# maropu/spark-data-repair-plugin

Hardware: AMD Instinct MI355X
Metric: repaired cells/sec (higher is better)
Workload: dtype f32 gradients (LightGBM's score_t), exact int64 fixed-point histogram sums, f64 scores

## Files before the change

### include/rgbm.h

```cpp
#ifndef RGBM_H_
#define RGBM_H_

#include <stddef.h>
#include <stdint.h>

#ifdef __cplusplus
extern "C" {
#endif

#define RGBM_OK 0
#define RGBM_ERR_ARG (-1)
#define RGBM_ERR_PARAM (-2)
#define RGBM_ERR_LABEL (-3)
#define RGBM_ERR_NO_DEVICE (-10)
#define RGBM_ERR_HIP (-11)
#define RGBM_ERR_NOMEM (-12)
#define RGBM_ERR_FORMAT (-20)

#define RGBM_OBJ_BINARY 0
#define RGBM_OBJ_MULTICLASS 1
#define RGBM_OBJ_REGRESSION 2

typedef struct rgbm_model rgbm_model;
typedef struct rgbm_table rgbm_table;
// ... 35 lines not shown
    int64_t level_atomics_per_row;
} rgbm_train_stats;

int rgbm_device_count(void);
int rgbm_release_cache(void);
const char* rgbm_last_error(void);
int rgbm_version(void);

int rgbm_train(const int32_t* X_colmajor, int64_t n, int32_t f, const int32_t* n_codes,
               const int32_t* y_code, int32_t n_y_codes, const double* y_value,
               const double* class_weight, const double* sample_weight,
               const rgbm_params* p, rgbm_model** out, rgbm_train_stats* stats );

int rgbm_predict(const rgbm_model* m, const int32_t* X_colmajor, int64_t n, int32_t f,
                 int32_t device_id, double* out);

int rgbm_repair_chain(const rgbm_model* const* models, int32_t T, const int32_t* target_col,
                      const int32_t* feat_cols, const int32_t* feat_off,
                      const int32_t* class_code, const int32_t* class_off,
                      int32_t* table_colmajor, int64_t n, int32_t c, int32_t device_id,
                      int32_t* out_label, double* out_prob);

int rgbm_table_create(const int32_t* codes_colmajor, int64_t n, int32_t c, const int32_t* n_codes,
                      int32_t device_id, rgbm_table** out);
int rgbm_table_set_column_kind(rgbm_table* t, int32_t col, int32_t kind);
int rgbm_table_set_column_values(rgbm_table* t, int32_t col, const double* values, int32_t n);
int rgbm_host_alloc(size_t bytes, void** out);
void rgbm_host_free(void* p);
void rgbm_table_free(rgbm_table* t);
int rgbm_table_train(const rgbm_table* t, int32_t target_col, const int32_t* feat_cols, int32_t f,
                     const double* y_value ,
                     const double* class_weight ,
                     const rgbm_params* p, rgbm_model** out, rgbm_train_stats* stats);
int rgbm_table_set_row_multiplicity(rgbm_table* t, const uint8_t* mult );
int rgbm_table_read_row_multiplicity(const rgbm_table* t, uint8_t* mult_out );
int rgbm_table_distinct_rows(const rgbm_table* t, rgbm_table** out, int64_t* n_out, int64_t* inverse_out );
int rgbm_table_distinct_view_info(const rgbm_table* t, int32_t* state, int64_t* rows, int64_t* builds);
int rgbm_distinct_view_eligible(int64_t rows, int32_t f, const rgbm_params* p, int32_t table_has_mult, int64_t min_rows);
typedef struct {
    const rgbm_table* table;
    int32_t target_col, n_features;
    const int32_t* feat_cols;
    const double* y_value;
    const double* class_weight;
    const rgbm_params* params;
    const rgbm_table* valid_table;
    int32_t* valid_label_out;
    double* valid_value_out;
} rgbm_fit_spec;
int rgbm_table_train_batch(const rgbm_fit_spec* fits, int32_t n_fits, rgbm_model** out_models , int32_t* out_status );
int rgbm_table_repair_chain(rgbm_table* t, const rgbm_model* const* models, int32_t T,
                            const int32_t* target_col, const int32_t* feat_cols, const int32_t* feat_off,
                            int64_t row_begin, int64_t n_rows, int32_t* out_label, double* out_prob);
int rgbm_table_read_column(const rgbm_table* t, int32_t col, int32_t* out );

int rgbm_table_detect_nulls(rgbm_table* t, const int32_t* cols, int32_t n_cols, int64_t* n_cells_out);
int rgbm_table_detect_cells(rgbm_table* t, const int32_t* cols, int32_t n_cols, const uint8_t* null_is_error ,
                            const int32_t* keep_lo, const int32_t* keep_hi ,
                            const uint64_t* const* flag_bits , int64_t* n_cells_out);
int rgbm_table_detect_constraint(rgbm_table* t, const int32_t* eq_cols, int32_t n_eq, int32_t iq_col,
                                 const int32_t* cell_cols, int32_t n_cell_cols,
                                 int64_t* n_rows_out , int64_t* n_cells_out);
#define RGBM_DC_EQ 0
#define RGBM_DC_IQ 1
#define RGBM_DC_LT 2
#define RGBM_DC_GT 3
typedef struct rgbm_dc_pred {
    int32_t op;
    int32_t left_col;
    int32_t right_col;
    int32_t reserved;
    const int32_t* left_rank;
    const int32_t* right_rank;
} rgbm_dc_pred;
int rgbm_table_detect_dc(rgbm_table* t, const rgbm_dc_pred* preds, int32_t n_preds, const int32_t* cell_cols, int32_t n_cell_cols,
                         int64_t max_pairs, int64_t* n_rows_out , int64_t* n_cells_out);
int rgbm_table_detect_row_bits(rgbm_table* t, const int32_t* cols, int32_t n_cols, const uint64_t* const* bits ,
                               const int32_t* cell_cols, int32_t n_cell_cols, int64_t* n_rows_out , int64_t* n_cells_out);
int rgbm_table_rows_of_cells(rgbm_table* t, const int64_t* rows, int64_t n_cells, int64_t* n_rows_out);
int rgbm_table_cells_fetch(const rgbm_table* t, int64_t* rows_out , int32_t* cols_out );
int rgbm_table_null_cells(rgbm_table* t, const int64_t* rows, const int32_t* cols, int64_t n_cells,
                          const int32_t* target_cols, int32_t n_targets);
int rgbm_table_read_cells(const rgbm_table* t, const int64_t* rows, const int32_t* cols, int64_t n_cells, int32_t* codes_out);
int rgbm_table_write_cells(rgbm_table* t, const int64_t* rows, const int32_t* cols, const int32_t* codes, int64_t n_cells);
int rgbm_table_gather_rows(const rgbm_table* t, const int64_t* rows, int64_t n_rows, rgbm_table** out);
int rgbm_table_count_codes(const rgbm_table* t, int32_t col, int64_t* counts_out ,
                           int64_t* n_null_out );
int rgbm_table_column_stats(const rgbm_table* t, const int32_t* cols, int32_t n_cols, const int32_t* const* len_lut,
                            int32_t n_bins, int64_t* stats_out, int32_t* edges_out);
int rgbm_table_create_dict(const int32_t* idx_colmajor, int64_t n, int32_t c, const int32_t* const* remap,
                           const int32_t* dict_size , int32_t device_id, rgbm_table** out);
int rgbm_table_repair_pmf(rgbm_table* t, const rgbm_model* m, int32_t target_col, const int32_t* feat_cols, int32_t f,
                          int32_t top_k, double threshold, const int32_t* cur_code, int64_t cap, int64_t* n_cells_out,
                          int64_t* rows_out , int32_t* class_out ,
                          double* prob_out , double* cur_prob_out );
int rgbm_table_repair_pmf_weighted(rgbm_table* t, const rgbm_model* m, int32_t target_col, const int32_t* feat_cols, int32_t f,
                                   int32_t top_k, double threshold, const int32_t* cur_code ,
                                   const int32_t* cost_row , const double* cost ,
                                   int64_t n_cost_rows, double weight, int32_t renormalise, int64_t cap, int64_t* n_cells_out,
                                   int64_t* rows_out , int32_t* class_out , double* prob_out ,
                                   double* cur_prob_out , double* top1_cost_out );
int rgbm_edit_distance(int32_t device_id, const int32_t* a_cp, const int64_t* a_off, int64_t n_a, const int32_t* b_cp,
                       const int64_t* b_off, int64_t n_b, int32_t* dist_out);
int rgbm_table_pair_counts(rgbm_table* t, const int32_t* pair_cols, int32_t n_pairs, const int32_t* const* luts ,
                           const int32_t* n_bins , int64_t* counts_out);
int rgbm_table_cell_domains(rgbm_table* t, int32_t target_col, const int64_t* rows, int64_t n_cells, const int32_t* pair_idx, int32_t k,
                            const int64_t* min_cnt , const uint8_t* single_ok , double beta, int64_t row_count,
                            uint8_t* weak_out, int32_t* top_out, double* top_prob_out, double* probs_out );
int rgbm_table_fd_map(const rgbm_table* t, int32_t x_col, int32_t y_col, int32_t* map_out );
int rgbm_table_rule_fill(rgbm_table* t, int32_t y_col, int32_t x_col , const int32_t* lut, int32_t n_lut, int64_t row_begin,
                         int64_t n_rows, int32_t* out_label );
int rgbm_nearest_values(int32_t device_id, const int32_t* a_cp, const int64_t* a_off, int64_t n_a, const int32_t* b_cp, const int64_t* b_off,
                        int64_t n_b, const double* cost , double threshold, int32_t* nearest_out );
int rgbm_lof_1d(int32_t device_id, const double* values , const int64_t* counts ,
                int32_t d, int32_t k , double threshold ,
                double* score_out , uint64_t* flag_bits_out , int64_t* info_out );
int rgbm_table_kmeans_assign(rgbm_table* t, const int32_t* cols, int32_t n_cols, const int64_t* code_off ,
                             int32_t k, const double* p , int64_t d_tot, const double* h ,
                             int32_t first ,
                             int64_t* counts_out , int64_t* sizes_out , int64_t* n_changed_out);
int rgbm_table_kmeans_read(const rgbm_table* t, int32_t* assign_out );
int rgbm_table_shape(const rgbm_table* t, int64_t* n_out, int32_t* c_out, int32_t* n_codes_out );

#define RGBM_COMM_ID_BYTES 128
#define RGBM_FLAG_ROW_SHARDED 1
#define RGBM_FLAG_WHOLE_TABLE 4
#define RGBM_FLAG_NO_MODEL 2
int rgbm_comm_unique_id(void* id_out );
int rgbm_comm_init(const void* id, int32_t rank, int32_t nranks, int32_t device_id);
int rgbm_comm_finalize(void);
int rgbm_comm_info(int32_t* info );
int rgbm_comm_count(int32_t* n_out );
int rgbm_comm_all_gather_sizes(const int64_t* mine, int32_t n, int64_t* all );
int rgbm_comm_all_gather_bytes(const void* send, int64_t my_bytes, int64_t block_bytes , void* recv );
int rgbm_table_repair_chain_gather(rgbm_table* t, const rgbm_model* const* models, int32_t T, const int32_t* target_col,
                                   const int32_t* feat_cols, const int32_t* feat_off, int64_t row_begin, int64_t n_rows, int64_t max_rows,
                                   int32_t* out_label, double* out_prob);
int rgbm_comm_gather_stats(int64_t* out );
int rgbm_local_group_create(int32_t nranks, int32_t device_id, void** group_out);
void rgbm_local_group_free(void* group);
int rgbm_comm_init_local(void* group, int32_t rank);

int rgbm_fusion_create(int32_t n_members, void** fusion_out);
int rgbm_fusion_join(void* fusion, int32_t member );
int rgbm_fusion_leave(int32_t failed );
int rgbm_fusion_info(void* fusion, int64_t* info );
int rgbm_fusion_free(void* fusion);

int rgbm_model_save(const rgbm_model* m, void* buf, size_t* len);
int rgbm_model_load(const void* buf, size_t len, rgbm_model** out);
void rgbm_model_free(rgbm_model* m);
int rgbm_model_info(const rgbm_model* m, int32_t* info);
int rgbm_model_predict_form(const rgbm_model* m, int32_t* out);
int rgbm_level_pass_plan(const int32_t* nbins, int32_t f, int64_t n_rows, int32_t k, int32_t max_depth, int32_t with_mult, double* out, int32_t out_len, int32_t* n_out);
int rgbm_model_importance(const rgbm_model* m, int32_t type, double* out );

#ifdef __cplusplus
}
#endif
#endif
```

### spark-data-repair-plugin_amd/csrc/rgbm.hip

```cpp
#include <hip/hip_runtime.h>
#include <algorithm>
#include <atomic>
#include <condition_variable>
#include <chrono>
#include <cmath>
#include <cstdio>
#include <cstdlib>
#include <cstring>
#include <deque>
#include <map>
#include <memory>
#include <stdexcept>
#include <mutex>
#include <string>
#include <thread>
#include <vector>

#include "rgbm_host.h"
#include "rgbm_kernels.h"
#include "rgbm_level.h"
#include "rgbm_small.h"


namespace {
using rgh::fail; using rgh::DevBuf; using rgh::use_device; using rgh::StreamGuard; using rgh::guarded;
using rgh::AR_I64; using rgh::AR_U32; using rgh::AR_I32; using rgh::all_reduce; using rgh::all_gather_on; using rgh::stream_sync_watchdog; using rgh::comm_abort;
using rgh::comm_kind; using rgh::comm_rank; using rgh::comm_nranks; using rgh::upload_pinned;

struct Feat {
    int32_t n_codes = 0, V = 0, has_nan = 0; std::vector<int32_t> ub;
    std::vector<uint32_t> unseen;
    bool is_unseen(int32_t c) const { return !unseen.empty() && ((unseen[(size_t)c >> 5] >> (c & 31)) & 1u); }
};
struct Tree {
    int32_t L = 1;
    double *gain = nullptr, *leaf_value = nullptr;
    int32_t *feat = nullptr, *theta = nullptr, *dleft = nullptr, *left = nullptr, *right = nullptr, *leaf_count = nullptr;
    std::unique_ptr<double[]> own;
    static size_t doubles(int L) { const size_t n = (size_t)L - 1; return n + (size_t)L + (5 * n + (size_t)L + 1) / 2; }
    void place(double* p, int L_) {
        L = L_; const size_t n = (size_t)L - 1;
        gain = p; leaf_value = p + n;
        int32_t* q = reinterpret_cast<int32_t*>(p + n + L);
        feat = q; theta = q + n; dleft = q + 2 * n; left = q + 3 * n; right = q + 4 * n; leaf_count = q + 5 * n;
    }
    void alloc(int L_) { own.reset(new double[doubles(L_)]); place(own.get(), L_); }
};

struct DeviceModel {
    DevBuf<rg::PNode> nodes; DevBuf<double> leaf_value;
    DevBuf<uint32_t> qs_masks, qs_used; DevBuf<double> qs_leaves; DevBuf<int32_t> qs_foff; int qs_S = 0, qs_MW = 0;
    DevBuf<uint8_t> lut; DevBuf<long long> lut_off; DevBuf<int32_t> n_codes; DevBuf<uint8_t> miss; DevBuf<int32_t> ident;
    int node_stride = 1, leaf_stride = 1;
};

}

struct rgbm_model {
    int32_t objective = 0, num_class = 0, K = 1, n_iter = 0, F = 0;
    std::vector<Feat> feats;
    std::vector<Tree> trees;
    std::unique_ptr<double[]> tree_arena;
    std::mutex mu;
    std::map<int, DeviceModel*> dev;
    ~rgbm_model() { for (auto& kv : dev) { (void)hipSetDevice(kv.first); delete kv.second; } }
};


namespace {

int32_t mid_code(int32_t a, int32_t b, const double* vals) {
    if (!vals) return (int32_t)(((int64_t)a + (int64_t)b) / 2);
    const double m = (vals[a] + vals[b]) / 2.0;
    int32_t lo = a, hi = b - 1;
    while (lo < hi) { const int32_t c = lo + (hi - lo + 1) / 2; if (vals[c] <= m) lo = c; else hi = c - 1; }
    return lo;
}

int greedy_find_bin(const std::vector<int32_t>& dv, const std::vector<int64_t>& cnt, int max_bin, int64_t total_cnt,
                    int min_data_in_bin, std::vector<int32_t>& ub, const double* vals) {
    const int nd = (int)dv.size();
    ub.clear();
    if (nd <= 0) return 0;
    if (nd <= max_bin) {
        int64_t cur = 0;
        for (int i = 0; i + 1 < nd; ++i) {
            cur += cnt[i];
            if (cur >= min_data_in_bin) { ub.push_back(mid_code(dv[i], dv[i + 1], vals)); cur = 0; }
        }
        ub.push_back(INT32_MAX);
        return (int)ub.size();
    }
    if (min_data_in_bin > 0) {
        max_bin = (int)std::min<int64_t>(max_bin, total_cnt / min_data_in_bin);
        max_bin = std::max(max_bin, 1);
    }
    double mean_bin_size = (double)total_cnt / max_bin;
    int rest_bin_cnt = max_bin;
    int64_t rest_sample_cnt = total_cnt;
    std::vector<char> big(nd, 0);
    for (int i = 0; i < nd; ++i)
        if ((double)cnt[i] >= mean_bin_size) { big[i] = 1; --rest_bin_cnt; rest_sample_cnt -= cnt[i]; }
    mean_bin_size = (double)rest_sample_cnt / rest_bin_cnt;
    std::vector<int32_t> upper(max_bin, INT32_MAX), lower(max_bin, INT32_MAX);
    int bin_cnt = 0;
    lower[0] = dv[0];
    int64_t cur = 0;
    for (int i = 0; i + 1 < nd; ++i) {
        if (!big[i]) rest_sample_cnt -= cnt[i];
        cur += cnt[i];
        double half = mean_bin_size * 0.5f;
        if (half < 1.0) half = 1.0;
        if (big[i] || (double)cur >= mean_bin_size || (big[i + 1] && (double)cur >= half)) {
            upper[bin_cnt] = dv[i];
            ++bin_cnt;
            lower[bin_cnt] = dv[i + 1];
            if (bin_cnt >= max_bin - 1) break;
            cur = 0;
            if (!big[i]) { --rest_bin_cnt; mean_bin_size = (double)rest_sample_cnt / (double)rest_bin_cnt; }
        }
    }
    ++bin_cnt;
    for (int i = 0; i + 1 < bin_cnt; ++i) {
        int32_t v = mid_code(upper[i], lower[i + 1], vals);
        if (ub.empty() || ub.back() != v) ub.push_back(v);
    }
    ub.push_back(INT32_MAX);
    return (int)ub.size();
}

void find_bin(const unsigned int* cnt, int32_t n_codes, int64_t n_train, const rgbm_params& p, Feat& f, const double* vals) {
    std::vector<int32_t> dv; std::vector<int64_t> dc;
    int64_t seen = 0;
    for (int32_t c = 0; c < n_codes; ++c) if (cnt[c]) { dv.push_back(c); dc.push_back(cnt[c]); seen += cnt[c]; }
    const int64_t na = n_train - seen;
    int mb = p.max_bin - (na > 0 ? 1 : 0) - 1;
    if (mb < 1) mb = 1;
    f.n_codes = n_codes; f.has_nan = na > 0 ? 1 : 0;
    f.V = greedy_find_bin(dv, dc, mb, seen, p.min_data_in_bin, f.ub, vals);
}


constexpr double DISTINCT_MAX_RATIO = 0.5;
constexpr long long DISTINCT_MIN_ROWS = 1ll << 20;
struct RunSwitches {
    int grower = 0;
    bool timing = false;
    int lv_lds = 0;
    long long lv_blocks = 0;
    long long mt_blocks = 0;
    int mt_T = 0;
    int mt_rep = 8;
    bool joint_root = true;
    bool mt_acc2 = true;
    bool mt_sparse = true;
    int mt_rot = -1;
    int mt_rot_copies2 = 16;
    int mt_rot_tmin = 2;
    bool step_readback = false;
    int step_threads = 0;
    int step_max_gx = 0;
    bool fx_separate = false;
    bool distinct = true;
    double distinct_max_ratio = DISTINCT_MAX_RATIO;
    long long distinct_min_rows = DISTINCT_MIN_ROWS;
};
RunSwitches read_switches() {
    RunSwitches w;
    if (const char* e = getenv("RGBM_GROWER")) w.grower = strcmp(e, "leafwise") == 0 ? 2 : (strcmp(e, "level") == 0 ? 1 : 0);
    if (const char* e = getenv("RGBM_LV_LDS")) w.lv_lds = atoi(e);
    if (const char* e = getenv("RGBM_LV_BLOCKS")) w.lv_blocks = atoll(e);
    if (const char* e = getenv("RGBM_MT_BLOCKS")) w.mt_blocks = atoll(e);
    if (const char* e = getenv("RGBM_MT_TREES")) w.mt_T = atoi(e);
    if (const char* e = getenv("RGBM_MT_REP")) w.mt_rep = atoi(e);
    if (const char* e = getenv("RGBM_JOINT_ROOT")) w.joint_root = atoi(e) != 0;
    if (const char* e = getenv("RGBM_MT_ACC2")) w.mt_acc2 = atoi(e) != 0;
    if (const char* e = getenv("RGBM_MT_SPARSE")) w.mt_sparse = atoi(e) != 0;
    if (const char* e = getenv("RGBM_STEP_READBACK")) w.step_readback = atoi(e) != 0;
    if (const char* e = getenv("RGBM_STEP_THREADS")) w.step_threads = atoi(e);
    if (const char* e = getenv("RGBM_STEP_MAX_GX")) w.step_max_gx = atoi(e);
    if (const char* e = getenv("RGBM_FX_MEASURE")) w.fx_separate = strcmp(e, "separate") == 0;
    if (const char* e = getenv("RGBM_MT_ROT")) w.mt_rot = atoi(e);
    if (const char* e = getenv("RGBM_MT_ROT_COPIES2")) w.mt_rot_copies2 = atoi(e);
    if (const char* e = getenv("RGBM_MT_ROT_TMIN")) w.mt_rot_tmin = atoi(e);
    if (const char* e = getenv("RGBM_DISTINCT")) w.distinct = atoi(e) != 0;
    if (const char* e = getenv("RGBM_DISTINCT_MAX_RATIO")) { const double r = atof(e); if (r >= 0.0 && r <= 1.0) w.distinct_max_ratio = r; }
    if (const char* e = getenv("RGBM_DISTINCT_MIN_ROWS")) w.distinct_min_rows = std::max(1ll, atoll(e));
    w.timing = getenv("RGBM_TIMING") != nullptr;
    return w;
}

struct LgbRand {
    uint32_t x;
    explicit LgbRand(uint32_t seed) : x(seed) {}
    int rnd16() { x = 214013u * x + 2531011u; return (int)((x >> 16) & 0x7FFF); }
    int rnd32() { x = 214013u * x + 2531011u; return (int)(x & 0x7FFFFFFF); }
    float next_float() { return (float)rnd16() / 32768.0f; }
    int next_int(int lo, int hi) { return rnd32() % (hi - lo) + lo; }
    std::vector<int> sample(int N, int K) {
        std::vector<int> ret;
        if (K > N || K <= 0) return ret;
        if (K == N) { for (int i = 0; i < N; ++i) ret.push_back(i); return ret; }
        if (K > 1 && (double)K > ((double)N / std::log2((double)K))) {
            for (int i = 0; i < N; ++i) {
                double prob = (double)(K - (int)ret.size()) / (double)(N - i);
                if (next_float() < prob) ret.push_back(i);
            }
            return ret;
        }
        std::vector<char> in(N, 0);
        for (int r = N - K; r < N; ++r) { int v = next_int(0, r); if (in[v]) in[r] = 1; else in[v] = 1; }
        for (int i = 0; i < N; ++i) if (in[i]) ret.push_back(i);
        return ret;
    }
};


void check_params(const rgbm_params& p) {
    if (p.objective < 0 || p.objective > 2) throw std::invalid_argument("objective must be 0 (binary), 1 (multiclass) or 2 (regression)");
    if (p.max_bin < 2 || p.max_bin > 255) throw std::invalid_argument("max_bin must be in [2, 255]");
    if (p.num_leaves < 2 || p.num_leaves > 32767) throw std::invalid_argument("num_leaves must be in [2, 32767]");
    if (p.n_estimators < 1) throw std::invalid_argument("n_estimators must be positive");
    if (!(p.learning_rate > 0.0)) throw std::invalid_argument("learning_rate must be positive");
    if (p.objective == 2 && p.learning_rate > 1.0) throw std::invalid_argument("regression with learning_rate > 1 is not supported");
    if (p.objective == 1 && p.num_class < 2) throw std::invalid_argument("multiclass needs num_class >= 2");
    if (p.min_data_in_leaf < 0 || p.lambda_l1 < 0 || p.lambda_l2 < 0) throw std::invalid_argument("negative regularisation / min_data_in_leaf");
    if (p.bagging_fraction <= 0.0 || p.bagging_fraction > 1.0) throw std::invalid_argument("bagging_fraction must be in (0, 1]");
    if (p.feature_fraction <= 0.0 || p.feature_fraction > 1.0) throw std::invalid_argument("feature_fraction must be in (0, 1]");
}

struct HostLabelStats {
    bool valid = false;
    std::vector<double> tot; double suml = 0.0, w_max = 0.0;
};

struct FitHost {
    int64_t n_train = 0; int nchunk = 1; size_t lds_hist = 0;
    std::vector<int32_t> cols, ncod; std::vector<long long> cnt_off, lut_off; std::vector<unsigned int> cnt;
    std::vector<rg::FeatMeta> fmeta; std::vector<rg::ChunkMeta> cmeta; std::vector<uint8_t> lut, miss, trivial;
    std::vector<double> init, yv32; rg::TrainConst tc;
    std::unique_ptr<rgbm_model> model;
};

void fit_setup(const rgbm_table& tab, const double* y_value_in, const double* class_weight, const HostLabelStats* hls, const rgbm_params& p, int32_t F, FitHost& h) {
    using namespace rg;
    const int64_t N = tab.n;
    const int obj = p.objective;
    const std::vector<int32_t>& cols = h.cols; const std::vector<int32_t>& ncod = h.ncod; const std::vector<long long>& cnt_off = h.cnt_off;
    const std::vector<unsigned int>& cnt = h.cnt;
    const int n_y = ncod[F];
    const int K = obj == 1 ? p.num_class : 1;
    const double* y_value = nullptr;
    if (obj == 2) { h.yv32.resize(std::max(n_y, 1)); for (int c = 0; c < n_y; ++c) h.yv32[c] = (double)(float)y_value_in[c]; y_value = h.yv32.data(); }
    const unsigned int* ycnt = cnt.data() + cnt_off[F];
    int64_t& n_train = h.n_train; n_train = 0;
    for (int c = 0; c < n_y; ++c) n_train += ycnt[c];
    if (n_train <= 0) throw std::out_of_range("no training rows (every target cell is NULL)");
    if (N >= (1ll << 31) - 4096) throw std::invalid_argument("more than 2^31 rows per table are not supported");

    h.model.reset(new rgbm_model());
    rgbm_model* model = h.model.get();
    model->objective = obj; model->num_class = obj == 1 ? K : (obj == 0 ? 2 : 1); model->K = K; model->F = F;
    model->feats.resize(F);
    std::vector<FeatMeta>& fmeta = h.fmeta; fmeta.assign(F, FeatMeta());
    std::vector<long long>& lut_off = h.lut_off; lut_off.assign(F + 1, 0);
    std::vector<uint8_t>& miss = h.miss; std::vector<uint8_t>& trivial = h.trivial; miss.assign(F, 0); trivial.assign(F, 0);
    int totbins = 0;
    for (int f = 0; f < F; ++f) {
        Feat& ft = model->feats[f];
        const std::vector<double>* cv = (size_t)cols[f] < tab.col_values.size() ? &tab.col_values[cols[f]] : nullptr;
        find_bin(cnt.data() + cnt_off[f], ncod[f], n_train, p, ft, (cv && (int32_t)cv->size() == ncod[f] && ncod[f] > 0) ? cv->data() : nullptr);
        if ((size_t)cols[f] < tab.col_kind.size() && tab.col_kind[cols[f]] == 1) {
            const unsigned int* cf = cnt.data() + cnt_off[f];
            bool any = false;
            for (int32_t c = 0; c < ncod[f]; ++c) any |= cf[c] == 0;
            if (any) {
                ft.unseen.assign((size_t)(ncod[f] + 31) / 32, 0u);
                for (int32_t c = 0; c < ncod[f]; ++c) if (cf[c] == 0) ft.unseen[(size_t)c >> 5] |= 1u << (c & 31);
            }
        }
        fmeta[f].V = ft.V; fmeta[f].has_nan = ft.has_nan; fmeta[f].nbins = std::max(ft.V + ft.has_nan, 1); fmeta[f].hoff = totbins;
        totbins += fmeta[f].nbins;
        trivial[f] = (ft.V + ft.has_nan <= 1) || ft.V == 0;
        miss[f] = (uint8_t)(ft.has_nan ? ft.V : 0);
        lut_off[f + 1] = lut_off[f] + std::max(ncod[f], 1);
    }
    std::vector<uint8_t>& lut = h.lut; lut.assign(lut_off[F], 0);
    for (int f = 0; f < F; ++f) {
        const Feat& ft = model->feats[f];
        int b = 0;
        for (int c = 0; c < ncod[f]; ++c) { while (b < ft.V - 1 && c > ft.ub[b]) ++b; lut[lut_off[f] + c] = (uint8_t)(ft.V > 0 ? b : 0); }
    }
    const int nchunk = (F + 15) / 16; h.nchunk = nchunk;
    std::vector<ChunkMeta>& cmeta = h.cmeta; cmeta.assign(nchunk, ChunkMeta());
    size_t& lds_hist = h.lds_hist; lds_hist = 0;
    for (int ch = 0; ch < nchunk; ++ch) {
        ChunkMeta& cm = cmeta[ch]; cm.first_feat = ch * 16; cm.nfeat = std::min(16, F - ch * 16); cm.fast_slots = 0; cm.wide_bins = 0;
        for (int j = 0; j < cm.nfeat; ++j) {
            FeatMeta& m = fmeta[ch * 16 + j];
            int sh = 0; while (sh < 5 && (m.nbins << (sh + 1)) <= 256) ++sh;
            m.rep_shift = sh; m.fast_base = cm.fast_slots; m.wide_off = cm.wide_bins;
            cm.fast_slots += m.nbins << sh; cm.wide_bins += m.nbins;
        }
        lds_hist = std::max(lds_hist, (size_t)cm.fast_slots * 16);
    }

    const int nl = std::max({n_y, obj == 0 ? 2 : 1, obj == 1 ? K : 1});
    std::vector<double> tot(nl, 0.0);
    double w_max = 0.0;
    if (hls && hls->valid) { tot = hls->tot; tot.resize(nl, 0.0); w_max = hls->w_max; }
    else {
        for (int c = 0; c < n_y; ++c) {
            const double cw32 = class_weight ? (double)(float)class_weight[c] : 1.0;
            tot[c] = (double)ycnt[c] * cw32;
            if (ycnt[c]) w_max = std::max(w_max, cw32);
        }
    }
    if (!(w_max > 0.0)) w_max = 1.0;
    double sumw = 0.0;
    for (int c = 0; c < nl; ++c) sumw += tot[c];
    std::vector<double>& init = h.init; init.assign(K, 0.0);
    double ymin = 0.0, ymax = 0.0;
    const double keps = k_eps();
    if (obj == 2) {
        bool first = true; double suml = 0.0;
        for (int c = 0; c < n_y; ++c) {
            if (!ycnt[c]) continue;
            if (first) { ymin = ymax = y_value[c]; first = false; }
            ymin = std::min(ymin, y_value[c]); ymax = std::max(ymax, y_value[c]);
        }
        if (hls && hls->valid) suml = hls->suml; else for (int c = 0; c < nl; ++c) suml += tot[c] * (c < n_y ? y_value[c] : 0.0);
        init[0] = suml / sumw;
    } else if (obj == 0) {
        double pavg = tot[1] / sumw;
        if (pavg > 1.0 - keps) pavg = 1.0 - keps;
        if (pavg < keps) pavg = keps;
        init[0] = std::log(pavg / (1.0 - pavg));
    } else {
        for (int k = 0; k < K; ++k) { double pr = tot[k] / sumw; init[k] = std::log(pr > keps ? pr : keps); }
    }
    const double factor = obj == 1 ? (double)K / (double)(K - 1) : 1.0;
    double bound_g, bound_h;
    if (obj == 2) { bound_g = (ymax - ymin) * w_max; if (!(bound_g > 0.0)) bound_g = 1.0; bound_h = w_max; }
    else if (obj == 0) { bound_g = w_max; bound_h = 0.25 * w_max; }
    else { bound_g = w_max; bound_h = factor * 0.25 * w_max; }
    double wr = sumw / w_max;
    long long q_mult = 1;
    if (const char* th = std::getenv("RGBM_TEST_HOOKS")) if (std::atoi(th) != 0) if (const char* ev = std::getenv("RGBM_FX_ROWS")) {
        const double R = std::atof(ev);
        if (R > (double)n_train && R <= 4294967296.0 && n_train > 0) {
            wr *= R / (double)n_train; q_mult = ((long long)R + n_train - 1) / n_train;
            static std::atomic<bool> said{false};
            if (!said.exchange(true)) fprintf(stderr, "[rgbm] TEST HOOK active: RGBM_FX_ROWS=%s coarsens the fixed-point grid of every model trained by this process\n", ev);
        }
    }
    const int e_g = rg::fx_exponent(bound_g, wr), e_h = rg::fx_exponent(bound_h, wr);

    TrainConst& tc = h.tc; memset(&tc, 0, sizeof(tc));
    tc.sg = std::ldexp(1.0, e_g); tc.sh = std::ldexp(1.0, e_h); tc.inv_sg = std::ldexp(1.0, -e_g); tc.inv_sh = std::ldexp(1.0, -e_h);
    tc.l1 = p.lambda_l1; tc.l2 = p.lambda_l2; tc.min_gain_to_split = p.min_gain_to_split; tc.min_sum_hessian = p.min_sum_hessian_in_leaf;
    tc.learning_rate = p.learning_rate; tc.factor = factor; tc.min_data_in_leaf = p.min_data_in_leaf; tc.max_depth = p.max_depth;
    tc.num_leaves = p.num_leaves; tc.F = F; tc.K = K; tc.totbins = std::max(totbins, 1); tc.nchunk = nchunk; tc.objective = obj;
    tc.N = N; tc.n_train = n_train; tc.NG = N;
    tc.fx.c_g = 24 - rg::fx_ceil_log2(bound_g); tc.fx.c_h = 24 - rg::fx_ceil_log2(bound_h);
    tc.fx.e_g_min = e_g; tc.fx.e_h_min = e_h;
    tc.fx.e_g_max = 50 - rg::fx_ceil_log2(bound_g); tc.fx.e_h_max = 50 - rg::fx_ceil_log2(bound_h);
    tc.fx.q_mult = q_mult;
}

struct HostTrees { const int32_t *L, *feat, *theta, *dleft, *left, *right, *cnt; const double *gain, *val; const int32_t* any; };
size_t model_trees_begin(rgbm_model* model, const HostTrees& h, int NE, int K) {
    int n_iter = NE;
    for (int it = 0; it < NE; ++it) if (!h.any[it]) { n_iter = it > 0 ? it : 1; break; }
    model->n_iter = n_iter;
    const size_t nt = (size_t)n_iter * K;
    model->trees.clear(); model->trees.resize(nt);
    size_t total = 0;
    for (size_t t = 0; t < nt; ++t) total += Tree::doubles(std::max(h.L[t], 1));
    model->tree_arena.reset(new double[std::max<size_t>(total, 1)]);
    size_t off = 0;
    for (size_t t = 0; t < nt; ++t) { const int L = std::max(h.L[t], 1); model->trees[t].place(model->tree_arena.get() + off, L); off += Tree::doubles(L); }
    return nt;
}
void model_trees_fill(rgbm_model* model, const HostTrees& h, int NL, size_t t0, size_t t1) {
    for (size_t t = t0; t < t1; ++t) {
        Tree& tr = model->trees[t];
        const size_t n = (size_t)tr.L - 1, nb = t * (NL - 1), lb = t * NL;
        memcpy(tr.feat, h.feat + nb, 4 * n); memcpy(tr.theta, h.theta + nb, 4 * n); memcpy(tr.dleft, h.dleft + nb, 4 * n);
        memcpy(tr.left, h.left + nb, 4 * n); memcpy(tr.right, h.right + nb, 4 * n); memcpy(tr.gain, h.gain + nb, 8 * n);
        memcpy(tr.leaf_value, h.val + lb, 8 * (size_t)tr.L); memcpy(tr.leaf_count, h.cnt + lb, 4 * (size_t)tr.L);
    }
}
void model_from_trees(rgbm_model* model, const HostTrees& h, int NE, int K, int NL) {
    const size_t n = model_trees_begin(model, h, NE, K);
    model_trees_fill(model, h, NL, 0, n);
}

std::vector<uint8_t> make_used_masks(const rgbm_params& p, size_t NT, int F, const std::vector<uint8_t>& trivial) {
    std::vector<uint8_t> used(NT * F, 0);
    LgbRand sr((uint32_t)p.seed);
    sr.rnd16(); sr.rnd16(); sr.rnd16();
    LgbRand ff((uint32_t)sr.rnd16());
    std::vector<int> valid; for (int f = 0; f < F; ++f) if (!trivial[f]) valid.push_back(f);
    for (size_t t = 0; t < NT; ++t) {
        uint8_t* u = used.data() + t * F;
        if (p.feature_fraction < 1.0) {
            int cntf = (int)std::floor((double)valid.size() * p.feature_fraction + 0.5);
            if (cntf < 1) cntf = 1;
            for (int i : ff.sample((int)valid.size(), cntf)) u[valid[i]] = 1;
        } else for (int f : valid) u[f] = 1;
    }
    return used;
}

struct MtLaunch { int ch, slot0, nslots, route, T, G, gx, acc2, rot; };
struct LevelPassPlan {
    int root_gx = 8;
    std::vector<std::vector<MtLaunch>> mt;
    std::vector<int> mt_gx;
    size_t part_items = 0;
};

struct PassCost { double t_fix_us, t_row_ns, t_pair_ns; };
constexpr PassCost MT_COST_REP{14.0, 0.2, 0.75};
constexpr PassCost MT_COST_ROT{14.0, 1.0, 0.5};
constexpr PassCost ROOT_PASS_COST{8.0, 1.2, 0.0};
inline const PassCost& mt_pass_cost(bool , bool rot) { return rot ? MT_COST_ROT : MT_COST_REP; }
inline double pass_model_us(long long workgroups, double rows_per_block, int T, const PassCost& c) {
    const long long rounds = (workgroups + 255) / 256;
    return (double)rounds * (c.t_fix_us + rows_per_block * (c.t_row_ns + (double)T * c.t_pair_ns) * 1e-3);
}

inline int level_lds_bytes(const RunSwitches& sw) { return (sw.lv_lds >= 65536 && sw.lv_lds <= rg::LV_LDS_BYTES) ? sw.lv_lds : rg::LV_LDS_BYTES; }

LevelPassPlan plan_level_passes(const RunSwitches& sw, const std::vector<rg::FeatMeta>& fmeta, const std::vector<rg::ChunkMeta>& cmeta,
                                long long N, int K, int max_depth, bool wm , int lds_bytes) {
    using namespace rg;
    const int nchunk = (int)cmeta.size();
    LevelPassPlan P;
    P.mt.resize(LV_MAX_DEPTH + 1); P.mt_gx.assign(LV_MAX_DEPTH + 1, 8);
    const long long ntiles = (N + LV_TILE - 1) / LV_TILE;
    {
        const long long cu_slots = 256, per = (long long)K * nchunk;
        const long long gmin = std::max<long long>(1, (N + (1ll << 22) - 1) >> 22);
        auto time_of = [&](long long g) { return pass_model_us(g * per, (double)N / (double)g, 1, ROOT_PASS_COST); };
        const long long gfloor = std::max<long long>(8, (gmin + 7) / 8 * 8), gcap = std::max<long long>(gfloor, std::min<long long>(512, (ntiles + 7) / 8 * 8));
        long long g2 = gfloor; double best2 = -1.0;
        for (int pass = 0; pass < 2 && best2 < 0.0; ++pass)
            for (long long g = gfloor; g <= gcap; g += 8) {
                if (pass == 0 && per >= 16 && (g * per < 3 * cu_slots || g * per > 5 * cu_slots)) continue;
                const double t = time_of(g);
                if (best2 < 0.0 || t < best2 * (1.0 - 1e-9)) { best2 = t; g2 = g; }
            }
        if (sw.lv_blocks >= 1) g2 = (sw.lv_blocks + 7) / 8 * 8;
        P.root_gx = (int)g2;
    }
    for (int ch = 0; ch < nchunk; ++ch)
        if ((long long)lv_slots(fmeta.data() + cmeta[ch].first_feat, cmeta[ch].nfeat, 0) * 16 + LV_ROOT_FIXED > lds_bytes)
            throw std::invalid_argument("histogram of one node exceeds LDS");
    P.part_items = (size_t)K * P.root_gx;
    for (int level = 1; level < max_depth; ++level) {
        const int worst = 1 << (level - 1);
        bool acc2 = nchunk == 2 && sw.mt_acc2;
        if (acc2) {
            const long long nb2 = ((long long)lv_slots(fmeta.data() + cmeta[0].first_feat, cmeta[0].nfeat, 0) + lv_slots(fmeta.data() + cmeta[1].first_feat, cmeta[1].nfeat, 0)) * 16;
            if (nb2 > mt_hist_bytes(lds_bytes, MT_THREADS_ACC2, true, true, cmeta[1].nfeat > 15 || wm)) acc2 = false;
        }
        if (wm && nchunk == 2 && !acc2) throw std::invalid_argument("a two-chunk table with row multiplicities needs the one-pass level form (the multiplicity rides in the second record)");
        for (int ch = 0; ch < (acc2 ? 1 : nchunk); ++ch) {
            const FeatMeta* fm = fmeta.data() + cmeta[ch].first_feat;
            long long node_bytes = (long long)lv_slots(fm, cmeta[ch].nfeat, 0) * 16;
            if (acc2) node_bytes += (long long)lv_slots(fmeta.data() + cmeta[1].first_feat, cmeta[1].nfeat, 0) * 16;
            const int mt_thr = acc2 ? MT_THREADS_ACC2 : LV_THREADS;
            const bool li_arr = cmeta[acc2 ? 1 : ch].nfeat > 15 || wm;
            const long long hist_room = mt_hist_bytes(lds_bytes, mt_thr, acc2, acc2 , li_arr);
            long long cap = hist_room / std::max<long long>(node_bytes, 1);
            cap = std::min<long long>(cap, MT_MAX_NODES);
            if (cap < 1) throw std::invalid_argument("histogram of one node exceeds LDS");
            const int win = (int)std::min<long long>(worst, cap);
            const long long rep_target = std::max(1, sw.mt_rep);
            const long long t_nodes = std::max<long long>(win, cap / rep_target);
            int T = (int)std::max<long long>(1, std::min<long long>(std::min<long long>(t_nodes / win, MT_MAX_T), std::min<long long>(K, MT_RT_BUDGET / (2 * worst))));
            if (sw.mt_T >= 1) T = std::max(1, std::min(T, sw.mt_T));
            const bool plain1 = nchunk == 1 || acc2;
            const bool rot_full = cmeta[ch].nfeat >= 12 && (!acc2 || cmeta[1].nfeat >= 12);
            const long long rot_node_bytes = node_bytes + mt_rot_dummy(true) * 16;
            const long long cap_rot = std::min<long long>(hist_room / rot_node_bytes, MT_MAX_NODES);
            const long long T_rot = std::min<long long>(std::min<long long>(cap_rot / win, MT_MAX_T), std::min<long long>(K, MT_RT_BUDGET / (2 * worst)));
            const bool few_trees = T < sw.mt_rot_tmin && T_rot >= 2 * (long long)T;
            const bool rot = plain1 && (sw.mt_rot == 1 || (sw.mt_rot < 0 && rot_full && (cap * 2 < (long long)sw.mt_rot_copies2 * T * win || few_trees))) &&
                             (long long)T * win * rot_node_bytes <= hist_room;
            if (rot && sw.mt_T < 1) T = (int)std::max<long long>(T, T_rot);
            const int G = (K + T - 1) / T;
            for (int s0 = 0; s0 < worst; s0 += win)
                P.mt[level].push_back(MtLaunch{ch, s0, win, (ch == 0 && s0 == 0) ? 1 : 0, T, G, 0, acc2 ? 1 : 0, rot ? 1 : 0});
        }
        const long long gmin = std::max<long long>(1, (N + (1ll << 22) - 1) >> 22);
        const long long nwt = (N + MT_WT_ROWS - 1) / MT_WT_ROWS;
        const long long gx_lo = std::max<long long>(8, (gmin + 7) / 8 * 8), gx_hi = std::max<long long>(gx_lo, std::min<long long>(512, (nwt / (4 * (LV_THREADS / 64)) + 7) / 8 * 8));
        long long gx = gx_lo; double best = 0.0;
        for (long long g = gx_lo; g <= gx_hi; g += 8) {
            double t = 0.0;
            for (const auto& L : P.mt[level]) t += pass_model_us((long long)L.G * g, (double)N / (double)g, std::min(L.T, K), mt_pass_cost(L.acc2 != 0, L.rot != 0));
            if (g == gx_lo || t < best * (1.0 - 1e-9)) { best = t; gx = g; }
        }
        if (sw.mt_blocks >= 1) gx = (sw.mt_blocks + 7) / 8 * 8;
        P.mt_gx[level] = (int)gx;
        for (auto& L : P.mt[level]) L.gx = (int)gx;
        P.part_items = std::max(P.part_items, (size_t)K * (size_t)gx * (size_t)worst);
    }
    return P;
}

struct JointRootPlan {
    bool on = false;
    std::vector<std::vector<int>> groups;
    std::vector<rg::FeatMeta> vfm; rg::ChunkMeta vcm;
    std::vector<rg::JointFeat> jf;
    std::vector<int16_t> binfeat;
};
JointRootPlan plan_joint_root(const std::vector<rg::FeatMeta>& fmeta, int totbins, bool wm, int lds_bytes) {
    using namespace rg;
    const int F = (int)fmeta.size();
    JointRootPlan J;
    std::vector<int> order(F); for (int f = 0; f < F; ++f) order[f] = f;
    std::stable_sort(order.begin(), order.end(), [&](int a, int b) { return fmeta[a].nbins > fmeta[b].nbins; });
    std::vector<int> prod;
    for (int f : order) {
        int best = -1;
        for (size_t g = 0; g < J.groups.size(); ++g)
            if ((long long)prod[g] * fmeta[f].nbins <= 256 && (best < 0 || prod[g] > prod[best])) best = (int)g;
        if (best < 0) { J.groups.emplace_back(); prod.push_back(1); best = (int)J.groups.size() - 1; }
        J.groups[best].push_back(f); prod[best] *= fmeta[f].nbins;
    }
    const int VF = (int)J.groups.size();
    if (VF > (wm ? 15 : 16) || VF > F - 2) return J;
    J.vfm.resize(VF); J.jf.resize(F); J.binfeat.assign(totbins, 0);
    ChunkMeta& vcm = J.vcm; vcm.first_feat = 0; vcm.nfeat = VF; vcm.fast_slots = 0; vcm.wide_bins = 0;
    for (int v = 0; v < VF; ++v) {
        FeatMeta& m = J.vfm[v]; memset(&m, 0, sizeof(m));
        m.V = prod[v]; m.has_nan = 0; m.nbins = prod[v]; m.hoff = vcm.wide_bins; m.wide_off = vcm.wide_bins;
        int sh = 0; while (sh < 5 && (m.nbins << (sh + 1)) <= 256) ++sh;
        m.rep_shift = sh; m.fast_base = vcm.fast_slots; vcm.fast_slots += m.nbins << sh; vcm.wide_bins += m.nbins;
        int stride = 1;
        for (int f : J.groups[v]) {
            JointFeat& j = J.jf[f]; memset(&j, 0, sizeof(j));
            j.voff = m.hoff; j.stride = stride; j.nbins = fmeta[f].nbins; j.nbv = prod[v]; j.hoff = fmeta[f].hoff; j.vbyte = v;
            stride *= fmeta[f].nbins;
            for (int b = 0; b < fmeta[f].nbins; ++b) J.binfeat[fmeta[f].hoff + b] = (int16_t)f;
        }
    }
    J.on = (long long)lv_slots(J.vfm.data(), VF, 0) * 16 + LV_ROOT_FIXED <= lds_bytes;
    return J;
}

#define RGBM_MT_FORMS(X) \
    X(0, rg::LV_THREADS, false, false, false)  \
    X(1, rg::LV_THREADS, false, false, false)  \
    X(1, rg::LV_THREADS, false, false, true)   \
    X(2, rg::LV_THREADS, false, false, false)  \
    X(2, rg::MT_THREADS_ACC2, true, true, false)  \
    X(2, rg::MT_THREADS_ACC2, true, true, true)
struct MtForm { int nchr, threads; bool acc2, spec, rot; };
constexpr MtForm MT_FORMS[] = {
#define RGBM_MT_FORM_ENTRY(NCHR, THR, ACC, SPEC, ROT) {NCHR, THR, ACC, SPEC, ROT},
    RGBM_MT_FORMS(RGBM_MT_FORM_ENTRY)
#undef RGBM_MT_FORM_ENTRY
};
using MtKernel = decltype(&rg::k_level_mt<1, false, true, rg::LV_THREADS, false, false, false>);
MtKernel mt_kernel(const MtForm& f, bool bag, bool route) {
#define RGBM_MT_FORM_KERNEL(NCHR, THR, ACC, SPEC, ROT) \
    if (f.nchr == NCHR && f.threads == THR && f.acc2 == ACC && f.spec == SPEC && f.rot == ROT) \
        return bag ? (route ? rg::k_level_mt<NCHR, true, true, THR, ACC, SPEC, ROT> : rg::k_level_mt<NCHR, true, false, THR, ACC, SPEC, ROT>) \
                   : (route ? rg::k_level_mt<NCHR, false, true, THR, ACC, SPEC, ROT> : rg::k_level_mt<NCHR, false, false, THR, ACC, SPEC, ROT>);
    RGBM_MT_FORMS(RGBM_MT_FORM_KERNEL)
#undef RGBM_MT_FORM_KERNEL
    throw std::logic_error("level pass: no such launch form");
}
void launch_level_mt(const MtForm& f, bool bag, bool route, dim3 grid, hipStream_t s, const uint4* rec, const float2* gh, uint8_t* node, const uint8_t* inbag,
                     const rg::LvPlan* plan, rg::HistBin* part, int32_t* count, const rg::FeatMeta* fmeta, const rg::ChunkMeta* cmeta, int32_t* err_flag,
                     const rg::FxScale* fxs, const rg::LevelConst& c) {
    hipLaunchKernelGGL(mt_kernel(f, bag, route), grid, dim3(f.threads), rg::LV_LDS_BYTES, s, rec, gh, node, inbag, plan, part, count, fmeta, cmeta, err_flag, fxs, c);
}
struct HistTimers {
    bool on; hipStream_t s;
    std::deque<rgh::Event> ev; std::vector<char> root;
    template <typename Fn> void timed(bool is_root, Fn&& fn) {
        if (!on) { fn(); return; }
        HIPCHK(hipEventRecord(ev.emplace_back().e, s));
        fn();
        HIPCHK(hipEventRecord(ev.emplace_back().e, s));
        root.push_back(is_root ? 1 : 0);
    }
};

struct LevelTrace {
    struct Rec { std::string name; int it, level; size_t off, bytes; };
    const char* dir; bool on; hipStream_t s;
    int lo = 44, hi = 44, cur_it = 0;
    std::vector<Rec> idx; size_t used = 0;
    DevBuf<unsigned char> buf;
    LevelTrace(bool level_mode, int K, hipStream_t stream) : dir(getenv("RGBM_TRACE")), s(stream) {
        on = dir && level_mode && (!getenv("RGBM_TRACE_K") || atoi(getenv("RGBM_TRACE_K")) == K);
        if (on && getenv("RGBM_TRACE_ITERS")) sscanf(getenv("RGBM_TRACE_ITERS"), "%d:%d", &lo, &hi);
    }
    void copy(const char* name, int level, const void* src, size_t bytes) {
        if (!on || cur_it < lo || cur_it > hi) return;
        if (used + bytes > buf.n) return;
        HIPCHK(hipMemcpyAsync(buf.p + used, src, bytes, hipMemcpyDeviceToDevice, s));
        idx.push_back({name, cur_it, level, used, bytes}); used += (bytes + 15) & ~(size_t)15;
    }
    void sum(const char* name, const void* src, size_t bytes) {
        if (!on || used + 16 > buf.n) return;
        HIPCHK(hipMemsetAsync(buf.p + used, 0, 8, s));
        rgh::trace_sum(src, bytes, (unsigned long long*)(buf.p + used), s);
        idx.push_back({name, cur_it, -1, used, 8}); used += 16;
    }
    void write(int target_col) {
        if (!on || !used) return;
        std::vector<unsigned char> h(used);
        HIPCHK(hipMemcpy(h.data(), buf.p, used, hipMemcpyDeviceToHost));
        char path[512];
        snprintf(path, sizeof(path), "%s/target%d.bin", dir, target_col);
        if (FILE* f = fopen(path, "wb")) { fwrite(h.data(), 1, h.size(), f); fclose(f); }
        snprintf(path, sizeof(path), "%s/target%d.idx", dir, target_col);
        if (FILE* f = fopen(path, "w")) { for (const auto& r : idx) fprintf(f, "%s %d %d %zu %zu\n", r.name.c_str(), r.it, r.level, r.off, r.bytes); fclose(f); }
    }
};

void fill_train_stats(rgbm_train_stats* stats, float total_ms, const HistTimers& timers, const HostTrees& h, const rgbm_params& p, bool level_mode, bool use_bagging,
                      int nranks , int64_t N, int64_t n_train, int F, int root_feats ,
                      int K, unsigned long long statrows) {
    const int NE = p.n_estimators, NL = p.num_leaves;
    memset(stats, 0, sizeof(*stats));
    stats->total_ms = total_ms;
    stats->hist_launches = (int64_t)timers.root.size();
    for (size_t i = 0; i < timers.root.size(); ++i) {
        float m2 = 0.f; HIPCHK(hipEventElapsedTime(&m2, timers.ev[2 * i].e, timers.ev[2 * i + 1].e));
        stats->hist_ms += m2; if (timers.root[i]) stats->root_ms += m2;
    }
    stats->trees = (int64_t)NE * K;
    const bool root_done = n_train >= (int64_t)p.min_data_in_leaf * 2;
    if (level_mode) {
        const int64_t root_rows = (root_done && !use_bagging) ? (int64_t)NE * K * n_train : 0;
        const int64_t rows_acc = (int64_t)(statrows / (unsigned long long)nranks);
        stats->hist_rows = rows_acc; stats->root_rows = root_rows / nranks;
        stats->root_atomics_per_row = 2 * (int64_t)root_feats; stats->level_atomics_per_row = 2 * (int64_t)F;
        stats->hist_bytes = rows_acc * ((int64_t)F + 8);
        return;
    }
    int64_t rows = 0, root_rows = 0;
    for (size_t t = 0; t < (size_t)NE * K; ++t) {
        const int L = h.L[t];
        const int32_t* left = h.left + t * (NL - 1); const int32_t* right = h.right + t * (NL - 1);
        if (root_done) { rows += N; root_rows += N; }
        std::vector<int64_t> fin(h.cnt + t * NL, h.cnt + t * NL + NL);
        std::vector<int64_t> nodecnt(std::max(L - 1, 1), 0);
        auto sub = [&](int ch) -> int64_t { return ch < 0 ? fin[~ch] : nodecnt[ch]; };
        for (int j = L - 2; j >= 0; --j) nodecnt[j] = sub(left[j]) + sub(right[j]);
        std::vector<int> node_depth(std::max(L - 1, 1), 0);
        for (int j = 0; j < L - 1; ++j) {
            const int lc = left[j], rc = right[j];
            if (lc >= 0) node_depth[lc] = node_depth[j] + 1;
            if (rc >= 0) node_depth[rc] = node_depth[j] + 1;
            const int64_t a = sub(lc), b = sub(rc);
            bool go = j + 2 < NL;
            if (p.max_depth > 0 && node_depth[j] + 1 >= p.max_depth) go = false;
            if (a < (int64_t)p.min_data_in_leaf * 2 && b < (int64_t)p.min_data_in_leaf * 2) go = false;
            if (go) rows += std::min(a, b);
        }
    }
    stats->hist_rows = rows; stats->root_rows = root_rows;
    stats->hist_bytes = rows * ((int64_t)F + 8) + (rows - root_rows) * 4;
}

void check_fit_args(const rgbm_table& tab, int32_t target_col, const int32_t* feat_cols, int32_t F, const double* y_value, const rgbm_params& p) {
    check_params(p);
    if (F <= 0) throw std::invalid_argument("no feature columns");
    if (target_col < 0 || target_col >= tab.c) throw std::invalid_argument("target column out of range");
    for (int f = 0; f < F; ++f) if (feat_cols[f] < 0 || feat_cols[f] >= tab.c) throw std::invalid_argument("feature column out of range");
    const int obj = p.objective, n_y = tab.n_codes[target_col];
    if (obj == 1 && n_y > p.num_class) throw std::out_of_range("target has more label codes than num_class");
    if (obj == 0 && n_y > 2) throw std::out_of_range("binary objective with more than 2 label codes");
    if (obj == 2 && !y_value) throw std::out_of_range("regression needs the y_value dictionary");
}

struct BinRecords {
    DevBuf<int32_t> cols, ncod; DevBuf<long long> cnt_off; DevBuf<unsigned int> cnt;
    DevBuf<rg::FeatMeta> fmeta; DevBuf<rg::ChunkMeta> cmeta; DevBuf<long long> lut_off; DevBuf<uint8_t> lut, miss; DevBuf<uint4> rec;
    void count_codes(const rgbm_table& tab, int32_t target_col, const int32_t* feat_cols, int32_t F, FitHost& h, hipStream_t s) {
        h.cols.assign(feat_cols, feat_cols + F); h.cols.push_back(target_col);
        h.ncod.resize(F + 1); h.cnt_off.assign(F + 2, 0);
        for (int f = 0; f <= F; ++f) { h.ncod[f] = tab.n_codes[h.cols[f]]; h.cnt_off[f + 1] = h.cnt_off[f] + std::max(h.ncod[f], 1); }
        cols.alloc(F + 1); ncod.alloc(F + 1); cnt_off.alloc(F + 2); cnt.alloc(h.cnt_off[F + 1]);
        cols.upload(h.cols.data(), F + 1, s); ncod.upload(h.ncod.data(), F + 1, s); cnt_off.upload(h.cnt_off.data(), F + 2, s); cnt.zero(s);
        const int gx = (int)std::min<int64_t>((tab.n + 255) / 256, 1024);
        hipLaunchKernelGGL(rg::k_count_codes, dim3(gx, F + 1), dim3(256), 0, s, tab.codes.p, (long long)tab.n, tab.codes.p + (long long)target_col * tab.n, cols.p, ncod.p,
                           cnt_off.p, cnt.p, tab.has_mult ? tab.mult.p : (const uint8_t*)nullptr);
    }
    void download_counts(FitHost& h, hipStream_t s) const { h.cnt.resize(cnt.n); cnt.download(h.cnt.data(), cnt.n, s); }
    void fill(const FitHost& h, long long N, hipStream_t s) {
        const int F = h.tc.F;
        fmeta.alloc(F); cmeta.alloc(h.nchunk); lut_off.alloc(F + 1); lut.alloc(h.lut.size()); miss.alloc(F);
        fmeta.upload(h.fmeta.data(), F, s); cmeta.upload(h.cmeta.data(), h.nchunk, s); lut_off.upload(h.lut_off.data(), F + 1, s);
        lut.upload(h.lut.data(), h.lut.size(), s); miss.upload(h.miss.data(), F, s);
        rec.alloc((size_t)h.nchunk * N);
    }
    void pack(const rgbm_table& t, const uint8_t* lut_, const uint8_t* miss_, uint4* out, const uint8_t* mult, hipStream_t s) const {
        hipLaunchKernelGGL(rg::k_pack_bins, dim3((unsigned)((t.n + 255) / 256)), dim3(256), 0, s, t.codes.p, (long long)t.n, 0ll, (long long)t.n, cols.p, ncod.p,
                           lut_off.p, lut_, miss_, (int)fmeta.n, (int)cmeta.n, out, mult);
    }
    void pack(const rgbm_table& tab, hipStream_t s) { pack(tab, lut.p, miss.p, rec.p, tab.has_mult ? tab.mult.p : (const uint8_t*)nullptr, s); }
};

struct BagState {
    DevBuf<unsigned int> blk, rand, bagcnt; DevBuf<int32_t> sorted_rows, oob; DevBuf<uint8_t> inbag;
    std::vector<unsigned int> seeds;
    long long off = 0, local = 0, nrb = 1;
    void order_rows(const int32_t* d_ycol, long long N, long long n_train, hipStream_t s) {
        const long long nblk = (N + 1023) / 1024;
        blk.alloc(nblk); sorted_rows.alloc(n_train); oob.alloc(n_train); inbag.alloc(N); bagcnt.alloc(2);
        hipLaunchKernelGGL(rg::k_block_count, dim3((unsigned)nblk), dim3(256), 0, s, d_ycol, N, blk.p);
        hipLaunchKernelGGL(rg::k_block_scan, dim3(1), dim3(1024), 0, s, blk.p, nblk);
        hipLaunchKernelGGL(rg::k_stable_compact, dim3((unsigned)nblk), dim3(256), 0, s, d_ycol, N, blk.p, sorted_rows.p);
    }
    void seed(const rgbm_params& p, long long bag_off, long long bag_local, hipStream_t s) {
        off = bag_off; local = bag_local;
        nrb = std::max<long long>(1, (off + local + 1023) / 1024 - off / 1024);
        LgbRand sr2((uint32_t)p.seed); sr2.rnd16();
        const int bagging_seed = sr2.rnd16();
        seeds.resize(nrb);
        for (long long b = 0; b < nrb; ++b) seeds[b] = (unsigned int)(bagging_seed + off / 1024 + b);
        rand.alloc(nrb); rand.upload(seeds.data(), nrb, s);
    }
};

struct TreeBlock {
    DevBuf<int32_t> L, feat, theta, dleft, left, right, cnt, any; DevBuf<double> gain, val;
    void alloc(size_t NT, int NL, int NE, hipStream_t s) {
        const size_t nn = NT * (size_t)(NL - 1), nl = NT * (size_t)NL;
        any.alloc(NE); any.zero(s);
        L.alloc(NT); feat.alloc(nn); theta.alloc(nn); dleft.alloc(nn); left.alloc(nn); right.alloc(nn); cnt.alloc(nl); gain.alloc(nn); val.alloc(nl);
        cnt.zero(s); val.zero(s);
    }
    rg::TreeOut out() const { return rg::TreeOut{L.p, feat.p, theta.p, dleft.p, left.p, right.p, gain.p, val.p, cnt.p}; }
    void host_layout(size_t (&off)[11]) const {
        const size_t bytes[10] = {L.n * 4, feat.n * 4, theta.n * 4, dleft.n * 4, left.n * 4, right.n * 4, cnt.n * 4, gain.n * 8, val.n * 8, any.n * 4};
        off[0] = 0;
        for (int i = 0; i < 10; ++i) off[i + 1] = off[i] + ((bytes[i] + 63) & ~(size_t)63);
    }
    size_t host_bytes() const { size_t off[11]; host_layout(off); return off[10]; }
    HostTrees download(char* base, hipStream_t s) const {
        size_t off[11]; host_layout(off);
        auto get = [&](const auto& buf, int i) { auto* h = reinterpret_cast<decltype(buf.p)>(base + off[i]); buf.download(h, buf.n, s); return h; };
        return HostTrees{get(L, 0), get(feat, 1), get(theta, 2), get(dleft, 3), get(left, 4), get(right, 5), get(cnt, 6), get(gain, 7), get(val, 8), get(any, 9)};
    }
};

struct FitState {
    const rgbm_table& tab; const rgbm_params& p; hipStream_t s; const int32_t F;
    const RunSwitches sw = read_switches();
    const int K = p.objective == 1 ? p.num_class : 1, NL = p.num_leaves, NE = p.n_estimators; const int64_t N = tab.n;
    const bool use_bagging = p.bagging_freq > 0 && p.bagging_fraction < 1.0;
    const bool level_mode = p.max_depth >= 1 && p.max_depth <= rg::LV_MAX_DEPTH && F <= 255 && sw.grower != 2;
    const bool dp = (p.reserved & RGBM_FLAG_ROW_SHARDED) != 0;
    const int32_t* d_ycol; const uint8_t* d_mult = tab.has_mult ? tab.mult.p : (const uint8_t*)nullptr;
    FitHost h; BinRecords bins;
    DevBuf<int32_t> base;
    DevBuf<unsigned int> counter;
    DevBuf<float2> gh;
    DevBuf<double> score, init;
    DevBuf<unsigned long long> fxq;
    DevBuf<rg::FxScale> fxs;
    DevBuf<unsigned long long> qpart; long long fx_parts = 0; bool fx_fused = false;
    TreeBlock trees;
    DevBuf<double> cw, yv, sw_rows; DevBuf<uint8_t> used;
    BagState bag; DevBuf<unsigned int> bagcnt_g;
    const unsigned int* n_in_ptr = nullptr;
    DevBuf<int32_t> it;
    HistTimers timers;

    FitState(const rgbm_table& tab_, int32_t target_col, int32_t F_, const rgbm_params& p_, bool timed, hipStream_t s_)
        : tab(tab_), p(p_), s(s_), F(F_), d_ycol(tab_.codes.p + (long long)target_col * tab_.n), timers{timed, s_} {}

    int grad_gx() const { return (int)std::min<long long>((N + 255) / 256, 4096); }
    bool mc_tile() const { return p.objective == 1 && K >= 16 && K <= 112; }
    bool mc_rows() const { return p.objective == 1 && K < 16; }
    void alloc_fx_parts() {
        if (sw.fx_separate || (p.objective == 1 && !mc_tile() && !mc_rows())) return;
        fx_fused = true; fx_parts = mc_tile() ? (N + 63) / 64 : (mc_rows() ? ((N + 255) / 256) * 4 : (long long)grad_gx());
        qpart.alloc((size_t)fx_parts * K * 2);
    }
    void enqueue_grad(uint8_t* node0, long long NS);
    void enqueue_bagging();
};

struct LevelGrower {
    FitState& st; hipStream_t s;
    int root_feats;
    unsigned long long statrows = 0;
    rg::LevelConst lc, lcj; LevelPassPlan passes;
    const int n_hnodes = (1 << st.p.max_depth) - 1;
    bool use_reduce = false;
    bool joint_root = false; int vtotbins = 0;
    DevBuf<rg::FeatMeta> vfmeta; DevBuf<rg::ChunkMeta> vcmeta; DevBuf<uint4> rec_j; DevBuf<rg::HistBin> part_j, red_j; DevBuf<rg::JointFeat> jf; DevBuf<int16_t> binfeat;
    DevBuf<uint8_t> node; DevBuf<rg::LvPlan> plan; DevBuf<rg::SNode> snodes;
    DevBuf<rg::ScanLane> scan_map; std::vector<rg::ScanLane> h_scan; int scan_waves = 0; bool step_hist_lds = true;
    int step_threads = 512, step_max_gx = 256;
    DevBuf<rg::HistBin> part, lpool, part_red; DevBuf<int32_t> count, count_g, err, leafnode; DevBuf<double> ndelta; DevBuf<unsigned long long> d_statrows;
    const int score_gx = (int)std::max<long long>(1, std::min<long long>((st.N + 1023) / 1024, (2048 + st.K - 1) / st.K));
    LevelTrace trace;
    int32_t h_err = 0;
    std::vector<rg::RootLayout> h_root_lay; std::vector<rg::MtLayout> h_mt_lay; std::vector<int> mt_lay_keys;
    DevBuf<rg::RootLayout> root_lay; DevBuf<rg::MtLayout> mt_lay;
    static int mt_lay_key(const MtLaunch& L) { return L.ch * 4 + (L.acc2 ? 2 : 0) + (L.rot ? 1 : 0); }
    int mt_lay_index(const MtLaunch& L) const {
        for (size_t i = 0; i < mt_lay_keys.size(); ++i) if (mt_lay_keys[i] == mt_lay_key(L)) return (int)i;
        return -1;
    }

    explicit LevelGrower(FitState& st_) : st(st_), s(st_.s), root_feats(st_.F), trace(true, st_.K, st_.s) {
        using namespace rg;
        memset(&lc, 0, sizeof(lc)); memset(&lcj, 0, sizeof(lcj));
        lc.lds_bytes = level_lds_bytes(st.sw);
        lc.nchunk = st.h.nchunk; lc.K = st.K; lc.F = st.F; lc.totbins = st.h.tc.totbins;
        lc.num_leaves = st.NL; lc.max_depth = st.p.max_depth; lc.min_data_in_leaf = st.p.min_data_in_leaf; lc.N = st.N; lc.NS = (st.N + 255) & ~255ll; lc.NG = lc.NS;
        lc.sib_local = (st.dp && comm_rank() == 0) ? 1 : 0;
        lc.has_mult = st.tab.has_mult ? 1u : 0u;
        passes = plan_level_passes(st.sw, st.h.fmeta, st.h.cmeta, st.N, st.K, st.p.max_depth, st.tab.has_mult, lc.lds_bytes);
        lc.gx = passes.root_gx; lc.xcd_blocks = 1; lc.max_built = 1;
        node.alloc((size_t)st.K * lc.NS);
        HIPCHK(hipMemsetAsync(node.p, 0xFF, (size_t)st.K * lc.NS, s));
        plan.alloc(st.K); snodes.alloc((size_t)st.K * 256);
        part.alloc(passes.part_items * st.h.tc.totbins); lpool.alloc((size_t)st.K * n_hnodes * st.h.tc.totbins);
        scan_waves = scan_lane_map(st.h.fmeta.data(), st.F, h_scan);
        scan_map.alloc(h_scan.size()); scan_map.upload(h_scan.data(), h_scan.size(), s);
        step_hist_lds = ls_hist_in_lds(st.h.tc.totbins, st.F) && !st.sw.step_readback;
        if (st.sw.step_threads >= 128 && st.sw.step_threads <= LS_MAX_THREADS && st.sw.step_threads % 64 == 0) step_threads = st.sw.step_threads;
        if (st.sw.step_max_gx >= 1) step_max_gx = st.sw.step_max_gx;
        count.alloc((size_t)st.K * 256); use_reduce = st.dp || lc.gx > step_max_gx;
        if (st.dp) count_g.alloc((size_t)st.K * 256);
        const int max_built_all = 1 << std::max(0, st.p.max_depth - 2);
        part_red.alloc((size_t)st.K * max_built_all * st.h.tc.totbins + (size_t)st.K * 128 );
        leafnode.alloc((size_t)st.K * LV_MAX_LEAVES); err.alloc(1); err.zero(s); ndelta.alloc((size_t)st.K * 256); d_statrows.alloc(1); d_statrows.zero(s);
        if (st.sw.joint_root && ((long long)st.K * st.N >= (1ll << 21) || (st.tab.has_mult && st.h.nchunk == 2))) {
            const JointRootPlan jp = plan_joint_root(st.h.fmeta, st.h.tc.totbins, st.tab.has_mult, lc.lds_bytes);
            if (jp.on) {
                const int VF = (int)jp.vfm.size();
                joint_root = true; vtotbins = jp.vcm.wide_bins;
                vfmeta.alloc(VF); vfmeta.upload(jp.vfm.data(), VF, s); vcmeta.alloc(1); vcmeta.upload(&jp.vcm, 1, s);
                jf.alloc(st.F); jf.upload(jp.jf.data(), st.F, s); binfeat.alloc(jp.binfeat.size()); binfeat.upload(jp.binfeat.data(), jp.binfeat.size(), s);
                rec_j.alloc((size_t)st.N);
                hipLaunchKernelGGL(k_pack_joint, dim3((unsigned)((st.N + 255) / 256)), dim3(256), 0, s, st.bins.rec.p, (long long)st.N, st.F, jf.p, rec_j.p, st.tab.has_mult ? st.h.nchunk - 1 : -1);
                part_j.alloc((size_t)st.K * lc.gx * vtotbins); red_j.alloc((size_t)st.K * vtotbins + (size_t)st.K * 128 );
                lcj = lc; lcj.nchunk = 1; lcj.F = VF; lcj.totbins = vtotbins; lcj.max_built = 1;
                h_root_lay.resize(1); root_layout_fill(h_root_lay[0], jp.vfm.data(), VF, lc.lds_bytes);
                use_reduce = true; root_feats = VF;
                HIPCHK(hipStreamSynchronize(s));
            }
        }
        if (st.tab.has_mult && st.h.nchunk == 2 && !joint_root)
            throw std::invalid_argument("a two-chunk table with row multiplicities needs the joint-bin root pass (its record carries the multiplicity); this feature set does not pack into 15 groups");
        if (!joint_root) {
            h_root_lay.resize(st.h.nchunk);
            for (int ch = 0; ch < st.h.nchunk; ++ch) root_layout_fill(h_root_lay[ch], st.h.fmeta.data() + st.h.cmeta[ch].first_feat, st.h.cmeta[ch].nfeat, lc.lds_bytes);
        }
        root_lay.alloc(h_root_lay.size()); root_lay.upload(h_root_lay.data(), h_root_lay.size(), s);
        lc.root_lay = root_lay.p; lcj.root_lay = root_lay.p;
        for (int level = 1; level < st.p.max_depth; ++level) for (const auto& L : passes.mt[level]) if (mt_lay_index(L) < 0) {
            const bool acc2 = L.acc2 != 0;
            const ChunkMeta& cm = st.h.cmeta[L.ch];
            const int nf_last = acc2 ? st.h.cmeta[1].nfeat : cm.nfeat;
            const bool li_in_rec = nf_last <= 15 && !st.tab.has_mult;
            mt_lay_keys.push_back(mt_lay_key(L)); h_mt_lay.emplace_back();
            mt_layout_fill(h_mt_lay.back(), st.h.fmeta.data() + cm.first_feat, cm.nfeat, acc2 ? st.h.fmeta.data() + st.h.cmeta[1].first_feat : nullptr, acc2 ? st.h.cmeta[1].nfeat : 0,
                           cm.wide_bins, L.rot != 0, mt_hist_bytes(lc.lds_bytes, acc2 ? MT_THREADS_ACC2 : LV_THREADS, acc2, acc2, !li_in_rec));
        }
        if (!h_mt_lay.empty()) { mt_lay.alloc(h_mt_lay.size()); mt_lay.upload(h_mt_lay.data(), h_mt_lay.size(), s); }
        if (st.sw.timing) {
            fprintf(stderr, "[rgbm] root: gx %d joint %d groups %d\n", lc.gx, joint_root ? 1 : 0, joint_root ? lcj.F : 0);
            for (int level = 1; level < st.p.max_depth; ++level) for (const auto& L : passes.mt[level])
                fprintf(stderr, "[rgbm] level %d launch: chunk %d slots %d..%d route %d T %d G %d gx %d acc2 %d rot %d\n", level, L.ch, L.slot0, L.slot0 + L.nslots - 1, L.route, L.T, L.G, L.gx, L.acc2, L.rot);
        }
        rgh::once_per_device(st.tab.device, rgh::ONCE_LEVEL_LDS, [] {
            HIPCHK(hipFuncSetAttribute((const void*)rg::k_level_root, hipFuncAttributeMaxDynamicSharedMemorySize, rg::LV_LDS_BYTES));
            for (const MtForm& f : MT_FORMS) for (int bag = 0; bag < 2; ++bag) for (int route = 0; route < 2; ++route)
                HIPCHK(hipFuncSetAttribute((const void*)mt_kernel(f, bag != 0, route != 0), hipFuncAttributeMaxDynamicSharedMemorySize, rg::LV_LDS_BYTES));
        });
        if (trace.on) trace.buf.alloc(((size_t)st.K * n_hnodes * st.h.tc.totbins * 16 + (size_t)st.K * 256 * (sizeof(SNode) + 4) + (size_t)st.K * sizeof(LvPlan) + 4096) * (size_t)(st.p.max_depth + 1) * (size_t)(trace.hi - trace.lo + 1) + (size_t)st.NE * 64 + 4096);
    }

    void trace_level(int level) {
        trace.copy("count", level, count.p, (size_t)st.K * 256 * 4);
        trace.copy("plan", level, plan.p, (size_t)st.K * sizeof(rg::LvPlan));
        trace.copy("snodes", level, snodes.p, (size_t)st.K * 256 * sizeof(rg::SNode));
        trace.copy("lpool", level, lpool.p, (size_t)st.K * n_hnodes * st.h.tc.totbins * 16);
    }
    std::pair<const rg::HistBin*, rg::LevelConst> exchange(bool root, int nb, const rg::LevelConst& lp) {
        using namespace rg;
        if (root ? !use_reduce : (!st.dp && lp.gx <= step_max_gx)) return {part.p, lp};
        if (root && joint_root) {
            hipLaunchKernelGGL(k_level_reduce, dim3((vtotbins + 63) / 64, 1, st.K), dim3(256), 0, s, part_j.p, red_j.p, plan.p, count.p, 1, 1, lcj);
            hipLaunchKernelGGL(k_level_marginal, dim3((st.h.tc.totbins + 255) / 256, st.K), dim3(256), 0, s, red_j.p, part_red.p, plan.p, count.p, jf.p, binfeat.p, vtotbins, lc);
        } else
            hipLaunchKernelGGL(k_level_reduce, dim3((st.h.tc.totbins + 63) / 64, nb, st.K), dim3(256), 0, s, part.p, part_red.p, plan.p, count.p, root ? 1 : 0, nb, lp);
        if (st.dp) {
            const size_t nh = (size_t)st.K * nb * st.h.tc.totbins * 2;
            all_reduce(part_red.p, nh + (size_t)st.K * 256, AR_I64, s);
            hipLaunchKernelGGL(k_counts_unpack, dim3(st.K), dim3(256), 0, s, reinterpret_cast<const long long*>(part_red.p) + nh, count_g.p);
        }
        LevelConst r = lp; r.gx = 1; r.max_built = nb;
        return {part_red.p, r};
    }
    void enqueue_iteration(int it) {
        using namespace rg;
        const TreeOut to = st.trees.out();
        trace.cur_it = it;
        trace.sum("gh", st.gh.p, (size_t)st.K * st.h.tc.NG * 8);
        hipLaunchKernelGGL(k_level_init, dim3(st.K), dim3(64), 0, s, plan.p, snodes.p, count.p, st.n_in_ptr, (long long)st.h.n_train, st.fxq.p, st.h.tc.fx, st.fxs.p, st.it.p, lc);
        const size_t step_lds = ls_lds_bytes(st.h.tc.totbins, st.F, step_hist_lds);
        int32_t* cntg = st.dp ? count_g.p : count.p;
        st.timers.timed(true, [&]() {
            if (joint_root)
                hipLaunchKernelGGL(k_level_root, dim3((unsigned)lc.gx * (unsigned)st.K, 1, 1), dim3(LV_THREADS), lc.lds_bytes, s, rec_j.p, st.gh.p, node.p, plan.p, part_j.p,
                                   vfmeta.p, vcmeta.p, st.fxs.p, lcj);
            else
                hipLaunchKernelGGL(k_level_root, dim3((unsigned)lc.gx * (unsigned)st.K, 1, st.h.nchunk), dim3(LV_THREADS), lc.lds_bytes, s, st.bins.rec.p, st.gh.p, node.p, plan.p, part.p,
                                   st.bins.fmeta.p, st.bins.cmeta.p, st.fxs.p, lc);
        });
        {
            auto ex = exchange(true, 1, lc);
            hipLaunchKernelGGL(k_level_step<true>, dim3(1, st.K), dim3(step_threads), step_lds, s, ex.first, lpool.p, plan.p, snodes.p, cntg, count.p, st.bins.fmeta.p,
                               st.used.p, scan_map.p, scan_waves, step_hist_lds ? 1 : 0, d_statrows.p, st.it.p, n_hnodes, st.fxs.p, st.h.tc, ex.second);
            trace_level(0);
        }
        for (int level = 1; level < st.p.max_depth; ++level) {
            hipLaunchKernelGGL(k_level_plan, dim3(st.K), dim3(64), 0, s, plan.p, snodes.p, st.bins.fmeta.p, level, st.h.tc, lc);
            LevelConst lp = lc;
            lp.xcd_blocks = 0; lp.gx = passes.mt_gx[level]; lp.max_built = 1 << (level - 1);
            for (const MtLaunch& L : passes.mt[level]) {
                LevelConst l1 = lp;
                l1.mt_T = L.T; l1.mt_G = L.G; l1.mt_ch = L.ch; l1.mt_slot0 = L.slot0; l1.mt_nslots = L.nslots; l1.mt_route = L.route; l1.mt_sparse = st.sw.mt_sparse ? 1 : 0;
                l1.mt_lay = mt_lay.p + mt_lay_index(L);
                const bool acc2 = L.acc2 != 0;
                const MtForm form{acc2 ? 2 : (st.h.nchunk <= 2 ? st.h.nchunk : 0), acc2 ? MT_THREADS_ACC2 : LV_THREADS, acc2, acc2, L.rot != 0};
                st.timers.timed(false, [&]() {
                    launch_level_mt(form, st.use_bagging, L.route != 0, dim3((unsigned)L.G * (unsigned)L.gx), s, st.bins.rec.p, st.gh.p, node.p, st.bag.inbag.p,
                                    plan.p, part.p, count.p, st.bins.fmeta.p, st.bins.cmeta.p, err.p, st.fxs.p, l1);
                });
            }
            auto ex = exchange(false, 1 << (level - 1), lp);
            hipLaunchKernelGGL(k_level_step<false>, dim3(1 << (level - 1), st.K), dim3(step_threads), step_lds, s, ex.first, lpool.p, plan.p, snodes.p,
                               cntg, count.p, st.bins.fmeta.p, st.used.p, scan_map.p, scan_waves, step_hist_lds ? 1 : 0, d_statrows.p, st.it.p, n_hnodes, st.fxs.p, st.h.tc, ex.second);
            trace_level(level);
        }
        hipLaunchKernelGGL(k_level_plan, dim3(st.K), dim3(64), 0, s, plan.p, snodes.p, st.bins.fmeta.p, st.p.max_depth, st.h.tc, lc);
        hipLaunchKernelGGL(k_level_replay, dim3(st.K), dim3(64), 0, s, plan.p, snodes.p, cntg, to, st.init.p, ndelta.p, leafnode.p, st.trees.any.p, err.p, st.it.p, st.h.tc);
        hipLaunchKernelGGL(k_level_final, dim3(score_gx, st.K), dim3(256), 0, s, st.bins.rec.p, node.p, st.bag.inbag.p, plan.p, to, ndelta.p, st.score.p, count.p, st.it.p, lc);
        if (st.dp) { hipLaunchKernelGGL(k_copy_i32, dim3(st.K), dim3(256), 0, s, count.p, count_g.p, (long long)st.K * 256); all_reduce(count_g.p, (size_t)st.K * 256, AR_I32, s); }
        hipLaunchKernelGGL(k_level_leafcount, dim3(st.K), dim3(LV_MAX_LEAVES), 0, s, plan.p, cntg, leafnode.p, to, st.it.p, st.h.tc);
        trace_level(st.p.max_depth);
        trace.sum("score", st.score.p, (size_t)st.K * st.N * 8); trace.sum("node", node.p, (size_t)st.K * lc.NS);
    }
    void enqueue_report() { err.download(&h_err, 1, s); d_statrows.download(&statrows, 1, s); }
    void report(int32_t target_col) {
        trace.write(target_col);
        if (h_err & 2) throw std::runtime_error("level grower: a level pass was launched with more built nodes / route entries than its workgroup tables hold (sizing violated)");
        if (h_err) throw std::runtime_error("level grower: a node outside the speculative expansion was selected (expansion bound violated)");
    }
};

struct LeafwiseGrower {
    FitState& st; hipStream_t s;
    DevBuf<int32_t> idx0, idx1, sorted; DevBuf<rg::HistBin> pool; DevBuf<rg::TreeState> state; DevBuf<rg::Leaf> leaves; DevBuf<rg::Cand> cand; DevBuf<double> upd;
    const long long root_tiles = (st.N + rg::TILE_ROWS - 1) / rg::TILE_ROWS;
    const int hist_gx = (int)std::max<long long>(1, std::min<long long>(root_tiles, (1536 + (long long)st.K * st.h.nchunk - 1) / ((long long)st.K * st.h.nchunk)));
    const int part_gx = (int)std::max<long long>(1, std::min<long long>((st.h.n_train + 1023) / 1024, (1024 + st.K - 1) / st.K));
    const int upd_gx = (int)std::max<long long>(1, std::min<long long>((st.h.n_train + 255) / 256, (2048 + st.K - 1) / st.K));
    const size_t upd_lds = (size_t)(3 * st.NL + (st.NL & 1)) * 4 + (size_t)st.NL * 8;

    explicit LeafwiseGrower(FitState& st_) : st(st_), s(st_.s) {
        idx0.alloc((size_t)st.K * st.h.n_train); idx1.alloc((size_t)st.K * st.h.n_train);
        pool.alloc((size_t)st.K * st.NL * st.h.tc.totbins);
        state.alloc(st.K); leaves.alloc((size_t)st.K * st.NL); cand.alloc((size_t)st.K * 2 * st.F);
        upd.alloc((size_t)st.K * st.NL); sorted.alloc((size_t)st.K * st.NL * 3);
        if (st.h.lds_hist > 64 * 1024)
            rgh::once_per_device(st.tab.device, rgh::ONCE_HIST_LDS, [] { HIPCHK(hipFuncSetAttribute((const void*)rg::k_hist, hipFuncAttributeMaxDynamicSharedMemorySize, 160 * 1024)); });
        if (st.h.lds_hist > 160 * 1024) throw std::invalid_argument("histogram working set exceeds LDS");
    }
    void enqueue_iteration(int it) {
        using namespace rg;
        const TreeOut to = st.trees.out();
        const uint8_t* usedp = st.used.p + (size_t)it * st.K * st.F;
        hipLaunchKernelGGL(k_init_iter, dim3(st.K), dim3(64), 0, s, state.p, leaves.p, pool.p, to, st.n_in_ptr, it, st.h.tc);
        for (int step = 0; step < st.NL - 1; ++step) {
            st.timers.timed(step == 0, [&]() {
                hipLaunchKernelGGL(k_hist, dim3(hist_gx, st.K, st.h.nchunk), dim3(256), st.h.lds_hist, s, st.bins.rec.p, st.gh.p, idx0.p, idx1.p, st.base.p,
                                   state.p, pool.p, st.bins.fmeta.p, st.bins.cmeta.p, st.fxs.p, st.h.tc);
            });
            hipLaunchKernelGGL(k_split_find, dim3((st.F + 3) / 4, st.K), dim3(256), 0, s, pool.p, state.p, leaves.p, st.bins.fmeta.p, usedp, cand.p, st.fxs.p, st.h.tc);
            hipLaunchKernelGGL(k_tree_step, dim3(st.K), dim3(64), 0, s, state.p, leaves.p, cand.p, pool.p, st.bins.fmeta.p, to, it, st.h.tc);
            hipLaunchKernelGGL(k_partition, dim3(part_gx, st.K), dim3(256), 0, s, reinterpret_cast<const uint8_t*>(st.bins.rec.p), idx0.p, idx1.p, st.base.p, state.p, st.h.tc);
            hipLaunchKernelGGL(k_finish_split, dim3(st.K), dim3(64), 0, s, state.p, leaves.p, to, it, st.h.tc);
        }
        hipLaunchKernelGGL(k_finalize_tree, dim3(st.K), dim3(64), 0, s, state.p, leaves.p, to, st.init.p, upd.p, sorted.p, st.trees.any.p, it, st.h.tc);
        hipLaunchKernelGGL(k_score_update, dim3(upd_gx, st.K), dim3(256), upd_lds, s, state.p, leaves.p, sorted.p, upd.p, idx0.p, idx1.p, st.base.p, st.score.p, st.n_in_ptr, st.h.tc);
        if (st.use_bagging)
            hipLaunchKernelGGL(k_score_update_oob, dim3(upd_gx, st.K), dim3(256), 0, s, reinterpret_cast<const uint8_t*>(st.bins.rec.p), st.bag.oob.p, st.bag.bagcnt.p,
                               state.p, to, st.bins.fmeta.p, upd.p, st.score.p, it, st.h.tc);
    }
};

void FitState::enqueue_grad(uint8_t* node0, long long NS) {
    using namespace rg;
    if (p.objective == 0) hipLaunchKernelGGL(k_grad<0>, dim3(grad_gx()), dim3(256), 0, s, score.p, d_ycol, yv.p, cw.p, sw_rows.p, bag.inbag.p, gh.p, node0, NS, qpart.p, d_mult, h.tc);
    else if (mc_rows())
        hipLaunchKernelGGL(k_grad_mc_rows<256>, dim3((unsigned)((N + 255) / 256)), dim3(256), (size_t)K * 256 * 8, s, score.p, d_ycol, cw.p, sw_rows.p, bag.inbag.p, gh.p, node0, NS, qpart.p, d_mult, h.tc);
    else if (mc_tile())
        hipLaunchKernelGGL(k_grad_mc, dim3((unsigned)((N + 63) / 64)), dim3(256), (size_t)(K * 64 + 320) * 8, s, score.p, d_ycol, cw.p, sw_rows.p, bag.inbag.p, gh.p, node0, NS, qpart.p, d_mult, h.tc);
    else if (p.objective == 1) hipLaunchKernelGGL(k_grad<1>, dim3(grad_gx()), dim3(256), 0, s, score.p, d_ycol, yv.p, cw.p, sw_rows.p, bag.inbag.p, gh.p, node0, NS, (unsigned long long*)nullptr, d_mult, h.tc);
    else hipLaunchKernelGGL(k_grad<2>, dim3(grad_gx()), dim3(256), 0, s, score.p, d_ycol, yv.p, cw.p, sw_rows.p, bag.inbag.p, gh.p, node0, NS, qpart.p, d_mult, h.tc);
    if (fx_fused) {
        const long long total = fx_parts * K * 2;
        const unsigned gx = (unsigned)std::max<long long>(1, std::min<long long>(256, (total + 8191) / 8192));
        hipLaunchKernelGGL(k_fx_reduce, dim3(gx), dim3(256), (size_t)K * 2 * 8, s, qpart.p, fx_parts, 2 * K, fxq.p);
    } else {
        const unsigned gx = (unsigned)std::max<long long>(1, std::min<long long>(128, (N + 4095) / 4096));
        hipLaunchKernelGGL(k_fx_measure, dim3(gx, K), dim3(256), 0, s, gh.p, (long long)N, (long long)h.tc.NG, h.tc.fx, fxq.p, d_mult);
    }
    if (dp) all_reduce(fxq.p, (size_t)K * 2, AR_I64, s);
    if (!level_mode) hipLaunchKernelGGL(k_fx_scale, dim3(1), dim3(256), 0, s, fxq.p, K, h.tc.fx, fxs.p);
}
void FitState::enqueue_bagging() {
    using namespace rg;
    hipLaunchKernelGGL(k_bagging, dim3((unsigned)((bag.nrb + 63) / 64)), dim3(64), 0, s, bag.rand.p, bag.local, p.bagging_fraction, bag.sorted_rows.p, bag.inbag.p, bag.bagcnt.p,
                       bag.off, (long long)h.n_train);
    hipLaunchKernelGGL(k_bag_lists, dim3((unsigned)((std::max<long long>(bag.local, 1) + 255) / 256)), dim3(256), 0, s, bag.sorted_rows.p, bag.local, bag.inbag.p, base.p, bag.oob.p, bag.bagcnt.p);
    if (dp) {
        hipLaunchKernelGGL(k_copy_i32, dim3(1), dim3(256), 0, s, reinterpret_cast<const int32_t*>(bag.bagcnt.p), reinterpret_cast<int32_t*>(bagcnt_g.p), 2ll);
        all_reduce(bagcnt_g.p, 2, AR_U32, s);
    }
}

rgbm_model* train_core(const rgbm_table& tab, int32_t target_col, const int32_t* feat_cols, int32_t F,
                       const double* y_value, const double* class_weight, const double* sample_weight_host,
                       const HostLabelStats* hls, const rgbm_params& p, rgbm_train_stats* stats, bool view_stats = false) {
    using namespace rg;
    check_fit_args(tab, target_col, feat_cols, F, y_value, p);
    if (F > 65535) throw std::invalid_argument("more than 65535 feature columns");
    StreamGuard sg_; hipStream_t s = sg_.s;
    rgh::Event ev_begin, ev_end;
    HIPCHK(hipEventRecord(ev_begin.e, s));

    FitState st(tab, target_col, F, p, stats != nullptr, s);
    auto now = []() { return std::chrono::duration<double, std::milli>(std::chrono::steady_clock::now().time_since_epoch()).count(); };
    const double t_start = now();
    st.bins.count_codes(tab, target_col, feat_cols, F, st.h, s);
    if (st.dp) {
        if (comm_kind() == 0) throw std::invalid_argument("row-sharded training requested but this thread has no communicator (rgbm_comm_init)");
        all_reduce(st.bins.cnt.p, st.bins.cnt.n, AR_U32, s);
    }
    st.bins.download_counts(st.h, s);
    if (st.dp) stream_sync_watchdog(s); else HIPCHK(hipStreamSynchronize(s));
    fit_setup(tab, y_value, class_weight, hls, p, F, st.h);
    if (p.objective == 2) y_value = st.h.yv32.data();
    const int n_y = st.h.ncod[F];

    const double t_bins = now();
    st.bins.fill(st.h, st.N, s);
    if (tab.has_mult && (!st.level_mode || st.h.nchunk > 2 || (F % 16) == 0 || sample_weight_host || st.use_bagging))
        throw std::invalid_argument("a table with row multiplicities trains with the level grower (1 <= max_depth <= 7), at most 32 features of which the last 16-feature "
                                    "chunk holds at most 15, without bagging and without per-row weights");
    st.bins.pack(tab, s);
    if (st.dp && (!st.level_mode || sample_weight_host))
        throw std::invalid_argument("row-sharded training supports the level grower (1 <= max_depth <= 7) without per-row weights");
    st.counter.alloc(1); st.counter.zero(s);
    if (!st.level_mode || st.use_bagging) {
        st.base.alloc(st.h.n_train);
        hipLaunchKernelGGL(k_iota_train, dim3((unsigned)((st.N + 255) / 256)), dim3(256), 0, s, st.d_ycol, (long long)st.N, st.base.p, st.counter.p);
    }
    if (st.level_mode) st.h.tc.NG = (st.N + 255) & ~255ll;
    st.gh.alloc((size_t)st.K * st.h.tc.NG); st.gh.zero(s);
    st.score.alloc((size_t)st.K * st.N); st.init.alloc(st.K);
    st.init.upload(st.h.init.data(), st.K, s);
    st.fxq.alloc((size_t)st.K * 2); st.fxq.zero(s);
    st.fxs.alloc(st.K);
    hipLaunchKernelGGL(k_init_score, dim3((unsigned)((st.N + 255) / 256)), dim3(256), 0, s, st.score.p, (long long)st.N, st.K, st.init.p);
    const size_t NT = (size_t)st.NE * st.K;
    st.trees.alloc(NT, st.NL, st.NE, s);
    std::unique_ptr<LevelGrower> lg; std::unique_ptr<LeafwiseGrower> lw;
    if (st.level_mode) lg.reset(new LevelGrower(st)); else lw.reset(new LeafwiseGrower(st));
    if (class_weight) { st.cw.alloc(n_y); st.cw.upload(class_weight, n_y, s); }
    if (y_value) { st.yv.alloc(n_y); st.yv.upload(y_value, n_y, s); }
    if (sample_weight_host) { st.sw_rows.alloc(st.N); st.sw_rows.upload(sample_weight_host, st.N, s); }

    const std::vector<uint8_t> used = make_used_masks(p, NT, F, st.h.trivial);
    st.used.alloc(used.size()); st.used.upload(used.data(), used.size(), s);

// ... 874 lines not shown
        HIPCHK(hipMemcpy(table, codes.p, (size_t)n * c * sizeof(int32_t), hipMemcpyDeviceToHost));
        return RGBM_OK;
    });
}

RGBM_EXPORT int rgbm_table_set_row_multiplicity(rgbm_table* t, const uint8_t* mult) {
    if (!t) return fail(RGBM_ERR_ARG, "rgbm_table_set_row_multiplicity: bad argument");
    return guarded([&]() {
        use_device(t->device);
        rgh::ViewWrite view_wr(t);
        if (!mult) { t->has_mult = false; t->mult_total = 0; return RGBM_OK; }
        int64_t tot = 0;
        for (int64_t i = 0; i < t->n; ++i) { if (mult[i] == 0) throw std::invalid_argument("rgbm_table_set_row_multiplicity: a multiplicity of 0"); tot += mult[i]; }
        if (tot >= (1ll << 31) - 4096) throw std::invalid_argument("rgbm_table_set_row_multiplicity: the expanded table has more than 2^31 rows");
        StreamGuard sg;
        t->mult.alloc((size_t)t->n);
        t->mult.upload(mult, (size_t)t->n, sg.s);
        HIPCHK(hipStreamSynchronize(sg.s));
        t->has_mult = true; t->mult_total = tot;
        return RGBM_OK;
    });
}

RGBM_EXPORT int rgbm_table_repair_chain(rgbm_table* t, const rgbm_model* const* models, int32_t T, const int32_t* target_col,
                                        const int32_t* feat_cols, const int32_t* feat_off, int64_t row_begin, int64_t n_rows,
                                        int32_t* out_label, double* out_prob) {
    if (!t || !models || T < 0 || !target_col || !feat_cols || !feat_off || row_begin < 0 || n_rows < 0 || row_begin + n_rows > t->n)
        return fail(RGBM_ERR_ARG, "rgbm_table_repair_chain: bad argument");
    if (n_rows == 0 || T == 0) return RGBM_OK;
    return guarded([&]() {
        use_device(t->device);
        rgh::ViewWrite view_wr(t);
        StreamGuard sg;
        return chain_device(const_cast<rgbm_model* const*>(models), T, target_col, feat_cols, feat_off, nullptr, nullptr, t->codes.p, t->n, row_begin, n_rows,
                            t->device, sg.s, out_label, out_prob);
    });
}

RGBM_EXPORT int rgbm_model_save(const rgbm_model* m, void* buf, size_t* len) {
    if (!m || !len) return fail(RGBM_ERR_ARG, "rgbm_model_save: bad argument");
    return guarded([&]() {
        const size_t need = serialised_size(*m);
        if (!buf) { *len = need; return RGBM_OK; }
        if (*len < need) { *len = need; return fail(RGBM_ERR_ARG, "rgbm_model_save: buffer too small"); }
        serialise_into(*m, (uint8_t*)buf); *len = need;
        return RGBM_OK;
    });
}

RGBM_EXPORT int rgbm_model_load(const void* buf, size_t len, rgbm_model** out) {
    if (!buf || !out) return fail(RGBM_ERR_ARG, "rgbm_model_load: bad argument");
    return guarded([&]() {
        const uint8_t* p = (const uint8_t*)buf; const uint8_t* end = p + len;
        auto need = [&](size_t n) { if ((size_t)(end - p) < n) throw std::length_error("truncated model"); };
        try {
            need(28); int32_t hdr[7]; memcpy(hdr, p, 28); p += 28;
            if (hdr[0] != 0x4D424752 || (hdr[1] != 1 && hdr[1] != 2)) return fail(RGBM_ERR_FORMAT, "rgbm_model_load: bad magic/version");
            std::unique_ptr<rgbm_model> m(new rgbm_model());
            m->objective = hdr[2]; m->num_class = hdr[3]; m->K = hdr[4]; m->n_iter = hdr[5]; m->F = hdr[6];
            if (m->F < 0 || m->K < 1 || m->n_iter < 0 || m->F > 65535) return fail(RGBM_ERR_FORMAT, "rgbm_model_load: bad header");
            if (m->objective < 0 || m->objective > 2 || m->num_class < 1) return fail(RGBM_ERR_FORMAT, "rgbm_model_load: bad objective / num_class");
            if (m->objective == 1 ? m->K != m->num_class : m->K != 1) return fail(RGBM_ERR_FORMAT, "rgbm_model_load: class-tree count does not match the objective");
            if (m->objective == 0 && m->num_class != 2) return fail(RGBM_ERR_FORMAT, "rgbm_model_load: binary model with num_class != 2");
            if ((unsigned long long)m->n_iter * (unsigned long long)m->K > (unsigned long long)(end - p) / 16ull) return fail(RGBM_ERR_FORMAT, "rgbm_model_load: tree count exceeds the buffer");
            m->feats.resize(m->F);
            for (Feat& f : m->feats) {
                need(12); int32_t h3[3]; memcpy(h3, p, 12); p += 12;
                f.n_codes = h3[0]; f.V = h3[1]; f.has_nan = h3[2];
                if (f.V < 0 || f.V > 255) return fail(RGBM_ERR_FORMAT, "rgbm_model_load: bad bin count");
                need(4 * (size_t)f.V); f.ub.resize(f.V); memcpy(f.ub.data(), p, 4 * (size_t)f.V); p += 4 * (size_t)f.V;
                if (hdr[1] == 2) {
                    need(4); int32_t nw; memcpy(&nw, p, 4); p += 4;
                    if (nw < 0 || (nw != 0 && (f.n_codes < 0 || nw != (f.n_codes + 31) / 32))) return fail(RGBM_ERR_FORMAT, "rgbm_model_load: bad unseen-category bitmap");
                    need(4 * (size_t)nw); f.unseen.resize(nw); memcpy(f.unseen.data(), p, 4 * (size_t)nw); p += 4 * (size_t)nw;
                }
            }
            m->trees.resize((size_t)m->n_iter * m->K);
            std::vector<uint8_t> refs;
            for (Tree& t : m->trees) {
                int32_t L_; need(4); memcpy(&L_, p, 4); p += 4;
                if (L_ < 1 || L_ > 32767) return fail(RGBM_ERR_FORMAT, "rgbm_model_load: bad leaf count");
                const size_t n = (size_t)L_ - 1;
                need(n * 28 + (size_t)L_ * 12);
                t.alloc(L_);
                auto rd32 = [&](int32_t* v, size_t k) { memcpy(v, p, 4 * k); p += 4 * k; };
                auto rd64 = [&](double* v, size_t k) { memcpy(v, p, 8 * k); p += 8 * k; };
                rd32(t.feat, n); rd32(t.theta, n); rd32(t.dleft, n); rd32(t.left, n); rd32(t.right, n); rd64(t.gain, n);
                rd64(t.leaf_value, t.L); rd32(t.leaf_count, t.L);
                for (size_t j = 0; j < n; ++j) {
                    if (t.feat[j] < 0 || t.feat[j] >= m->F) return fail(RGBM_ERR_FORMAT, "rgbm_model_load: node feature out of range");
                    if (t.theta[j] < -1 || t.theta[j] > 254) return fail(RGBM_ERR_FORMAT, "rgbm_model_load: node threshold out of range");
                    auto okc = [&](int ch) { return ch < 0 ? (~ch) < t.L : ch < (int)n && ch > (int)j; };
                    if (!okc(t.left[j]) || !okc(t.right[j])) return fail(RGBM_ERR_FORMAT, "rgbm_model_load: bad child link");
                }
                refs.assign(n + (size_t)t.L, 0);
                bool tree_ok = true;
                for (size_t j = 0; j < n; ++j)
                    for (int ch : {t.left[j], t.right[j]}) if (++refs[ch < 0 ? n + (size_t)(~ch) : (size_t)ch] > 1) tree_ok = false;
                for (size_t j = 1; j < refs.size(); ++j) if (refs[j] != 1) tree_ok = false;
                if (!tree_ok) return fail(RGBM_ERR_FORMAT, "rgbm_model_load: child links do not form a tree");
            }
            *out = m.release();
            return RGBM_OK;
        } catch (const std::length_error&) { return fail(RGBM_ERR_FORMAT, "rgbm_model_load: truncated buffer"); }
    });
}

RGBM_EXPORT int rgbm_table_repair_chain_gather(rgbm_table* t, const rgbm_model* const* models, int32_t T, const int32_t* target_col,
                                               const int32_t* feat_cols, const int32_t* feat_off, int64_t row_begin, int64_t n_rows, int64_t max_rows,
                                               int32_t* out_label, double* out_prob) {
    if (!t || !models || T < 1 || !target_col || !feat_cols || !feat_off || row_begin < 0 || n_rows < 0 || row_begin + n_rows > t->n || max_rows < n_rows || max_rows < 1 || !out_label || !out_prob)
        return fail(RGBM_ERR_ARG, "rgbm_table_repair_chain_gather: bad argument");
    return guarded([&]() {
        use_device(t->device);
        rgh::ViewWrite view_wr(t);
        const int nr = std::max(1, comm_nranks());
        StreamGuard sg; hipStream_t s = sg.s;
        const size_t blk = (size_t)T * (size_t)max_rows;
        DevBuf<int32_t> d_lab(blk), d_lab_all(blk * (size_t)nr); DevBuf<double> d_prob(blk), d_prob_all(blk * (size_t)nr);
        d_lab.zero(s); d_prob.zero(s);
        if (n_rows > 0)
            chain_device(const_cast<rgbm_model* const*>(models), T, target_col, feat_cols, feat_off, nullptr, nullptr, t->codes.p, t->n, row_begin, n_rows,
                         t->device, s, nullptr, nullptr, d_lab.p, d_prob.p, (long long)max_rows);
        const auto t0 = std::chrono::steady_clock::now();
        all_gather_on(d_lab.p, d_lab_all.p, blk * sizeof(int32_t), s);
        all_gather_on(d_prob.p, d_prob_all.p, blk * sizeof(double), s);
        HIPCHK(hipMemcpyAsync(out_label, d_lab_all.p, blk * (size_t)nr * sizeof(int32_t), hipMemcpyDeviceToHost, s));
        HIPCHK(hipMemcpyAsync(out_prob, d_prob_all.p, blk * (size_t)nr * sizeof(double), hipMemcpyDeviceToHost, s));
        stream_sync_watchdog(s);
        rgh::GatherStats& G = rgh::gather_stats();
        G.bytes += (long long)(blk * (size_t)nr * 12); G.calls += 2;
        G.ns += std::chrono::duration_cast<std::chrono::nanoseconds>(std::chrono::steady_clock::now() - t0).count();
        return RGBM_OK;
    });
}

RGBM_EXPORT void rgbm_model_free(rgbm_model* m) { delete m; }

RGBM_EXPORT int rgbm_model_info(const rgbm_model* m, int32_t* info) {
    if (!m || !info) return fail(RGBM_ERR_ARG, "rgbm_model_info: bad argument");
    info[0] = m->objective; info[1] = m->num_class; info[2] = m->K; info[3] = m->n_iter; info[4] = m->F;
    return RGBM_OK;
}

RGBM_EXPORT int rgbm_model_predict_form(const rgbm_model* m, int32_t* out) {
    if (!m || !out) return fail(RGBM_ERR_ARG, "rgbm_model_predict_form: bad argument");
    return guarded([&]() {
        const PredictForm pf = predict_form(m);
        out[0] = pf.form; out[1] = pf.mw; out[2] = pf.tw; out[3] = pf.tb; out[4] = (int32_t)pf.lds;
        return RGBM_OK;
    });
}

RGBM_EXPORT int rgbm_level_pass_plan(const int32_t* nbins, int32_t f, int64_t n_rows, int32_t k, int32_t max_depth, int32_t with_mult, double* out, int32_t out_len, int32_t* n_out) {
    if (!nbins || !out || !n_out || f < 1 || f > 255 || n_rows < 1 || k < 1 || max_depth < 1 || max_depth > rg::LV_MAX_DEPTH) return fail(RGBM_ERR_ARG, "rgbm_level_pass_plan: bad argument");
    return guarded([&]() {
        using namespace rg;
        const RunSwitches sw = read_switches();
        std::vector<FeatMeta> fmeta(f); std::vector<ChunkMeta> cmeta((f + 15) / 16);
        int totbins = 0;
        for (int j = 0; j < f; ++j) {
            if (nbins[j] < 1 || nbins[j] > 256) return fail(RGBM_ERR_ARG, "rgbm_level_pass_plan: a feature has 1..256 bins");
            FeatMeta& m = fmeta[j]; memset(&m, 0, sizeof(m)); m.nbins = nbins[j]; m.V = nbins[j]; m.hoff = totbins; totbins += nbins[j];
        }
        for (size_t ch = 0; ch < cmeta.size(); ++ch) {
            ChunkMeta& cm = cmeta[ch]; cm.first_feat = (int)ch * 16; cm.nfeat = std::min(16, f - (int)ch * 16); cm.fast_slots = 0; cm.wide_bins = 0;
            for (int j = 0; j < cm.nfeat; ++j) { fmeta[ch * 16 + j].wide_off = cm.wide_bins; cm.wide_bins += fmeta[ch * 16 + j].nbins; }
        }
        const LevelPassPlan P = plan_level_passes(sw, fmeta, cmeta, n_rows, k, max_depth, with_mult != 0, level_lds_bytes(sw));
        std::vector<double> v;
        const long long root_wg = (long long)P.root_gx * k * (long long)cmeta.size();
        v.insert(v.end(), {(double)P.root_gx, (double)P.part_items, 0.0, (double)root_wg, ROOT_PASS_COST.t_fix_us, (double)n_rows / P.root_gx * ROOT_PASS_COST.t_row_ns * 1e-3});
        int nl = 0;
        for (int level = 1; level < max_depth; ++level) for (const MtLaunch& L : P.mt[level]) {
            const PassCost& c = mt_pass_cost(L.acc2 != 0, L.rot != 0);
            v.insert(v.end(), {(double)level, (double)L.ch, (double)L.slot0, (double)L.nslots, (double)L.route, (double)L.T, (double)L.G, (double)L.gx, (double)L.acc2, (double)L.rot,
                               c.t_fix_us, (double)n_rows / L.gx * (c.t_row_ns + std::min(L.T, (int)k) * c.t_pair_ns) * 1e-3});
            ++nl;
        }
        v[2] = (double)nl;
        *n_out = (int32_t)v.size();
        if ((size_t)out_len < v.size()) return fail(RGBM_ERR_ARG, "rgbm_level_pass_plan: output too small");
        std::copy(v.begin(), v.end(), out);
        return RGBM_OK;
    });
}

RGBM_EXPORT int rgbm_model_importance(const rgbm_model* m, int32_t type, double* out) {
    if (!m || !out) return fail(RGBM_ERR_ARG, "rgbm_model_importance: bad argument");
    for (int f = 0; f < m->F; ++f) out[f] = 0.0;
    for (const Tree& t : m->trees) for (int j = 0; j < t.L - 1; ++j) out[t.feat[j]] += type == 0 ? 1.0 : t.gain[j];
    return RGBM_OK;
}

}
```

### spark-data-repair-plugin_amd/csrc/rgbm_level.h

```cpp
#pragma once
#include "rgbm_kernels.h"
#include "rgbm_small.h"

namespace rg {

constexpr int LV_INACTIVE = 255;
constexpr int LV_MAX_EXP = 64;
constexpr int LV_MAX_BUILT = 32;
constexpr int LV_CNT_REP = 16;
constexpr int LV_THREADS = 1024;
constexpr int LV_TILE = 2 * LV_THREADS;
constexpr int LV_LDS_TOTAL = 160 * 1024;
constexpr int LV_LDS_BYTES = LV_LDS_TOTAL;
constexpr int LV_MAX_DEPTH = 7;
constexpr int LV_MAX_LEAVES = 128;

constexpr int MT_MAX_T = 64;
constexpr int MT_MAX_NODES = 128;
constexpr int MT_RT_BUDGET = 256;
constexpr int MT_MAX_RT = MT_RT_BUDGET + MT_MAX_T;
constexpr int MT_WT_ROWS = 256;
constexpr int MT_RING_PLAIN = 128;
constexpr int MT_RING_SPEC = 128;
__host__ __device__ constexpr int mt_ring(bool spec) { return spec ? MT_RING_SPEC : MT_RING_PLAIN; }
constexpr int MT_CNT_REP = 4;

constexpr int MT_THREADS_ACC2 = 768;
#ifndef MT_CONSUMERS_N
#define MT_CONSUMERS_N 4
#endif
constexpr int MT_CONSUMERS = MT_CONSUMERS_N;

struct SNode {
    long long Gq, Hq;
    double pmin;
    int32_t count, depth, parent, is_left;
    int32_t left, right;
    int32_t best_feature, searched;
    int32_t hslot, pad;
    Cand best;
};

struct LvPlan {
    int32_t n_nodes, lvl_first, lvl_end, n_exp, n_built, live_rows , pad1, pad2, pad3, done, error, child_first, n_hslots, pad4;
    long long n_in;
    uint8_t exp[LV_MAX_EXP];
    uint8_t built_is_left[LV_MAX_EXP];
    uint32_t route0[256];
    uint32_t route1[256];
};

struct MtLayout;
struct RootLayout;
struct LevelConst {
    const MtLayout* mt_lay;
    const RootLayout* root_lay;
    int32_t gx;
    int32_t max_built;
    int32_t nchunk, K, F, totbins, num_leaves, max_depth, min_data_in_leaf, lds_bytes;
    int32_t sib_local;
    int32_t xcd_blocks;
    int32_t mt_T, mt_G, mt_ch, mt_slot0, mt_nslots, mt_route;
    int32_t mt_sparse;
    uint32_t has_mult;
    long long N, NS, NG;
};

__device__ __forceinline__ uint32_t rec_byte(const uint4& r, int j) {
    uint32_t w = (j < 8) ? ((j < 4) ? r.x : r.y) : ((j < 12) ? r.z : r.w);
    return (w >> (8 * (j & 3))) & 0xFFu;
}

constexpr int LV_MAX_Q = 11;
__host__ __device__ inline int lv_shift(int nbins, int q) {
    int l = 0; while ((1 << l) < nbins) ++l;
    int s = q - l;
    return s < 0 ? 0 : (s > 5 ? 5 : s);
}

__host__ __device__ inline int lv_slots(const FeatMeta* fm, int nfeat, int q) {
    int t = 0;
    for (int j = 0; j < nfeat; ++j) t += fm[j].nbins << lv_shift(fm[j].nbins, q);
    return t;
}

__host__ __device__ constexpr int mt_rot_dummy(bool rot) { return rot ? 4 : 0; }
__host__ __device__ inline int mt_shift(int nbins, int q, bool rot) { return rot ? (q < 0 ? 0 : (q > 2 ? 2 : q)) : lv_shift(nbins, q); }
__host__ __device__ inline int mt_slots(const FeatMeta* fm, int nfeat, int q, bool rot) {
    int t = 0;
    for (int j = 0; j < nfeat; ++j) t += fm[j].nbins << mt_shift(fm[j].nbins, q, rot);
    return t;
}
__host__ __device__ constexpr int mt_max_q(bool rot) { return rot ? 2 : LV_MAX_Q; }

constexpr int LV_ROOT_FIXED = 256;
#if !defined(MT_SPARSE_DIV_N)
#define MT_SPARSE_DIV_N 16
#endif
constexpr long long MT_SPARSE_DIV = MT_SPARSE_DIV_N;
__host__ __device__ constexpr long long mt_fixed_bytes(int threads, bool acc2, bool spec = false, bool li = true ) {
    return ((!acc2 && !spec) ? (long long)MT_MAX_T * 8  : 0) + (long long)MT_MAX_T * 32 + MT_MAX_NODES + 16 + 512 + 256 + (long long)(MT_MAX_T + 2) * 8 + (long long)MT_MAX_RT * 8 + (long long)MT_MAX_NODES * MT_CNT_REP * 4 + (long long)MT_MAX_NODES * 8 +
           (long long)(threads / 64 - (spec ? MT_CONSUMERS : 0)) * mt_ring(spec) * ((acc2 ? 32 : 16) + 8 + (li ? 2 : 0)) + 256;
}
__host__ __device__ constexpr long long mt_hd(int threads, bool acc2, bool spec) { return ((LV_LDS_TOTAL - mt_fixed_bytes(threads, acc2, spec, false)) / 2) & ~15ll; }
__host__ __device__ constexpr long long mt_hist_bytes(long long lds_bytes, int threads, bool acc2, bool spec, bool li) {
    const long long fixed = mt_fixed_bytes(threads, acc2, spec, li), hd = mt_hd(threads, acc2, spec);
    const long long room_h = (long long)LV_LDS_TOTAL - fixed - hd;
    const long long x = hd < room_h ? hd : room_h;
    const long long a = lds_bytes - fixed;
    return a < 2 * x ? a : 2 * x;
}

constexpr int MT_LAY_Q = LV_MAX_Q + 1;
struct MtLayout {
    uint32_t q_spn[MT_MAX_NODES + 4];
    int32_t wide[32], hdelta[32];
    int32_t fb[MT_LAY_Q][32];
    int32_t sh[MT_LAY_Q][32];
    uint8_t bin_feat[32 * 256];
};
struct RootLayout { int32_t q, spn, pad0, pad1; int32_t sh[16], fbase[16]; };

inline void mt_layout_fill(MtLayout& L, const FeatMeta* fm, int nfeat, const FeatMeta* fm1 , int nfeat1, int wide_bins0,
                           bool rot, long long avail ) {
    memset(&L, 0, sizeof(L));
    const bool acc2 = fm1 != nullptr;
    auto spn_of = [&](int q) { return mt_slots(fm, nfeat, q, rot) + (acc2 ? mt_slots(fm1, nfeat1, q, rot) : 0) + mt_rot_dummy(rot); };
    for (int tot = 0; tot < MT_MAX_NODES + 4; ++tot) {
        int q = mt_max_q(rot);
        while (q > 0 && (long long)tot * spn_of(q) * 16 > avail) --q;
        L.q_spn[tot] = (uint32_t)q | (uint32_t)spn_of(q) << 8;
    }
    for (int q = 0; q < MT_LAY_Q; ++q) {
        int o = 0;
        for (int a = 0; a < (acc2 ? 2 : 1); ++a) {
            const FeatMeta* fa = a == 0 ? fm : fm1;
            const int na = a == 0 ? nfeat : nfeat1;
            for (int j = 0; j < 16; ++j) {
                int shj = 0, fbj = 0;
                if (j < na) { shj = mt_shift(fa[j].nbins, q, rot); fbj = o; o += fa[j].nbins << shj; }
                L.fb[q][a * 16 + j] = fbj; L.sh[q][a * 16 + j] = shj;
            }
        }
    }
    for (int q = 0; q < 32; ++q) L.wide[q] = 0x7FFFFFFF;
    for (int a = 0; a < (acc2 ? 2 : 1); ++a) {
        const FeatMeta* fa = a == 0 ? fm : fm1;
        const int na = a == 0 ? nfeat : nfeat1;
        for (int j = 0; j < na && j < 16; ++j) {
            const int wide = (a == 0 ? 0 : wide_bins0) + fa[j].wide_off;
            L.wide[a * 16 + j] = wide; L.hdelta[a * 16 + j] = fa[j].hoff - wide;
            for (int b = 0; b < fa[j].nbins && wide + b < 32 * 256; ++b) L.bin_feat[wide + b] = (uint8_t)(a * 16 + j);
        }
    }
}
inline void root_layout_fill(RootLayout& L, const FeatMeta* fm, int nfeat, int lds_bytes) {
    memset(&L, 0, sizeof(L));
    int q = LV_MAX_Q;
    while (q > 0 && (long long)lv_slots(fm, nfeat, q) * 16 + LV_ROOT_FIXED > lds_bytes) --q;
    L.q = q;
    for (int j = 0; j < 16 && j < nfeat; ++j) { L.sh[j] = lv_shift(fm[j].nbins, q); L.fbase[j] = L.spn; L.spn += fm[j].nbins << L.sh[j]; }
}

__global__ __launch_bounds__(64) void k_level_init(LvPlan* __restrict__ plan, SNode* __restrict__ nodes, int32_t* __restrict__ count,
                                                   const unsigned int* __restrict__ n_in_ptr, long long n_train,
                                                   unsigned long long* __restrict__ Q, FxGrid fx, FxScale* __restrict__ fxs,
                                                   int32_t* __restrict__ itp , LevelConst c) {
    const int k = blockIdx.x, lane = lane_id();
    if (k == 0 && lane == 0) itp[0] += 1;
    if (lane == 0) {
        const int e_g = fx_tree_exponent(Q[2 * k], fx.q_mult, fx.c_g, fx.e_g_min, fx.e_g_max);
        const int e_h = fx_tree_exponent(Q[2 * k + 1], fx.q_mult, fx.c_h, fx.e_h_min, fx.e_h_max);
        FxScale f; f.sg = fx_pow2(e_g); f.sh = fx_pow2(e_h); f.inv_sg = fx_pow2(-e_g); f.inv_sh = fx_pow2(-e_h);
        fxs[k] = f;
        Q[2 * k] = 0ull; Q[2 * k + 1] = 0ull;
    }
    LvPlan* pp = &plan[k];
    const long long n_in = n_in_ptr ? (long long)n_in_ptr[0] : n_train;
    for (int i = lane; i < 256; i += 64) { pp->route0[i] = 0; pp->route1[i] = 0xFFFFFFFFu; count[(long long)k * 256 + i] = 0; }
    if (lane == 0) {
        pp->n_nodes = 1; pp->lvl_first = 0; pp->lvl_end = 1; pp->n_exp = 0; pp->n_built = 1;
        pp->error = 0; pp->child_first = 1; pp->n_hslots = 1; pp->n_in = n_in;
        pp->done = (n_in < (long long)c.min_data_in_leaf * 2) ? 1 : 0;
        SNode r; memset(&r, 0, sizeof(r));
        r.count = (int)n_in; r.depth = 0; r.parent = -1; r.left = -1; r.right = -1; r.best_feature = -1; r.searched = 0; r.hslot = 0;
        r.best.gain = -INFINITY; r.pmin = -INFINITY;
        nodes[(long long)k * 256] = r;
    }
}

__global__ __launch_bounds__(LV_THREADS, 1) void k_level_root(const uint4* __restrict__ rec, const float2* __restrict__ gh, const uint8_t* __restrict__ node,
                                                              const LvPlan* __restrict__ plan, HistBin* __restrict__ part,
                                                              const FeatMeta* __restrict__ fmeta, const ChunkMeta* __restrict__ cmeta,
                                                              const FxScale* __restrict__ fxs , LevelConst c) {
    extern __shared__ __attribute__((aligned(16))) unsigned char smem[];
    int k, bx, nbx;
    if (c.xcd_blocks) { const unsigned id = blockIdx.x, r = id >> 3; k = (int)(r % (unsigned)c.K); bx = (int)(r / (unsigned)c.K) * 8 + (int)(id & 7u); nbx = c.gx; }
    else { k = blockIdx.y; bx = blockIdx.x; nbx = gridDim.x; }
    const int ch = blockIdx.z;
    if (plan[k].done) return;
    const double sg_k = fxs[k].sg, sh_k = fxs[k].sh;
    const ChunkMeta cm = cmeta[ch];
    const FeatMeta* fm = fmeta + cm.first_feat;
    const int tid = threadIdx.x, lane = tid & 63, nfeat = cm.nfeat;
    const RootLayout* lay = c.root_lay + ch;
    int sh[16], fbase[16];
    const int spn = lay->spn;
#pragma unroll
    for (int j = 0; j < 16; ++j) { sh[j] = lay->sh[j]; fbase[j] = lay->fbase[j]; }
    unsigned long long* hist_g = reinterpret_cast<unsigned long long*>(smem);
    unsigned long long* hist_h = hist_g + spn;
    for (int i = tid; i < spn; i += LV_THREADS) reinterpret_cast<uint4*>(smem)[i] = make_uint4(0u, 0u, 0u, 0u);
    int cj[16], sh3[16];
#pragma unroll
    for (int j = 0; j < 16; ++j) { sh3[j] = sh[j] + 3; cj[j] = (fbase[j] + (lane & ((1 << sh[j]) - 1))) * 8; }
    const int hdelta = spn;
    __syncthreads();

    const long long N = c.N;
    const uint8_t* node_in = node + (long long)k * c.NS;
    const uint4* recc = rec + (long long)ch * N;
    const float2* ghk = gh + (long long)k * c.NG;
    const long long ntiles_all = (N + LV_TILE - 1) / LV_TILE;
    const long long tbeg = c.xcd_blocks ? ntiles_all * bx / nbx : bx;
    const long long ntiles = c.xcd_blocks ? ntiles_all * (bx + 1) / nbx : ntiles_all;
    const long long tstep = c.xcd_blocks ? 1 : nbx;

    constexpr int RPT = LV_TILE / LV_THREADS;
    int cur_n[RPT], nxt_n[RPT]; uint4 cur_r[RPT], nxt_r[RPT]; float2 cur_g[RPT], nxt_g[RPT];
    auto fetch = [&](long long t, int (&fn)[RPT], uint4 (&fr)[RPT], float2 (&fg)[RPT]) __attribute__((always_inline)) {
        const bool tv = t < ntiles;
        const long long pb = tv ? t * LV_TILE : 0;
        const long long left_rows = N - pb;
        const unsigned lim = (unsigned)(left_rows < LV_TILE ? left_rows : LV_TILE) - 1u;
#pragma unroll
        for (int q = 0; q < RPT; ++q) {
            const unsigned o = (unsigned)(q * LV_THREADS + tid);
            const unsigned oc = o < lim ? o : lim;
            typedef float v2f __attribute__((ext_vector_type(2)));
            const int nv = (int)__builtin_nontemporal_load(node_in + pb + oc);
            fr[q] = (recc + pb)[oc];
            const v2f gv = __builtin_nontemporal_load(reinterpret_cast<const v2f*>(ghk + pb + oc));
            fg[q] = make_float2(gv.x, gv.y);
            fn[q] = (tv && o <= lim) ? nv : LV_INACTIVE;
        }
    };
    auto accumulate = [&](bool on, const uint4& r, const float2& g) __attribute__((always_inline)) {
        if (on && (g.x != 0.0f || g.y != 0.0f)) {
            unsigned long long gq = (unsigned long long)fx_from_f32(g.x, sg_k), hq = (unsigned long long)fx_from_f32(g.y, sh_k);
            if (c.has_mult) { const unsigned long long m = r.w >> 24; gq *= m; hq *= m; }
            unsigned char* hb = reinterpret_cast<unsigned char*>(hist_g);
            const uint32_t w[4] = {r.x, r.y, r.z, r.w};
#define LV_ATOM(j) { const uint32_t code_ = (w[(j) >> 2] >> (8 * ((j) & 3))) & 0xFFu; \
                     unsigned long long* p_ = reinterpret_cast<unsigned long long*>(hb + cj[j] + (int)(code_ << sh3[j])); \
                     atomicAdd(p_, gq); atomicAdd(p_ + hdelta, hq); }
#pragma unroll
            for (int j = 0; j < 16; ++j) if (j < nfeat) LV_ATOM(j);
#undef LV_ATOM
        }
    };
    long long t = tbeg;
    fetch(t, cur_n, cur_r, cur_g);
    while (t < ntiles) {
        fetch(t + tstep, nxt_n, nxt_r, nxt_g);
#pragma unroll
        for (int q = 0; q < RPT; ++q) accumulate(cur_n[q] != LV_INACTIVE, cur_r[q], cur_g[q]);
        t += tstep; if (t >= ntiles) break;
        fetch(t + tstep, cur_n, cur_r, cur_g);
#pragma unroll
        for (int q = 0; q < RPT; ++q) accumulate(nxt_n[q] != LV_INACTIVE, nxt_r[q], nxt_g[q]);
        t += tstep;
    }
    __syncthreads();
    HistBin* dst = part + (((long long)k * c.gx + bx) * c.max_built) * c.totbins;
    for (int j = 0; j < nfeat; ++j) {
        const int shj = lay->sh[j], fb = lay->fbase[j];
        for (int b = tid; b < fm[j].nbins; b += LV_THREADS) {
            long long tg = 0, th = 0;
            const unsigned long long* sg_ = hist_g + fb + (b << shj); const unsigned long long* sh_ = hist_h + fb + (b << shj);
            for (int r2 = 0; r2 < (1 << shj); ++r2) { tg += (long long)sg_[r2]; th += (long long)sh_[r2]; }
            HistBin o; o.g = tg; o.h = th;
            dst[fm[j].hoff + b] = o;
        }
    }
}

struct MtTree { int32_t base, nlev, rt_off, slot0, nb, live, child_first, k; };

template <int NCHR , bool BAG,
          bool ROUTE ,
          int THREADS , bool ACC2 ,
          bool SPEC ,
          bool ROTP = false >
__global__ __launch_bounds__(THREADS, 1) void k_level_mt(const uint4* __restrict__ rec, const float2* __restrict__ gh, uint8_t* __restrict__ node ,
                                                         const uint8_t* __restrict__ inbag, const LvPlan* __restrict__ plan, HistBin* __restrict__ part,
                                                         int32_t* __restrict__ count, const FeatMeta* __restrict__ fmeta, const ChunkMeta* __restrict__ cmeta,
                                                         int32_t* __restrict__ err_flag,
                                                         const FxScale* __restrict__ fxs , LevelConst c) {
    static_assert(!ACC2 || NCHR == 2, "a two-chunk pass keeps both records in registers");
    static_assert(ACC2 == SPEC && THREADS == (ACC2 ? MT_THREADS_ACC2 : LV_THREADS) && (!ROTP || NCHR == 1 || ACC2) && (NCHR == 0 || NCHR == 1 || NCHR == 2),
                  "k_level_mt: not one of the six launch forms");
    constexpr int WAVES = THREADS / 64;
    constexpr int NCONS = SPEC ? MT_CONSUMERS : 0, NPROD = WAVES - NCONS;
    constexpr int NACC = ACC2 ? 2 : 1;
    constexpr int NRINGS = SPEC ? NPROD : WAVES;
    constexpr int MT_RING = mt_ring(SPEC);
    constexpr bool ROT = ROTP;
    constexpr bool SPARSE = (NCHR == 1) && !ACC2 && !SPEC;
    extern __shared__ __attribute__((aligned(16))) unsigned char smem[];
    const unsigned id = blockIdx.x;
    const int xl = (int)(id & 7u), bslot = (int)(id >> 3);
    const int grp = bslot % c.mt_G, rb = (bslot / c.mt_G) * 8 + xl;
    const int k0 = grp * c.mt_T;
    const int nk = (c.K - k0) < c.mt_T ? (c.K - k0) : c.mt_T;
    const int tid = threadIdx.x, lane = tid & 63, wave = tid >> 6;
    const int ch = ACC2 ? 0 : c.mt_ch;
    constexpr bool route = ROUTE;
    const ChunkMeta cm = cmeta[ch];
    const ChunkMeta cm1 = cmeta[ACC2 ? 1 : ch];
    const int nfeat = cm.nfeat, nfeat1 = ACC2 ? cm1.nfeat : 0;
    const int wb = cm.wide_bins + (ACC2 ? cm1.wide_bins : 0);
    const bool li_in_rec = (ACC2 ? nfeat1 : nfeat) <= 15 && !c.has_mult;

    MtTree* ti = reinterpret_cast<MtTree*>(smem);
    uint8_t* nd_tree = smem + MT_MAX_T * 32;
    int32_t* scal = reinterpret_cast<int32_t*>(nd_tree + MT_MAX_NODES);
    int32_t* ftab = scal + 4;
    uint32_t* rsync = reinterpret_cast<uint32_t*>(ftab + 128);
#define RS_LOAD(i) __hip_atomic_load(rsync + (i), __ATOMIC_RELAXED, __HIP_MEMORY_SCOPE_WORKGROUP)
#define RS_STORE(i, v) __hip_atomic_store(rsync + (i), (uint32_t)(v), __ATOMIC_RELAXED, __HIP_MEMORY_SCOPE_WORKGROUP)
    uint2* tpk = reinterpret_cast<uint2*>(ftab + 128 + 64);
    uint2* rt = tpk + MT_MAX_T + 2;
    int32_t* cnt = reinterpret_cast<int32_t*>(rt + MT_MAX_RT);
    uint2* nd_sc = reinterpret_cast<uint2*>(cnt + MT_MAX_NODES * MT_CNT_REP);
    uint4* ring_rec_all = reinterpret_cast<uint4*>(nd_sc + MT_MAX_NODES);
    uint4* ring_rec1_all = ring_rec_all + (ACC2 ? NRINGS * MT_RING : 0);
    uint2* ring_gh_all = reinterpret_cast<uint2*>(ring_rec1_all + NRINGS * MT_RING);
    uint16_t* ring_li_all = reinterpret_cast<uint16_t*>(ring_gh_all + NRINGS * MT_RING);
    size_t off = reinterpret_cast<unsigned char*>(ring_li_all + (li_in_rec ? 0 : NRINGS * MT_RING)) - smem;
    off = (off + 15) & ~(size_t)15;
    unsigned long long* xmask = reinterpret_cast<unsigned long long*>(smem + off);
    if (!ACC2 && !SPEC) off += (size_t)MT_MAX_T * 8;
    unsigned long long* hist_g = reinterpret_cast<unsigned long long*>(smem + off);
    constexpr int MT_HD = (int)mt_hd(THREADS, ACC2, SPEC);
    const long long avail = mt_hist_bytes(c.lds_bytes, THREADS, ACC2, SPEC, !li_in_rec);
    if (tid == 0 && ((long long)off > mt_fixed_bytes(THREADS, ACC2, SPEC, !li_in_rec) || (long long)off + MT_HD + avail / 2 > (long long)LV_LDS_TOTAL)) atomicOr(err_flag, 2);

    const MtLayout* __restrict__ lay = c.mt_lay;
    if (tid < 64) {
        const uint32_t qs0 = lay->q_spn[lane], qs1 = lay->q_spn[64 + lane], qs2 = lay->q_spn[128 + (lane & 3)];
        MtTree t; t.base = 0; t.nlev = 0; t.nb = 0; t.live = 0; t.child_first = 0; t.k = k0 + lane; t.slot0 = 0; t.rt_off = 0;
        if (lane < nk) {
            const LvPlan* pp = &plan[k0 + lane];
            const bool live = !pp->done && pp->n_exp > 0;
            t.live = live ? 1 : 0;
            t.child_first = pp->child_first;
            t.base = live ? (route ? (int)pp->exp[0] : pp->child_first) : 0;
            t.nlev = live ? (route ? pp->child_first - (int)pp->exp[0] : 2 * pp->n_exp) : 0;
            int nb = live ? pp->n_built - c.mt_slot0 : 0;
            if (nb > c.mt_nslots) nb = c.mt_nslots;
            t.nb = nb < 0 ? 0 : nb;
        }
        bool sparse_t = false;
        if (SPARSE && lane < nk && t.live && t.nlev <= 64) {
            const LvPlan* pp = &plan[k0 + lane];
            const long long lr = route ? (long long)pp->live_rows : 0ll;
            sparse_t = route && lr * MT_SPARSE_DIV < pp->n_in && c.mt_sparse != 0;
        }
        const int ntab = lane < nk ? (route ? (t.live ? t.child_first : 0) : t.nlev) + 1 : 0;
        int inc_nb = t.nb, inc_rt = ntab;
#pragma unroll
        for (int o = 1; o < 64; o <<= 1) { const int a = __shfl_up(inc_nb, o), b2 = __shfl_up(inc_rt, o); if (lane >= o) { inc_nb += a; inc_rt += b2; } }
        t.slot0 = inc_nb - t.nb; t.rt_off = inc_rt - ntab;
        const int total = __shfl(inc_nb, 63), rt_total = __shfl(inc_rt, 63);
        const unsigned long long livem = __ballot(t.live != 0);
        const bool ok = total <= MT_MAX_NODES && rt_total <= MT_MAX_RT;
        if (!ok) { t.live = 0; t.nb = 0; t.nlev = 0; if (lane == 0) atomicOr(err_flag, 2); }
        const bool dead_t = lane < nk && (!t.live || (!route && t.nb == 0));
        const unsigned long long dmask = __ballot(lane < nk && !sparse_t && !dead_t), smask = __ballot(lane < nk && sparse_t && !dead_t), zmask = __ballot(dead_t);
        const int nkd_ = __popcll(dmask), nks_ = __popcll(smask);
        const unsigned long long below = (1ull << lane) - 1ull;
        const int pos = lane >= nk ? lane : (dead_t ? nkd_ + nks_ + __popcll(zmask & below) : (sparse_t ? nkd_ + __popcll(smask & below) : __popcll(dmask & below)));
        if (lane < nk) ti[pos] = t;
        tpk[pos] = make_uint2((uint32_t)t.base | (uint32_t)t.nlev << 8 | (uint32_t)(ntab > 0 ? ntab - 1 : 0) << 17 | (t.live && lane < nk ? 1u << 31 : 0u), (uint32_t)t.rt_off | (uint32_t)t.k << 16);
        if (lane < 2) tpk[64 + lane] = make_uint2(0u, 0u);
        if (SPARSE) xmask[lane] = 0ull;
        const int tot = ok ? total : 0;
        const uint32_t qs = (uint32_t)__shfl((int)(tot < 64 ? qs0 : (tot < 128 ? qs1 : qs2)), tot & 63);
        if (lane == 0) {
            const int s = (int)(qs & 0xFFu), spn0 = (int)(qs >> 8);
            if ((long long)tot * spn0 * 16 > avail) atomicOr(err_flag, 2);
            scal[0] = tot; scal[1] = s; scal[2] = spn0; scal[3] = ((ok && livem != 0ull) ? 1 : 0) | nkd_ << 8 | (nkd_ + nks_) << 16;
        }
    }
    __syncthreads();
    if (!(scal[3] & 1)) return;
    const int total = __builtin_amdgcn_readfirstlane(scal[0]), s = __builtin_amdgcn_readfirstlane(scal[1]), spn = __builtin_amdgcn_readfirstlane(scal[2]);
    if (!route && total == 0) return;
    const int nkd = __builtin_amdgcn_readfirstlane((scal[3] >> 8) & 0xFF), nke = __builtin_amdgcn_readfirstlane((scal[3] >> 16) & 0xFF);
    for (int kk = __builtin_amdgcn_readfirstlane(wave); kk < nk; kk += WAVES) {
        const MtTree t = ti[kk];
        const LvPlan* pp = &plan[t.k];
        const int ntab_k = (route ? (t.live ? t.child_first : 0) : t.nlev) + 1;
        for (int i = lane; i < ntab_k; i += 64) {
            const int n = route ? i : t.base + i;
            uint2 e;
            if (route) {
                const bool cur = i < ntab_k - 1 && n >= t.base;
                const uint32_t w0 = cur ? pp->route0[n] : 0u; const uint32_t w1 = cur ? pp->route1[n] : 0u;
                if (w0 & (1u << 24)) {
                    const int ls = (int)((w1 >> 16) & 0xFFu) - c.mt_slot0, rs = (int)(w1 >> 24) - c.mt_slot0;
                    const bool lb = ((w1 >> 16) & 0xFFu) != 0xFFu && ls >= 0 && ls < t.nb, rbb = (w1 >> 24) != 0xFFu && rs >= 0 && rs < t.nb;
                    const uint32_t theta1 = (w0 >> 8) & 0xFFu, nanbin = (w0 >> 16) & 0xFFu, dleft = (w0 >> 25) & 1u;
                    uint32_t offb, thr;
                    if (nanbin != 255u && dleft) { offb = nanbin; thr = (theta1 - 1u - nanbin) & 0xFFu; }
                    else if (theta1 == 0u) { offb = 255u; thr = 0u; }
                    else { offb = 0u; thr = theta1 - 1u; }
                    const uint32_t f = w0 & 0xFFu;
                    e = make_uint2((NCHR == 0 ? f : (f & 7u) | ((f >> 4) & 1u) << 30 | ((f >> 3) & 1u) << 31) | thr << 8 | offb << 16 | 1u << 24,
                                   (w1 & 0xFFu) | (lb ? (uint32_t)(t.slot0 + ls) : 0xFFu) << 8 | ((w1 >> 8) & 0xFFu) << 16 | (rbb ? (uint32_t)(t.slot0 + rs) : 0xFFu) << 24);
                    if (SPARSE && kk >= nkd && kk < nke && n - t.base < 64) atomicOr(&xmask[kk], 1ull << (n - t.base));
                } else {
                    const uint32_t self = i < ntab_k - 1 ? (uint32_t)n : (uint32_t)LV_INACTIVE;
                    e = make_uint2(0u, self | 0xFF00u | self << 16 | 0xFF000000u);
                }
            } else {
                const int ei = i >> 1, ls = ei - c.mt_slot0;
                const bool mine = i < ntab_k - 1 && (pp->built_is_left[ei] ? 0 : 1) == (i & 1) && ls >= 0 && ls < t.nb;
                e = make_uint2(mine ? 1u : 0u, mine ? (uint32_t)(t.slot0 + ls) : 0xFFu);
            }
            rt[t.rt_off + i] = e;
        }
        const uint2 sc_k = make_uint2((uint32_t)__double2hiint(fxs[t.k].sg), (uint32_t)__double2hiint(fxs[t.k].sh));
        for (int i = lane; i < t.nb; i += 64) { nd_tree[t.slot0 + i] = (uint8_t)kk; nd_sc[t.slot0 + i] = sc_k; }
    }
    for (int i = tid; i < total * MT_CNT_REP; i += THREADS) cnt[i] = 0;
    if (tid < 48) rsync[tid] = 0u;
    unsigned long long* hist_h = hist_g + MT_HD / 8;
    {
        uint4* zg = reinterpret_cast<uint4*>(hist_g); uint4* zh = reinterpret_cast<uint4*>(hist_h);
        const int n16 = (total * spn + 1) >> 1;
        for (int i = tid; i < n16; i += THREADS) { zg[i] = make_uint4(0u, 0u, 0u, 0u); zh[i] = make_uint4(0u, 0u, 0u, 0u); }
    }
    unsigned long long sh3p[NACC];
    int cj[NACC][16];
    {
        const int32_t* __restrict__ fb_s = lay->fb[s]; const int32_t* __restrict__ sh_s = lay->sh[s];
#pragma unroll
        for (int a = 0; a < NACC; ++a) {
            unsigned long long pk = 0ull;
#pragma unroll
            for (int j = 0; j < 16; ++j) {
                const int shj = sh_s[a * 16 + j], fb = fb_s[a * 16 + j];
                pk |= (unsigned long long)(shj + 3) << (4 * j); cj[a][j] = (fb + (lane & ((1 << shj) - 1))) * 8;
            }
            sh3p[a] = (unsigned long long)(unsigned)__builtin_amdgcn_readfirstlane((int)(unsigned)pk) |
                      (unsigned long long)(unsigned)__builtin_amdgcn_readfirstlane((int)(unsigned)(pk >> 32)) << 32;
        }
        if (tid < 128) { const int q = tid & 31, r = tid >> 5; ftab[tid] = r == 0 ? lay->wide[q] : (r == 1 ? fb_s[q] : (r == 2 ? sh_s[q] : lay->hdelta[q])); }
        if (tid == 0) { const unsigned long long la = (unsigned long long)reinterpret_cast<uintptr_t>(lay->bin_feat); rsync[48] = (uint32_t)la; rsync[49] = (uint32_t)(la >> 32); }
    }
    constexpr int hdelta = MT_HD / 8;
    __syncthreads();
    uint32_t rmask[NACC][4];
    const int rot_sh = mt_shift(1, s, ROT) + 3;
    if (ROT) {
        const int r16 = lane & 15, c4 = lane >> 4;
        const int spn_valid = spn - mt_rot_dummy(ROT);
#pragma unroll
        for (int a = 0; a < NACC; ++a) {
            const int na = a == 0 ? nfeat : nfeat1;
#pragma unroll
            for (int w = 0; w < 4; ++w) rmask[a][w] = 0u;
#pragma unroll
            for (int j = 0; j < 16; ++j) {
                const int f = (j + r16) & 15;
                const bool fv = f < na;
                cj[a][j] = fv ? (ftab[32 + a * 16 + f] + (c4 & ((1 << (rot_sh - 3)) - 1))) * 8 : (spn_valid + c4) * 8;
                rmask[a][j >> 2] |= fv ? (0xFFu << (8 * (j & 3))) : 0u;
            }
        }
    }

    const int my_ring = __builtin_amdgcn_readfirstlane(wave < NRINGS ? wave : 0);
    uint4* ring_rec = ring_rec_all + my_ring * MT_RING;
    uint4* ring_rec1 = ring_rec1_all + my_ring * MT_RING;
    uint2* ring_gh = ring_gh_all + my_ring * MT_RING;
    uint16_t* ring_li = ring_li_all + my_ring * MT_RING;
    int r_head = 0, r_cnt = 0;
    const unsigned long long lane_lt = (1ull << lane) - 1ull;
    const unsigned spn8 = (unsigned)spn * 8u;
    const uint2 tpk_v = tpk[lane];
    auto tree_entry = [&](int kk) __attribute__((always_inline)) -> uint2 {
        const int kc = kk < 64 ? kk : 63;
        const uint32_t x = (uint32_t)__builtin_amdgcn_readlane((int)tpk_v.x, kc), y = (uint32_t)__builtin_amdgcn_readlane((int)tpk_v.y, kc);
        return kk < nkd ? make_uint2(x, y) : make_uint2(0u, 0u);
    };

    auto run_batch_of = [&](int rid, int head, int nb) __attribute__((always_inline)) {
// ... 413 lines not shown
}

__global__ __launch_bounds__(256) void k_level_marginal(const HistBin* __restrict__ red_j , HistBin* __restrict__ red, const LvPlan* __restrict__ plan,
                                                        const int32_t* __restrict__ count, const JointFeat* __restrict__ jf, const int16_t* __restrict__ bin_feat ,
                                                        int vtotbins, LevelConst c) {
    const int k = blockIdx.y;
    if (blockIdx.x == 0)
        reinterpret_cast<long long*>(red + (long long)c.K * c.totbins)[(long long)k * 256 + threadIdx.x] = (long long)count[(long long)k * 256 + threadIdx.x];
    const int b = blockIdx.x * 256 + threadIdx.x;
    if (b >= c.totbins) return;
    HistBin acc; acc.g = 0; acc.h = 0;
    if (!plan[k].done) {
        const JointFeat f = jf[bin_feat[b]];
        const int digit = b - f.hoff;
        const int period = f.stride * f.nbins;
        const HistBin* src = red_j + (long long)k * vtotbins + f.voff;
        for (int base = digit * f.stride; base < f.nbv; base += period)
            for (int lo = 0; lo < f.stride; ++lo) { const HistBin v = src[base + lo]; acc.g += v.g; acc.h += v.h; }
    }
    red[(long long)k * c.totbins + b] = acc;
}

__global__ __launch_bounds__(256) void k_counts_unpack(const long long* __restrict__ cnt64, int32_t* __restrict__ count_g) {
    const long long i = (long long)blockIdx.x * 256 + threadIdx.x;
    count_g[i] = (int32_t)cnt64[i];
}

constexpr int LS_MAX_THREADS = 1024;
constexpr int LS_LDS_BUDGET = 64 * 1024;
__host__ __device__ inline size_t ls_lds_bytes(int totbins, int F, bool hist_lds) { return (hist_lds ? (size_t)2 * totbins * sizeof(HistBin) : 0) + (size_t)2 * F * sizeof(Cand); }
inline bool ls_hist_in_lds(int totbins, int F) { return ls_lds_bytes(totbins, F, true) + 1024 <= (size_t)LS_LDS_BUDGET; }

template <bool ROOT>
__global__ __launch_bounds__(LS_MAX_THREADS) void k_level_step(const HistBin* __restrict__ part, HistBin* __restrict__ pool, const LvPlan* __restrict__ plan,
                                                               SNode* __restrict__ nodes, int32_t* __restrict__ count, int32_t* __restrict__ count_local,
                                                               const FeatMeta* __restrict__ fmeta, const uint8_t* __restrict__ used_all ,
                                                               const ScanLane* __restrict__ scan_map , int scan_waves, int hist_lds,
                                                               unsigned long long* __restrict__ stat_rows, const int32_t* __restrict__ itp ,
                                                               int n_hnodes, const FxScale* __restrict__ fxs, TrainConst c_model, LevelConst lc) {
    extern __shared__ __attribute__((aligned(16))) unsigned char smem[];
    const int k = blockIdx.y, pi = blockIdx.x;
    const LvPlan* pp = &plan[k];
    if (pp->done) return;
    if (!ROOT && pi >= pp->n_exp) return;
    const int T = blockDim.x, tid = threadIdx.x, lane = tid & 63, wv = tid >> 6, nwaves = T >> 6;
    const int tb = lc.totbins, F = lc.F;
    const int l = ROOT ? 0 : pp->child_first + 2 * pi, r = ROOT ? 0 : l + 1;
    const bool bl = ROOT ? true : pp->built_is_left[pi] != 0;
    const long long n_in = pp->n_in;
    SNode* nk = nodes + (long long)k * 256;
    int nl = ROOT ? 0 : count[(long long)k * 256 + l], nr = ROOT ? 0 : count[(long long)k * 256 + r];
    const int hs_l = ROOT ? 0 : nk[l].hslot, hs_r = ROOT ? 0 : nk[r].hslot;
    const int p = ROOT ? 0 : (int)pp->exp[pi];
    long long P_Gq = 0, P_Hq = 0, P_lGq = 0, P_lHq = 0; int P_count = 0, P_hslot = 0;
    if (!ROOT) { const SNode& P = nk[p]; P_Gq = P.Gq; P_Hq = P.Hq; P_lGq = P.best.left_gq; P_lHq = P.best.left_hq; P_count = P.count; P_hslot = P.hslot; }
    const TrainConst c = tree_const(c_model, fxs, k);
    const uint8_t* used_k = used_all + ((long long)(*itp) * lc.K + k) * F;
    HistBin* pk = pool + (long long)k * n_hnodes * tb;
    HistBin* gL = pk + (long long)hs_l * tb; HistBin* gR = pk + (long long)hs_r * tb;
    HistBin* hL = hist_lds ? reinterpret_cast<HistBin*>(smem) : gL;
    HistBin* hR = hist_lds ? reinterpret_cast<HistBin*>(smem) + tb : gR;
    Cand* ck = reinterpret_cast<Cand*>(smem + (hist_lds ? (size_t)2 * tb * sizeof(HistBin) : 0));
    HistBin* hbuilt = bl ? hL : hR; HistBin* hsib = bl ? hR : hL;

    {
        const int bslot = ROOT ? 0 : pi;
        const HistBin* src = part + (((long long)k * lc.gx) * lc.max_built + bslot) * tb;
        const long long xs = (long long)lc.max_built * tb;
        const int nbl = tb >= T ? T : ((tb + 63) & ~63);
        int PL = hist_lds ? T / nbl : 1;
        if (PL > lc.gx) PL = lc.gx;
        if (PL > 1) {
            for (int b = tid; b < tb; b += T) { HistBin z; z.g = 0; z.h = 0; hbuilt[b] = z; }
            __syncthreads();
            const int b = tid % nbl, xl = tid / nbl;
            if (b < tb && xl < PL) {
                long long ag = 0, ah = 0;
#pragma unroll 8
                for (int x = xl; x < lc.gx; x += PL) { const HistBin v = src[x * xs + b]; ag += v.g; ah += v.h; }
                atomicAdd(reinterpret_cast<unsigned long long*>(&hbuilt[b].g), (unsigned long long)ag);
                atomicAdd(reinterpret_cast<unsigned long long*>(&hbuilt[b].h), (unsigned long long)ah);
            }
        } else {
            for (int b = tid; b < tb; b += T) {
                long long ag = 0, ah = 0;
#pragma unroll 8
                for (int x = 0; x < lc.gx; ++x) { const HistBin v = src[x * xs + b]; ag += v.g; ah += v.h; }
                HistBin o; o.g = ag; o.h = ah; hbuilt[b] = o;
            }
        }
        __syncthreads();
    }
    if (ROOT) {
        if (hist_lds) for (int b = tid; b < tb; b += T) gL[b] = hL[b];
    } else {
        const HistBin* hp = pk + (long long)P_hslot * tb;
        HistBin* gbuilt = bl ? gL : gR; HistBin* gsib = bl ? gR : gL;
        for (int b = tid; b < tb; b += T) {
            const HistBin bu = hbuilt[b], par = hp[b];
            HistBin sb; sb.g = par.g - bu.g; sb.h = par.h - bu.h;
            hsib[b] = sb;
            if (hist_lds) { gbuilt[b] = bu; gsib[b] = sb; }
        }
    }
    bool go = true;
    if (!ROOT) {
        const int nb = bl ? nl : nr, ns = P_count - nb;
        if (bl) nr = ns; else nl = ns;
        go = !(nr < c.min_data_in_leaf * 2 && nl < c.min_data_in_leaf * 2);
        if (tid == 0) {
            const int sib = bl ? r : l;
            count[(long long)k * 256 + sib] = ns;
            if (lc.sib_local && count_local != count) count_local[(long long)k * 256 + sib] = ns;
            nk[l].count = nl; nk[l].searched = go ? 1 : 0;
            nk[r].count = nr; nk[r].searched = go ? 1 : 0;
            atomicAdd(stat_rows, (unsigned long long)nb);
        }
    }
    __syncthreads();
    const int nch = ROOT ? 1 : 2;
    if (go) {
        for (int ws = wv; ws < nch * scan_waves; ws += nwaves) {
            const int child = ws / scan_waves, slot = ws - child * scan_waves;
            const ScanLane sl = scan_map[slot * 64 + lane];
            if (ROOT) {
                const FeatMeta f0 = fmeta[0];
                long long sg_ = 0, sh_ = 0;
#pragma unroll
                for (int j = 0; j < 4; ++j) { const int b = lane * 4 + j; if (b < f0.nbins) { const HistBin v = hL[f0.hoff + b]; sg_ += v.g; sh_ += v.h; } }
#pragma unroll
                for (int o = 32; o >= 1; o >>= 1) { sg_ += __shfl_xor(sg_, o); sh_ += __shfl_xor(sh_, o); }
                if (ws == 0 && lane == 0) { nk[0].Gq = sg_; nk[0].Hq = sh_; nk[0].searched = 1; atomicAdd(stat_rows, (unsigned long long)n_in); }
                scan_child_packed(hL, fmeta, sl, sg_, sh_, n_in, c, used_k, ck);
            } else if (child == 0) scan_child_packed(hL, fmeta, sl, P_lGq, P_lHq, (long long)nl, c, used_k, ck);
            else scan_child_packed(hR, fmeta, sl, P_Gq - P_lGq, P_Hq - P_lHq, (long long)nr, c, used_k, ck + F);
        }
    }
    __syncthreads();
    if (wv < nch) {
        const int n = ROOT ? 0 : (wv == 0 ? l : r);
        const Cand* cf = ck + wv * F;
        double bg = -INFINITY; int bf = -1;
        if (go) for (int f = lane; f < F; f += 64) { const double g = cf[f].gain; if (g > -INFINITY && leaf_better(g, f, 0, bg, bf, 0)) { bg = g; bf = f; } }
#pragma unroll
        for (int o = 32; o >= 1; o >>= 1) { const double g2 = __shfl_xor(bg, o); const int f2 = __shfl_xor(bf, o); if (leaf_better(g2, f2, 0, bg, bf, 0)) { bg = g2; bf = f2; } }
        if (lane == 0) {
            if (bf >= 0) { nk[n].best = cf[bf]; nk[n].best_feature = bf; } else { nk[n].best.gain = -INFINITY; nk[n].best_feature = -1; }
        }
    }
}

__global__ __launch_bounds__(64) void k_level_plan(LvPlan* __restrict__ plan, SNode* __restrict__ nodes, const FeatMeta* __restrict__ fmeta,
                                                   int level, TrainConst c, LevelConst lc) {
    __shared__ double pm[256];
    const int k = blockIdx.x, lane = lane_id();
    LvPlan* pp = &plan[k];
    if (pp->done) return;
    SNode* nk = nodes + (long long)k * 256;
    const int first = pp->lvl_first, end = pp->lvl_end, nlev = end - first;
    for (int n = lane; n < first; n += 64) pm[n] = nk[n].pmin;
    __syncthreads();
    if (lane < nlev) {
        const int n = first + lane;
        const double g = nk[n].best.gain;
        const int par = nk[n].parent;
        double v = g;
        if (par >= 0) { const double pv = pm[par]; v = (pv < g) ? pv : g; }
        if (!(g > -INFINITY)) v = -INFINITY;
        pm[n] = v; nk[n].pmin = v;
    }
    __syncthreads();
    bool expand = false;
    if (lane < nlev) {
        const double v = pm[first + lane];
        if (v > 0.0) {
            int rank = 0;
            for (int y = 0; y < end; ++y) rank += (pm[y] > v) ? 1 : 0;
            expand = rank < c.num_leaves - 1;
        }
    }
    const unsigned long long em = __ballot(expand);
    const int n_exp = __popcll(em);
    for (int i = lane; i < 256; i += 64) { pp->route0[i] = 0; pp->route1[i] = 0xFFFFFFFFu; }
    __syncthreads();
    if (n_exp == 0) { if (lane == 0) { pp->done = 1; pp->n_exp = 0; pp->n_built = 0; } return; }
    const int child_first = pp->n_nodes;
    const bool with_hist = level < c.max_depth;
    const int hs0 = pp->n_hslots;
    if (expand) {
        const int ei = __popcll(em & ((1ull << lane) - 1ull));
        const int n = first + lane;
        const SNode P = nk[n];
        const int l = child_first + 2 * ei, r = l + 1;
        const int f = P.best_feature;
        const bool built_left = P.best.left_hq * 2 <= P.Hq;
        nk[n].left = l; nk[n].right = r;
        SNode L; memset(&L, 0, sizeof(L));
        L.depth = P.depth + 1; L.parent = n; L.left = -1; L.right = -1; L.best_feature = -1; L.searched = 0; L.best.gain = -INFINITY; L.pmin = -INFINITY;
        SNode R = L;
        L.is_left = 1; L.Gq = P.best.left_gq; L.Hq = P.best.left_hq; L.hslot = with_hist ? hs0 + 2 * ei : -1;
        R.is_left = 0; R.Gq = P.Gq - P.best.left_gq; R.Hq = P.Hq - P.best.left_hq; R.hslot = with_hist ? hs0 + 2 * ei + 1 : -1;
        nk[l] = L; nk[r] = R;
        pp->exp[ei] = (uint8_t)n; pp->built_is_left[ei] = built_left ? 1 : 0;
        const int nanbin = fmeta[f].has_nan ? fmeta[f].V : 255;
        pp->route0[n] = (uint32_t)f | ((uint32_t)(P.best.theta + 1) & 0xFFu) << 8 | (uint32_t)nanbin << 16 | 1u << 24 | (uint32_t)(P.best.dleft ? 1 : 0) << 25;
        const uint32_t ls = with_hist && built_left ? (uint32_t)ei : 0xFFu, rs = with_hist && !built_left ? (uint32_t)ei : 0xFFu;
        pp->route1[n] = (uint32_t)l | (uint32_t)r << 8 | ls << 16 | rs << 24;
    }
    const int n_built = with_hist ? n_exp : 0;
    long long live = expand ? (long long)nk[first + lane].count : 0ll;
#pragma unroll
    for (int o = 32; o >= 1; o >>= 1) live += __shfl_xor(live, o);
    if (lane == 0) {
        pp->live_rows = (int32_t)(live > 0x7FFFFFFFll ? 0x7FFFFFFFll : live);
        pp->n_exp = n_exp; pp->n_built = n_built;
        pp->child_first = child_first; pp->n_nodes = child_first + 2 * n_exp;
        pp->lvl_first = child_first; pp->lvl_end = child_first + 2 * n_exp;
        if (with_hist) pp->n_hslots = hs0 + 2 * n_exp;
    }
}

__global__ __launch_bounds__(64) void k_level_replay(LvPlan* __restrict__ plan, const SNode* __restrict__ nodes, const int32_t* __restrict__ count,
                                                     TreeOut out, const double* __restrict__ init, double* __restrict__ node_delta ,
                                                     int32_t* __restrict__ leaf_node_out ,
                                                     int32_t* __restrict__ any_split, int32_t* __restrict__ err_flag, const int32_t* __restrict__ itp, TrainConst c) {
    const int it = *itp;
    __shared__ int leaf_parent[LV_MAX_LEAVES], leaf_isleft[LV_MAX_LEAVES];
    __shared__ int node_leaf[256];
    __shared__ double upd[LV_MAX_LEAVES];
    const int k = blockIdx.x, lane = lane_id();
    LvPlan* pp = &plan[k];
    const SNode* nk = nodes + (long long)k * 256;
    const long long tbase = (long long)it * c.K + k;
    const long long nb = tbase * (c.num_leaves - 1);
    double* lv = out.leaf_value + tbase * c.num_leaves;
    const int n_nodes = pp->n_nodes;
    __shared__ double s_gain[256], s_lout[256], s_rout[256], s_lv[LV_MAX_LEAVES];
    __shared__ int s_feat[256], s_theta[256];
    __shared__ short s_left[256], s_right[256], s_parent[256];
    __shared__ unsigned char s_dleft[256];
    for (int n = lane; n < 256; n += 64) {
        node_leaf[n] = -1;
        if (n < n_nodes) {
            const SNode& sn = nk[n];
            const bool se = sn.searched != 0;
            s_gain[n] = se ? sn.best.gain : -INFINITY; s_feat[n] = se ? sn.best_feature : -1;
            s_theta[n] = sn.best.theta; s_dleft[n] = (unsigned char)(sn.best.dleft ? 1 : 0);
            s_lout[n] = sn.best.left_out; s_rout[n] = sn.best.right_out;
            s_left[n] = (short)sn.left; s_right[n] = (short)sn.right; s_parent[n] = (short)sn.parent;
        }
    }
    if (lane == 0) { leaf_parent[0] = -1; leaf_isleft[0] = 0; }
    __syncthreads();
    if (lane == 0) node_leaf[0] = 0;
    __syncthreads();
    static_assert(LV_MAX_LEAVES <= 128, "two leaves per lane");
    double lg[2] = {-INFINITY, -INFINITY}; int lf[2] = {-1, -1}, ln[2] = {0, 0};
    if (lane == 0) { lg[0] = s_gain[0]; lf[0] = s_feat[0]; }
    int L = 1;
    const int max_leaves = c.num_leaves < LV_MAX_LEAVES ? c.num_leaves : LV_MAX_LEAVES;
    while (L < max_leaves) {
        const bool up = leaf_better(lg[1], lf[1], lane + 64, lg[0], lf[0], lane);
        const double g = up ? lg[1] : lg[0]; const int f = up ? lf[1] : lf[0], l = up ? lane + 64 : lane, n = up ? ln[1] : ln[0];
        double m = g;
#pragma unroll
        for (int o = 32; o >= 1; o >>= 1) { const double m2 = __shfl_xor(m, o); m = m2 > m ? m2 : m; }
        if (!(m > 0.0)) break;
        unsigned long long tie = __ballot(g == m);
        int wl = __ffsll((long long)tie) - 1;
        if (tie & (tie - 1ull)) {
            const int fk = (g == m) ? (f < 0 ? 0x7FFFFFFF : f) : 0x7FFFFFFF;
            int fmin = fk;
#pragma unroll
            for (int o = 32; o >= 1; o >>= 1) { const int f2 = __shfl_xor(fmin, o); fmin = f2 < fmin ? f2 : fmin; }
            int lmin = (g == m && fk == fmin) ? l : 0x7FFFFFFF;
#pragma unroll
            for (int o = 32; o >= 1; o >>= 1) { const int l2 = __shfl_xor(lmin, o); lmin = l2 < lmin ? l2 : lmin; }
            wl = lmin & 63;
        }
        const int wpk = __shfl(n | (l >> 6) << 8, wl);
        const int sn = wpk & 0xFF, bl = wl + 64 * (wpk >> 8), bf = s_feat[sn];
        const int sl = s_left[sn], sr = s_right[sn];
        if (sl < 0) { if (lane == 0) { pp->error = 1; atomicOr(err_flag, 1); } break; }
        const int node = L - 1, right_leaf = L;
        if (lane == 0) {
            out.feat[nb + node] = bf; out.theta[nb + node] = s_theta[sn]; out.dleft[nb + node] = (int)s_dleft[sn]; out.gain[nb + node] = s_gain[sn];
            out.left[nb + node] = ~bl; out.right[nb + node] = ~right_leaf;
            const int pn = leaf_parent[bl];
            if (pn >= 0) { if (leaf_isleft[bl]) out.left[nb + pn] = node; else out.right[nb + pn] = node; }
            s_lv[bl] = s_lout[sn]; s_lv[right_leaf] = s_rout[sn];
            leaf_parent[bl] = node; leaf_isleft[bl] = 1; leaf_parent[right_leaf] = node; leaf_isleft[right_leaf] = 0;
            node_leaf[sl] = bl; node_leaf[sr] = right_leaf;
        }
        const double gl_ = s_gain[sl], gr_ = s_gain[sr]; const int fl_ = s_feat[sl], fr_ = s_feat[sr];
#pragma unroll
        for (int s2 = 0; s2 < 2; ++s2) {
            if (lane + 64 * s2 == bl) { lg[s2] = gl_; lf[s2] = fl_; ln[s2] = sl; }
            if (lane + 64 * s2 == right_leaf) { lg[s2] = gr_; lf[s2] = fr_; ln[s2] = sr; }
        }
        ++L;
    }
    __syncthreads();
    if (lane == 0) out.L[tbase] = L;
    if (lane < L) leaf_node_out[(long long)k * LV_MAX_LEAVES + lane] = ln[0];
    if (lane + 64 < L) leaf_node_out[(long long)k * LV_MAX_LEAVES + lane + 64] = ln[1];
    double* nd = node_delta + (long long)k * 256;
    if (L <= 1) {
        if (lane == 0) lv[0] = (it == 0) ? init[k] : 0.0;
        for (int i = lane; i < 256; i += 64) nd[i] = 0.0;
        return;
    }
    if (lane == 0) atomicOr(any_split + it, 1);
    for (int l = lane; l < L; l += 64) {
        double v = s_lv[l] * c.learning_rate;
        upd[l] = v;
        if (it == 0 && fabs(init[k]) > k_eps()) v += init[k];
        lv[l] = v;
    }
    __syncthreads();
    for (int n = lane; n < 256; n += 64) {
        double d = 0.0;
        if (n < n_nodes) {
            int a = n;
            while (a >= 0 && node_leaf[a] < 0) a = s_parent[a];
            if (a >= 0) d = upd[node_leaf[a]];
        }
        nd[n] = d;
    }
}


__device__ __forceinline__ int lv_final_route(int n, long long row, const uint4* __restrict__ rec, const uint8_t* __restrict__ inbag, const uint32_t* route0,
// ... 107 lines not shown
```

### spark-data-repair-plugin_amd/repair/_native.py

```python
import ctypes as C
import os

import numpy as np

_HERE = os.path.dirname(os.path.abspath(__file__))
LIB_PATH = os.path.join(_HERE, "..", "lib", "librepairgbm.so")


class RepairGbmError(RuntimeError):
    pass


class RgbmParams(C.Structure):
    _fields_ = [
        ("objective", C.c_int32), ("num_class", C.c_int32),
        ("n_estimators", C.c_int32), ("num_leaves", C.c_int32), ("max_depth", C.c_int32), ("max_bin", C.c_int32),
        ("min_data_in_leaf", C.c_int32), ("min_data_in_bin", C.c_int32), ("bagging_freq", C.c_int32), ("seed", C.c_int32),
        ("device_id", C.c_int32), ("reserved", C.c_int32),
        ("learning_rate", C.c_double), ("lambda_l1", C.c_double), ("lambda_l2", C.c_double), ("min_gain_to_split", C.c_double),
        ("min_sum_hessian_in_leaf", C.c_double), ("bagging_fraction", C.c_double), ("feature_fraction", C.c_double),
    ]


class RgbmTrainStats(C.Structure):
    _fields_ = [
        ("hist_ms", C.c_double), ("total_ms", C.c_double), ("hist_launches", C.c_int64), ("hist_rows", C.c_int64),
        ("hist_bytes", C.c_int64), ("root_rows", C.c_int64), ("root_ms", C.c_double), ("trees", C.c_int64),
        ("route_ms", C.c_double), ("route_launches", C.c_int64), ("root_atomics_per_row", C.c_int64), ("level_atomics_per_row", C.c_int64),
    ]

    def as_dict(self):
        return {k: getattr(self, k) for k, _ in self._fields_}


PARAM_DEFAULTS = dict(objective=1, num_class=2, n_estimators=300, num_leaves=31, max_depth=7, max_bin=255,
                      min_data_in_leaf=20, min_data_in_bin=3, bagging_freq=0, seed=42, device_id=0, reserved=0,
                      learning_rate=0.01, lambda_l1=0.0, lambda_l2=0.0, min_gain_to_split=0.0,
                      min_sum_hessian_in_leaf=1e-3, bagging_fraction=1.0, feature_fraction=1.0)


FLAG_ROW_SHARDED = 1
FLAG_NO_MODEL = 2
FLAG_WHOLE_TABLE = 4
VIEW_STATES = ("none", "built", "not worth it", "cannot")


def make_params(**kw):
    d = dict(PARAM_DEFAULTS)
    kw = dict(kw)
    if kw.pop("row_sharded", False):
        d["reserved"] = d.get("reserved", 0) | FLAG_ROW_SHARDED
    if kw.pop("whole_table", False):
        d["reserved"] = d.get("reserved", 0) | FLAG_WHOLE_TABLE
    if not kw.pop("want_model", True):
        d["reserved"] = d.get("reserved", 0) | FLAG_NO_MODEL
    for k, v in kw.items():
        if k not in d:
            raise TypeError("unknown parameter %r" % k)
        d[k] = v
    return RgbmParams(**d)


_lib = None


def lib():
    global _lib
    if _lib is None:
        path = os.path.abspath(os.environ.get("RGBM_LIB_PATH") or LIB_PATH)
        if not os.path.exists(path):
            raise RepairGbmError("librepairgbm.so is not built (%s); run `python __graft_entry__.py` or `make -C "
                                 "spark-data-repair-plugin_amd/csrc`" % path)
        l = C.CDLL(path)
        l.rgbm_last_error.restype = C.c_char_p
        for name in ("rgbm_device_count", "rgbm_version", "rgbm_release_cache", "rgbm_train", "rgbm_predict", "rgbm_repair_chain",
                     "rgbm_table_create", "rgbm_table_train", "rgbm_table_train_batch", "rgbm_table_repair_chain", "rgbm_table_read_column",
                     "rgbm_model_save", "rgbm_model_load", "rgbm_model_info", "rgbm_model_importance", "rgbm_model_predict_form",
                     "rgbm_comm_unique_id", "rgbm_comm_init", "rgbm_comm_finalize", "rgbm_comm_info", "rgbm_comm_count",
                     "rgbm_local_group_create", "rgbm_comm_init_local",
                     "rgbm_table_detect_nulls", "rgbm_table_detect_constraint", "rgbm_table_rows_of_cells", "rgbm_table_cells_fetch",
                     "rgbm_table_null_cells", "rgbm_table_gather_rows", "rgbm_table_count_codes", "rgbm_table_create_dict",
                     "rgbm_table_shape", "rgbm_table_repair_pmf", "rgbm_table_read_cells", "rgbm_table_repair_pmf_weighted",
                     "rgbm_edit_distance", "rgbm_table_pair_counts", "rgbm_table_cell_domains", "rgbm_table_fd_map", "rgbm_table_rule_fill",
                     "rgbm_nearest_values", "rgbm_table_detect_cells", "rgbm_table_distinct_rows",
                     "rgbm_table_read_row_multiplicity", "rgbm_table_detect_dc", "rgbm_table_detect_row_bits",
                     "rgbm_table_kmeans_assign", "rgbm_table_kmeans_read", "rgbm_lof_1d", "rgbm_table_column_stats"):
            getattr(l, name).restype = C.c_int
        for name in ("rgbm_table_distinct_view_info", "rgbm_distinct_view_eligible", "rgbm_level_pass_plan"):
            if hasattr(l, name):
                getattr(l, name).restype = C.c_int
        l.rgbm_local_group_free.restype = None
        l.rgbm_table_free.restype = None
        l.rgbm_model_free.restype = None
        l.rgbm_host_free.restype = None
        _lib = l
    return _lib


EXPORTED_SYMBOLS = [
    "rgbm_device_count", "rgbm_last_error", "rgbm_version", "rgbm_release_cache", "rgbm_train", "rgbm_predict", "rgbm_repair_chain",
    "rgbm_table_create", "rgbm_table_free", "rgbm_table_train", "rgbm_table_train_batch", "rgbm_table_repair_chain", "rgbm_table_read_column",
    "rgbm_model_save", "rgbm_model_load", "rgbm_model_free", "rgbm_model_info", "rgbm_model_importance",
    "rgbm_comm_unique_id", "rgbm_comm_init", "rgbm_comm_finalize", "rgbm_comm_info", "rgbm_comm_count",
    "rgbm_local_group_create", "rgbm_local_group_free", "rgbm_comm_init_local",
    "rgbm_comm_all_gather_sizes", "rgbm_comm_all_gather_bytes", "rgbm_table_repair_chain_gather", "rgbm_comm_gather_stats",
    "rgbm_fusion_create", "rgbm_fusion_join", "rgbm_fusion_leave", "rgbm_fusion_info", "rgbm_fusion_free",
    "rgbm_table_detect_nulls", "rgbm_table_detect_constraint", "rgbm_table_rows_of_cells", "rgbm_table_cells_fetch",
    "rgbm_table_null_cells", "rgbm_table_gather_rows", "rgbm_table_count_codes", "rgbm_table_create_dict", "rgbm_table_shape",
    "rgbm_table_repair_pmf", "rgbm_table_read_cells", "rgbm_table_write_cells", "rgbm_host_alloc", "rgbm_host_free",
    "rgbm_table_set_column_values", "rgbm_table_set_column_kind", "rgbm_table_set_row_multiplicity",
    "rgbm_table_repair_pmf_weighted", "rgbm_edit_distance", "rgbm_table_pair_counts", "rgbm_table_cell_domains",
    "rgbm_table_fd_map", "rgbm_table_rule_fill", "rgbm_nearest_values", "rgbm_table_detect_cells",
    "rgbm_table_distinct_rows", "rgbm_table_read_row_multiplicity", "rgbm_table_detect_dc", "rgbm_table_detect_row_bits", "rgbm_model_predict_form",
    "rgbm_table_kmeans_assign", "rgbm_table_kmeans_read", "rgbm_table_distinct_view_info", "rgbm_distinct_view_eligible",
    "rgbm_table_column_stats", "rgbm_level_pass_plan",
]
EXPORTED_SYMBOLS_WITH_DIGITS = ["rgbm_lof_1d"]

COMM_ID_BYTES = 128


def comm_unique_id():
    buf = (C.c_ubyte * COMM_ID_BYTES)()
    _check(lib().rgbm_comm_unique_id(buf), "rgbm_comm_unique_id")
    return bytes(buf)


def comm_init(uid, rank, nranks, device_id=0):
    buf = (C.c_ubyte * COMM_ID_BYTES).from_buffer_copy(bytes(uid))
    _check(lib().rgbm_comm_init(buf, C.c_int32(rank), C.c_int32(nranks), C.c_int32(device_id)), "rgbm_comm_init")


def comm_finalize():
    _check(lib().rgbm_comm_finalize(), "rgbm_comm_finalize")


def comm_info():
    a = np.zeros(3, np.int32)
    _check(lib().rgbm_comm_info(_p(a, C.c_int32)), "rgbm_comm_info")
    return dict(kind=int(a[0]), rank=int(a[1]), nranks=int(a[2]))


def model_trees(blob):
    import struct
    hdr = struct.unpack_from("7i", blob, 0)
    ver, K, n_iter, F = hdr[1], hdr[4], hdr[5], hdr[6]
    p = 28
    for _ in range(F):
        _, V, _ = struct.unpack_from("3i", blob, p); p += 12 + 4 * V
        if ver == 2:
            nw, = struct.unpack_from("i", blob, p); p += 4 + 4 * nw
    trees = []
    for _ in range(K * n_iter):
        L, = struct.unpack_from("i", blob, p); p += 4
        n = L - 1
        t = {}
        for name in ("feat", "theta", "dleft", "left", "right"):
            t[name] = np.frombuffer(blob, np.int32, n, p); p += 4 * n
        t["gain"] = np.frombuffer(blob, np.float64, n, p); p += 8 * n
        t["leaf_value"] = np.frombuffer(blob, np.float64, L, p); p += 8 * L
        t["leaf_count"] = np.frombuffer(blob, np.int32, L, p); p += 4 * L
        trees.append(t)
    return K, n_iter, trees


def needed_built_rows(blob, max_depth):
    _, _, trees = model_trees(blob)
    total = 0
    for tr in trees:
        n = len(tr["feat"])
        if n == 0:
            continue
        left, right, lc = tr["left"], tr["right"], tr["leaf_count"]
        cnt = np.zeros(n, np.int64)
        for j in range(n - 1, -1, -1):
            a, b = int(left[j]), int(right[j])
            cnt[j] = (cnt[a] if a >= 0 else int(lc[~a])) + (cnt[b] if b >= 0 else int(lc[~b]))
        depth = np.zeros(n, np.int32)
        for j in range(n):
            a, b = int(left[j]), int(right[j])
            if a >= 0:
                depth[a] = depth[j] + 1
            if b >= 0:
                depth[b] = depth[j] + 1
            if depth[j] + 1 < max_depth:
                ca = cnt[a] if a >= 0 else int(lc[~a]); cb = cnt[b] if b >= 0 else int(lc[~b])
                total += int(min(ca, cb))
    return total


def comm_count():
    n = C.c_int32(0)
    _check(lib().rgbm_comm_count(C.byref(n)), "rgbm_comm_count")
    return int(n.value)


def comm_all_gather_sizes(values):
    v = np.ascontiguousarray(values, np.int64).reshape(-1)
    out = np.zeros((max(1, comm_info()["nranks"]), v.size), np.int64)
    _check(lib().rgbm_comm_all_gather_sizes(_p(v, C.c_int64), C.c_int32(v.size), _p(out, C.c_int64)), "rgbm_comm_all_gather_sizes")
    return out


def comm_all_gather_bytes(payload):
    mine = np.frombuffer(bytes(payload), np.uint8) if not isinstance(payload, np.ndarray) else np.ascontiguousarray(payload).view(np.uint8).reshape(-1)
    sizes = comm_all_gather_sizes([mine.size])[:, 0]
    block = int(max(int(sizes.max()), 1))
    recv = np.zeros((len(sizes), block), np.uint8)
    _check(lib().rgbm_comm_all_gather_bytes(_p(mine, C.c_uint8) if mine.size else None, C.c_int64(mine.size), C.c_int64(block), _p(recv, C.c_uint8)),
           "rgbm_comm_all_gather_bytes")
    return [recv[r, :int(sizes[r])].copy() for r in range(len(sizes))]


def comm_gather_stats():
    a = np.zeros(3, np.int64)
    _check(lib().rgbm_comm_gather_stats(_p(a, C.c_int64)), "rgbm_comm_gather_stats")
    return dict(bytes=int(a[0]), seconds=float(a[1]) * 1e-9, collectives=int(a[2]))


class FusionGroup:

    def __init__(self, n_members):
        self.h = C.c_void_p()
        _check(lib().rgbm_fusion_create(C.c_int32(n_members), C.byref(self.h)), "rgbm_fusion_create")
        self.n_members = n_members

    class _Member:
        def __init__(self, group, j):
            self.group, self.j = group, j

        def __enter__(self):
            _check(lib().rgbm_fusion_join(self.group.h, C.c_int32(self.j)), "rgbm_fusion_join")
            return self

        def __exit__(self, et, ev, tb):
            lib().rgbm_fusion_leave(C.c_int32(0 if et is None else 1))
            return False

    def member(self, j):
        return FusionGroup._Member(self, j)

    def info(self):
        a = np.zeros(4, np.int64)
        _check(lib().rgbm_fusion_info(self.h, _p(a, C.c_int64)), "rgbm_fusion_info")
        return dict(collectives=int(a[0]), parts=int(a[1]), members_in=int(a[2]), broken=bool(a[3]))

    def close(self):
        if self.h:
            _check(lib().rgbm_fusion_free(self.h), "rgbm_fusion_free")
            self.h = C.c_void_p()


class LocalGroup:

    def __init__(self, nranks, device_id=0):
        self.h = C.c_void_p()
        _check(lib().rgbm_local_group_create(C.c_int32(nranks), C.c_int32(device_id), C.byref(self.h)), "rgbm_local_group_create")
        self.nranks = nranks

    def join(self, rank):
        _check(lib().rgbm_comm_init_local(self.h, C.c_int32(rank)), "rgbm_comm_init_local")

    def __del__(self):
        h, self.h = getattr(self, "h", None), None
        if h and _lib is not None:
            _lib.rgbm_local_group_free(h)


def _check(rc, what):
    if rc != 0:
        err = RepairGbmError("%s failed (%d): %s" % (what, rc, lib().rgbm_last_error().decode("utf-8", "replace")))
        err.code = rc
        raise err


def device_count():
    return int(lib().rgbm_device_count())


def release_cache():
    _check(lib().rgbm_release_cache(), "rgbm_release_cache")


def _p(a, t):
    return a.ctypes.data_as(C.POINTER(t)) if a is not None else None


def _i32(a):
    return None if a is None else np.ascontiguousarray(a, np.int32)


def _f64(a):
    return None if a is None else np.ascontiguousarray(a, np.float64)


class Model:

    def __init__(self, handle):
        self.h = handle

    def __del__(self):
        h, self.h = getattr(self, "h", None), None
        if h and _lib is not None:
            _lib.rgbm_model_free(h)

    def info(self):
        a = np.zeros(5, np.int32)
        _check(lib().rgbm_model_info(self.h, _p(a, C.c_int32)), "rgbm_model_info")
        return dict(objective=int(a[0]), num_class=int(a[1]), K=int(a[2]), n_iter=int(a[3]), F=int(a[4]))

    def save(self):
        n = C.c_size_t(0)
        _check(lib().rgbm_model_save(self.h, None, C.byref(n)), "rgbm_model_save")
        buf = bytearray(max(n.value, 1))
        _check(lib().rgbm_model_save(self.h, (C.c_char * len(buf)).from_buffer(buf), C.byref(n)), "rgbm_model_save")
        return bytes(buf[:n.value]) if n.value != len(buf) else bytes(buf)

    @staticmethod
    def load(b):
        h = C.c_void_p()
        arr = np.frombuffer(b, np.uint8)
        _check(lib().rgbm_model_load(arr.ctypes.data_as(C.c_void_p), C.c_size_t(len(b)), C.byref(h)), "rgbm_model_load")
        return Model(h)

    def importance(self, kind="gain"):
        out = np.zeros(self.info()["F"], np.float64)
        _check(lib().rgbm_model_importance(self.h, C.c_int32(0 if kind == "split" else 1), _p(out, C.c_double)), "rgbm_model_importance")
        return out

    def predict_form(self):
        a = np.zeros(5, np.int32)
        _check(lib().rgbm_model_predict_form(self.h, _p(a, C.c_int32)), "rgbm_model_predict_form")
        return dict(form=("fixed", "dynamic", "walk")[int(a[0])], MW=int(a[1]), TW=int(a[2]), tb=int(a[3]), lds=int(a[4]))

    def predict(self, X, device_id=0):
        X = _i32(X)
        F, n = X.shape
        inf = self.info()
        ncol = 1 if inf["objective"] == 2 else inf["num_class"]
        out = np.zeros((n, ncol), np.float64)
        _check(lib().rgbm_predict(self.h, _p(X, C.c_int32), C.c_int64(n), C.c_int32(F), C.c_int32(device_id), _p(out, C.c_double)), "rgbm_predict")
        return out


def train(X, n_codes, y_code, n_y_codes, y_value=None, class_weight=None, sample_weight=None, want_stats=False, **params):
    X = _i32(X)
    F, N = X.shape
    n_codes, y_code = _i32(n_codes), _i32(y_code)
    yv, cw, sw = _f64(y_value), _f64(class_weight), _f64(sample_weight)
    p = make_params(**params)
    h = C.c_void_p()
    st = RgbmTrainStats()
    _check(lib().rgbm_train(_p(X, C.c_int32), C.c_int64(N), C.c_int32(F), _p(n_codes, C.c_int32), _p(y_code, C.c_int32),
                            C.c_int32(n_y_codes), _p(yv, C.c_double), _p(cw, C.c_double), _p(sw, C.c_double),
                            C.byref(p), C.byref(h), C.byref(st) if want_stats else None), "rgbm_train")
    m = Model(h)
    return (m, st.as_dict()) if want_stats else m


class RgbmFitSpec(C.Structure):
    _fields_ = [("table", C.c_void_p), ("target_col", C.c_int32), ("n_features", C.c_int32), ("feat_cols", C.POINTER(C.c_int32)),
                ("y_value", C.POINTER(C.c_double)), ("class_weight", C.POINTER(C.c_double)), ("params", C.POINTER(RgbmParams)),
                ("valid_table", C.c_void_p), ("valid_label_out", C.POINTER(C.c_int32)), ("valid_value_out", C.POINTER(C.c_double))]


def level_pass_plan(nbins, rows, K, max_depth=7, with_mult=False):
    nb = _i32(nbins)
    out = np.zeros(6 + 12 * 4096, np.float64)
    n = C.c_int32(0)
    _check(lib().rgbm_level_pass_plan(_p(nb, C.c_int32), C.c_int32(len(nb)), C.c_int64(rows), C.c_int32(K), C.c_int32(max_depth), C.c_int32(1 if with_mult else 0),
                                      _p(out, C.c_double), C.c_int32(len(out)), C.byref(n)), "rgbm_level_pass_plan")
    keys = ("level", "ch", "slot0", "nslots", "route", "T", "G", "gx", "acc2", "rot")
    launches = []
    for i in range(int(out[2])):
        v = out[6 + 12 * i: 18 + 12 * i]
        launches.append(dict({k: int(x) for k, x in zip(keys, v)}, t_fix_us=float(v[10]), t_rows_us=float(v[11])))
    return dict(root_gx=int(out[0]), part_items=int(out[1]), root_workgroups=int(out[3]), root_t_fix_us=float(out[4]), root_t_rows_us=float(out[5]), launches=launches)


def distinct_view_eligible(rows, f, table_has_mult=False, min_rows=0, **params):
    p = make_params(**params)
    r = lib().rgbm_distinct_view_eligible(C.c_int64(rows), C.c_int32(f), C.byref(p), C.c_int32(1 if table_has_mult else 0), C.c_int64(min_rows))
    if r < 0:
        _check(r, "rgbm_distinct_view_eligible")
    return bool(r)


def train_batch(fits):
    n = len(fits)
    if n == 0:
        return []
    specs = (RgbmFitSpec * n)()
    keep = []
    for i, f in enumerate(fits):
        f = dict(f)
        tab = f.pop("table")
        fc = _i32(f.pop("feat_cols"))
        yv, cw = _f64(f.pop("y_value", None)), _f64(f.pop("class_weight", None))
        target = int(f.pop("target_col"))
        vtab = f.pop("valid_table", None)
        vlab = np.zeros(vtab.n, np.int32) if vtab is not None else None
        vval = np.zeros(vtab.n, np.float64) if vtab is not None else None
        f.setdefault("device_id", tab.device_id)
        p = make_params(**f)
        keep.append((tab, fc, yv, cw, p, vtab, vlab, vval))
        specs[i].valid_table = vtab.h if vtab is not None else None
        specs[i].valid_label_out = _p(vlab, C.c_int32)
        specs[i].valid_value_out = _p(vval, C.c_double)
        specs[i].table = tab.h
        specs[i].target_col = target
        specs[i].n_features = len(fc)
        specs[i].feat_cols = _p(fc, C.c_int32)
        specs[i].y_value = _p(yv, C.c_double)
        specs[i].class_weight = _p(cw, C.c_double)
        specs[i].params = C.pointer(p)
    handles = (C.c_void_p * n)()
    status = np.zeros(n, np.int32)
    _check(lib().rgbm_table_train_batch(specs, C.c_int32(n), handles, _p(status, C.c_int32)), "rgbm_table_train_batch")
    out = []
    failing = [i for i in range(n) if status[i] != 0]
    last_msg = lib().rgbm_last_error().decode("utf-8", "replace") if failing else ""
    for i in range(n):
        if status[i] == 0 and (handles[i] or (keep[i][5] is not None and keep[i][4].reserved & FLAG_NO_MODEL)):
            m = Model(C.c_void_p(handles[i])) if handles[i] else None
            out.append(m if keep[i][5] is None else (m, keep[i][6], keep[i][7]))
        else:
            why = last_msg if (failing and i == failing[-1]) else ("status %d" % int(status[i]) if status[i] != 0 else "no model returned")
            out.append(RepairGbmError("fit %d of the batch failed (%d): %s" % (i, int(status[i]), why)))
    return out


def _chain_args(models, feat_cols, class_codes):
    T = len(models)
    arr = (C.c_void_p * max(T, 1))(*[m.h for m in models])
    fo = np.zeros(T + 1, np.int32)
    co = np.zeros(T + 1, np.int32)
    for t in range(T):
        fo[t + 1] = fo[t] + len(feat_cols[t])
        if class_codes is not None:
            co[t + 1] = co[t] + len(class_codes[t])
    fc = _i32(np.concatenate([np.asarray(f, np.int32) for f in feat_cols])) if T else np.zeros(1, np.int32)
    cc = None
    if class_codes is not None:
        cc = _i32(np.concatenate([np.asarray(c, np.int32) for c in class_codes] + [np.zeros(1, np.int32)]))
    return arr, fc, fo, cc, co


def repair_chain(models, target_col, feat_cols, class_codes, table, device_id=0):
    T = len(models)
    Cc, n = table.shape
    assert table.dtype == np.int32 and table.flags.c_contiguous
    arr, fc, fo, cc, co = _chain_args(models, feat_cols, class_codes)
    tc = _i32(target_col)
    lab = np.zeros((T, n), np.int32)
    prob = np.zeros((T, n), np.float64)
    _check(lib().rgbm_repair_chain(arr, C.c_int32(T), _p(tc, C.c_int32), _p(fc, C.c_int32), _p(fo, C.c_int32), _p(cc, C.c_int32),
                                   _p(co, C.c_int32), _p(table, C.c_int32), C.c_int64(n), C.c_int32(Cc), C.c_int32(device_id),
                                   _p(lab, C.c_int32), _p(prob, C.c_double)), "rgbm_repair_chain")
    return lab, prob


class _PinnedBlock:

    def __init__(self, nbytes):
        p = C.c_void_p()
        _check(lib().rgbm_host_alloc(C.c_size_t(nbytes), C.byref(p)), "rgbm_host_alloc")
        self.p, self.nbytes = p, nbytes
        self.__array_interface__ = {"shape": (nbytes,), "typestr": "|u1", "data": (p.value, False), "version": 3}

    def __del__(self):
        if getattr(self, "p", None):
            lib().rgbm_host_free(self.p)
            self.p = None


def pinned_empty(shape, dtype=np.int32):
    n = int(np.prod(shape)) * np.dtype(dtype).itemsize
    return np.asarray(_PinnedBlock(max(n, 1)))[:n].view(dtype).reshape(shape)


def pack_code_points(strings):
    strings = [str(s) for s in strings]
    off = np.zeros(len(strings) + 1, np.int64)
    if strings:
        np.cumsum([len(s) for s in strings], out=off[1:])
    cp = np.frombuffer("".join(strings).encode("utf-32-le", "surrogatepass"), dtype="<u4").astype(np.int32)
    return cp, off


def edit_distance(a, b, device_id=0):
    a_cp, a_off = pack_code_points(a)
    b_cp, b_off = pack_code_points(b)
    out = np.zeros((len(a_off) - 1, len(b_off) - 1), np.int32)
    _check(lib().rgbm_edit_distance(C.c_int32(device_id), _p(a_cp, C.c_int32), _p(a_off, C.c_int64), C.c_int64(len(a_off) - 1),
                                    _p(b_cp, C.c_int32), _p(b_off, C.c_int64), C.c_int64(len(b_off) - 1), _p(out, C.c_int32)),
           "rgbm_edit_distance")
    return out


def nearest_values(a=None, b=None, cost=None, threshold=0.0, device_id=0):
    if cost is not None:
        m = _f64(cost)
        if m.ndim != 2:
            raise ValueError("cost must be a [n_a][n_b] matrix")
        out = np.full(m.shape[0], -1, np.int32)
        _check(lib().rgbm_nearest_values(C.c_int32(device_id), None, None, C.c_int64(m.shape[0]), None, None, C.c_int64(m.shape[1]),
                                         _p(m, C.c_double), C.c_double(threshold), _p(out, C.c_int32)), "rgbm_nearest_values")
        return out
    a_cp, a_off = pack_code_points(a)
    b_cp, b_off = pack_code_points(b)
    out = np.full(len(a_off) - 1, -1, np.int32)
    _check(lib().rgbm_nearest_values(C.c_int32(device_id), _p(a_cp, C.c_int32), _p(a_off, C.c_int64), C.c_int64(len(a_off) - 1),
                                     _p(b_cp, C.c_int32), _p(b_off, C.c_int64), C.c_int64(len(b_off) - 1), None, C.c_double(threshold),
                                     _p(out, C.c_int32)), "rgbm_nearest_values")
    return out


def lof_1d(values, counts, k=20, threshold=1.5, want_scores=True, device_id=0):
    v = _f64(values).reshape(-1)
    m = np.ascontiguousarray(counts, np.int64).reshape(-1)
    if len(v) != len(m):
        raise ValueError("values and counts must have one length")
    score = np.zeros(len(v), np.float64) if want_scores else None
    bits = np.zeros((len(v) + 63) // 64, np.uint64)
    info = np.zeros(2, np.int64)
    _check(lib().rgbm_lof_1d(C.c_int32(device_id), _p(v, C.c_double), _p(m, C.c_int64), C.c_int32(len(v)), C.c_int32(int(k)),
                             C.c_double(threshold), _p(score, C.c_double) if want_scores else None, _p(bits, C.c_uint64),
                             _p(info, C.c_int64)), "rgbm_lof_1d")
    return score, bits, int(info[0]), int(info[1])
# ... 372 lines not shown
```

Before: 1.930 million.

## Size level histogram windows by built-node bound and add 64-entry ring form

The level pass planner now computes an upper bound on how many nodes can actually be built at each level given num_leaves, and may split the slot range so the first window covers only that bound with more trees per launch. It also adds a seventh kernel form with a shorter 64-entry ring that frees LDS for more histogram nodes in the rotated single-chunk case. The per-level expand planner replaces the flat rank over min-path gains with an ancestor-path comparison using packed 64-bit paths. This is meant to raise trees per pass and cut wasted histogram work, but it adds another kernel instantiation and more complex planning and ranking logic.

Measured after the change: 1.952 million, median of 3. About the same (+1.1%).

```diff
diff --git a/include/rgbm.h b/include/rgbm.h
--- a/include/rgbm.h
+++ b/include/rgbm.h
@@ -211,7 +211,9 @@
 void rgbm_model_free(rgbm_model* m);
 int rgbm_model_info(const rgbm_model* m, int32_t* info);
 int rgbm_model_predict_form(const rgbm_model* m, int32_t* out);
-int rgbm_level_pass_plan(const int32_t* nbins, int32_t f, int64_t n_rows, int32_t k, int32_t max_depth, int32_t with_mult, double* out, int32_t out_len, int32_t* n_out);
+int rgbm_level_pass_plan(const int32_t* nbins, int32_t f, int64_t n_rows, int32_t k, int32_t max_depth, int32_t with_mult, double* out, int32_t out_len, int32_t* n_out,
+                         int32_t num_leaves);
+int rgbm_level_built_bound(int32_t num_leaves, int32_t level);
 int rgbm_model_importance(const rgbm_model* m, int32_t type, double* out );
 
 #ifdef __cplusplus
diff --git a/spark-data-repair-plugin_amd/csrc/rgbm.hip b/spark-data-repair-plugin_amd/csrc/rgbm.hip
--- a/spark-data-repair-plugin_amd/csrc/rgbm.hip
+++ b/spark-data-repair-plugin_amd/csrc/rgbm.hip
@@ -156,6 +156,7 @@
     bool mt_sparse = true;
     int mt_rot = -1;
     int mt_rot_copies2 = 16;
+    int mt_ring64 = -1;
     int mt_rot_tmin = 2;
     bool step_readback = false;
     int step_threads = 0;
@@ -183,6 +184,7 @@
     if (const char* e = getenv("RGBM_MT_ROT")) w.mt_rot = atoi(e);
     if (const char* e = getenv("RGBM_MT_ROT_COPIES2")) w.mt_rot_copies2 = atoi(e);
     if (const char* e = getenv("RGBM_MT_ROT_TMIN")) w.mt_rot_tmin = atoi(e);
+    if (const char* e = getenv("RGBM_MT_RING64")) w.mt_ring64 = atoi(e);
     if (const char* e = getenv("RGBM_DISTINCT")) w.distinct = atoi(e) != 0;
     if (const char* e = getenv("RGBM_DISTINCT_MAX_RATIO")) { const double r = atof(e); if (r >= 0.0 && r <= 1.0) w.distinct_max_ratio = r; }
     if (const char* e = getenv("RGBM_DISTINCT_MIN_ROWS")) w.distinct_min_rows = std::max(1ll, atoll(e));
@@ -413,7 +415,7 @@
     return used;
 }
 
-struct MtLaunch { int ch, slot0, nslots, route, T, G, gx, acc2, rot; };
+struct MtLaunch { int ch, slot0, nslots, route, T, G, gx, acc2, rot, cap , ring64 ; };
 struct LevelPassPlan {
     int root_gx = 8;
     std::vector<std::vector<MtLaunch>> mt;
@@ -433,8 +435,19 @@
 
 inline int level_lds_bytes(const RunSwitches& sw) { return (sw.lv_lds >= 65536 && sw.lv_lds <= rg::LV_LDS_BYTES) ? sw.lv_lds : rg::LV_LDS_BYTES; }
 
+int level_built_bound(int num_leaves, int level) {
+    const int depth = level - 1;
+    int best = 0;
+    for (int m = 1; m <= (1 << depth); ++m) {
+        int anc = 0;
+        for (int i = 1; i <= depth; ++i) anc += (m + (1 << i) - 1) >> i;
+        if (m - 1 + anc < num_leaves - 1) best = m;
+    }
+    return best;
+}
+
 LevelPassPlan plan_level_passes(const RunSwitches& sw, const std::vector<rg::FeatMeta>& fmeta, const std::vector<rg::ChunkMeta>& cmeta,
-                                long long N, int K, int max_depth, bool wm , int lds_bytes) {
+                                long long N, int K, int max_depth, bool wm , int lds_bytes, int num_leaves) {
     using namespace rg;
     const int nchunk = (int)cmeta.size();
     LevelPassPlan P;
@@ -477,23 +490,49 @@
             long long cap = hist_room / std::max<long long>(node_bytes, 1);
             cap = std::min<long long>(cap, MT_MAX_NODES);
             if (cap < 1) throw std::invalid_argument("histogram of one node exceeds LDS");
-            const int win = (int)std::min<long long>(worst, cap);
-            const long long rep_target = std::max(1, sw.mt_rep);
-            const long long t_nodes = std::max<long long>(win, cap / rep_target);
-            int T = (int)std::max<long long>(1, std::min<long long>(std::min<long long>(t_nodes / win, MT_MAX_T), std::min<long long>(K, MT_RT_BUDGET / (2 * worst))));
-            if (sw.mt_T >= 1) T = std::max(1, std::min(T, sw.mt_T));
             const bool plain1 = nchunk == 1 || acc2;
             const bool rot_full = cmeta[ch].nfeat >= 12 && (!acc2 || cmeta[1].nfeat >= 12);
             const long long rot_node_bytes = node_bytes + mt_rot_dummy(true) * 16;
             const long long cap_rot = std::min<long long>(hist_room / rot_node_bytes, MT_MAX_NODES);
-            const long long T_rot = std::min<long long>(std::min<long long>(cap_rot / win, MT_MAX_T), std::min<long long>(K, MT_RT_BUDGET / (2 * worst)));
-            const bool few_trees = T < sw.mt_rot_tmin && T_rot >= 2 * (long long)T;
-            const bool rot = plain1 && (sw.mt_rot == 1 || (sw.mt_rot < 0 && rot_full && (cap * 2 < (long long)sw.mt_rot_copies2 * T * win || few_trees))) &&
-                             (long long)T * win * rot_node_bytes <= hist_room;
-            if (rot && sw.mt_T < 1) T = (int)std::max<long long>(T, T_rot);
-            const int G = (K + T - 1) / T;
-            for (int s0 = 0; s0 < worst; s0 += win)
-                P.mt[level].push_back(MtLaunch{ch, s0, win, (ch == 0 && s0 == 0) ? 1 : 0, T, G, 0, acc2 ? 1 : 0, rot ? 1 : 0});
+            const bool ring64_form = nchunk == 1 && rot_full && sw.mt_rot != 0 && sw.mt_ring64 != 0;
+            const long long hist_room64 = ring64_form ? mt_hist_bytes(lds_bytes, mt_thr, false, false, li_arr, true) : 0;
+            const long long cap_rot64 = std::min<long long>(hist_room64 / rot_node_bytes, MT_MAX_NODES);
+            struct Sized { int T; bool rot, ring64; int cap; };
+            auto size_window = [&](int win, bool short_rings) {
+                const long long rep_target = std::max(1, sw.mt_rep);
+                const long long t_nodes = std::max<long long>(win, cap / rep_target);
+                int T = (int)std::max<long long>(1, std::min<long long>(std::min<long long>(t_nodes / win, MT_MAX_T), std::min<long long>(K, MT_RT_BUDGET / (2 * worst))));
+                if (sw.mt_T >= 1) T = std::max(1, std::min(T, sw.mt_T));
+                const long long T_rot = std::min<long long>(std::min<long long>(cap_rot / win, MT_MAX_T), std::min<long long>(K, MT_RT_BUDGET / (2 * worst)));
+                const bool few_trees = T < sw.mt_rot_tmin && T_rot >= 2 * (long long)T;
+                const bool rot = plain1 && (sw.mt_rot == 1 || (sw.mt_rot < 0 && rot_full && (cap * 2 < (long long)sw.mt_rot_copies2 * T * win || few_trees))) &&
+                                 (long long)T * win * rot_node_bytes <= hist_room;
+                if (rot && sw.mt_T < 1) T = (int)std::max<long long>(T, T_rot);
+                if (short_rings && ring64_form && (sw.mt_ring64 == 1 ? rot : T == 1)) {
+                    long long T64 = std::min<long long>(std::min<long long>(cap_rot64 / win, MT_MAX_T), std::min<long long>(K, MT_RT_BUDGET / (2 * worst)));
+                    if (sw.mt_T >= 1) T64 = std::min<long long>(T64, sw.mt_T);
+                    if (T64 >= (sw.mt_ring64 == 1 ? 1 : 2)) return Sized{(int)std::max<long long>(T64, sw.mt_ring64 == 1 ? T : 0), true, true, (int)cap_rot64};
+                }
+                return Sized{T, rot, false, (int)(rot ? cap_rot : cap)};
+            };
+            std::vector<int> wins;
+            const int win_all = (int)std::min<long long>(worst, cap);
+            for (int s0 = 0; s0 < worst; s0 += win_all) wins.push_back(std::min(win_all, worst - s0));
+            const int bound = level_built_bound(num_leaves, level);
+            if (bound >= 1 && bound < worst) {
+                const int wb = (int)std::min<long long>(bound, cap);
+                std::vector<int> wins_b{wb};
+                const int win_rest = (int)std::min<long long>(worst - wb, cap);
+                for (int s0 = wb; s0 < worst; s0 += win_rest) wins_b.push_back(std::min(win_rest, worst - s0));
+                const int T_all = size_window(win_all, true).T, T_b = size_window(wb, true).T;
+                if (T_b > T_all && (wins_b.size() <= wins.size() || (wins.size() == 1 && T_b >= 2 * T_all))) wins = wins_b;
+            }
+            int s0 = 0;
+            for (int win : wins) {
+                const Sized z = s0 == 0 ? size_window(win, true) : size_window(win_all, false);
+                P.mt[level].push_back(MtLaunch{ch, s0, win, (ch == 0 && s0 == 0) ? 1 : 0, z.T, (K + z.T - 1) / z.T, 0, acc2 ? 1 : 0, z.rot ? 1 : 0, z.cap, z.ring64 ? 1 : 0});
+                s0 += win;
+            }
         }
         const long long gmin = std::max<long long>(1, (N + (1ll << 22) - 1) >> 22);
         const long long nwt = (N + MT_WT_ROWS - 1) / MT_WT_ROWS;
@@ -555,24 +594,25 @@
 }
 
 #define RGBM_MT_FORMS(X) \
-    X(0, rg::LV_THREADS, false, false, false)  \
-    X(1, rg::LV_THREADS, false, false, false)  \
-    X(1, rg::LV_THREADS, false, false, true)   \
-    X(2, rg::LV_THREADS, false, false, false)  \
-    X(2, rg::MT_THREADS_ACC2, true, true, false)  \
-    X(2, rg::MT_THREADS_ACC2, true, true, true)
-struct MtForm { int nchr, threads; bool acc2, spec, rot; };
+    X(0, rg::LV_THREADS, false, false, false, false)  \
+    X(1, rg::LV_THREADS, false, false, false, false)  \
+    X(1, rg::LV_THREADS, false, false, true, false)   \
+    X(1, rg::LV_THREADS, false, false, true, true)    \
+    X(2, rg::LV_THREADS, false, false, false, false)  \
+    X(2, rg::MT_THREADS_ACC2, true, true, false, false)  \
+    X(2, rg::MT_THREADS_ACC2, true, true, true, false)
+struct MtForm { int nchr, threads; bool acc2, spec, rot, ring64; };
 constexpr MtForm MT_FORMS[] = {
-#define RGBM_MT_FORM_ENTRY(NCHR, THR, ACC, SPEC, ROT) {NCHR, THR, ACC, SPEC, ROT},
+#define RGBM_MT_FORM_ENTRY(NCHR, THR, ACC, SPEC, ROT, R64) {NCHR, THR, ACC, SPEC, ROT, R64},
     RGBM_MT_FORMS(RGBM_MT_FORM_ENTRY)
 #undef RGBM_MT_FORM_ENTRY
 };
-using MtKernel = decltype(&rg::k_level_mt<1, false, true, rg::LV_THREADS, false, false, false>);
+using MtKernel = decltype(&rg::k_level_mt<1, false, true, rg::LV_THREADS, false, false, false, false>);
 MtKernel mt_kernel(const MtForm& f, bool bag, bool route) {
-#define RGBM_MT_FORM_KERNEL(NCHR, THR, ACC, SPEC, ROT) \
-    if (f.nchr == NCHR && f.threads == THR && f.acc2 == ACC && f.spec == SPEC && f.rot == ROT) \
-        return bag ? (route ? rg::k_level_mt<NCHR, true, true, THR, ACC, SPEC, ROT> : rg::k_level_mt<NCHR, true, false, THR, ACC, SPEC, ROT>) \
-                   : (route ? rg::k_level_mt<NCHR, false, true, THR, ACC, SPEC, ROT> : rg::k_level_mt<NCHR, false, false, THR, ACC, SPEC, ROT>);
+#define RGBM_MT_FORM_KERNEL(NCHR, THR, ACC, SPEC, ROT, R64) \
+    if (f.nchr == NCHR && f.threads == THR && f.acc2 == ACC && f.spec == SPEC && f.rot == ROT && f.ring64 == R64) \
+        return bag ? (route ? rg::k_level_mt<NCHR, true, true, THR, ACC, SPEC, ROT, R64> : rg::k_level_mt<NCHR, true, false, THR, ACC, SPEC, ROT, R64>) \
+                   : (route ? rg::k_level_mt<NCHR, false, true, THR, ACC, SPEC, ROT, R64> : rg::k_level_mt<NCHR, false, false, THR, ACC, SPEC, ROT, R64>);
     RGBM_MT_FORMS(RGBM_MT_FORM_KERNEL)
 #undef RGBM_MT_FORM_KERNEL
     throw std::logic_error("level pass: no such launch form");
@@ -813,7 +853,7 @@
     int32_t h_err = 0;
     std::vector<rg::RootLayout> h_root_lay; std::vector<rg::MtLayout> h_mt_lay; std::vector<int> mt_lay_keys;
     DevBuf<rg::RootLayout> root_lay; DevBuf<rg::MtLayout> mt_lay;
-    static int mt_lay_key(const MtLaunch& L) { return L.ch * 4 + (L.acc2 ? 2 : 0) + (L.rot ? 1 : 0); }
+    static int mt_lay_key(const MtLaunch& L) { return L.ch * 8 + (L.ring64 ? 4 : 0) + (L.acc2 ? 2 : 0) + (L.rot ? 1 : 0); }
     int mt_lay_index(const MtLaunch& L) const {
         for (size_t i = 0; i < mt_lay_keys.size(); ++i) if (mt_lay_keys[i] == mt_lay_key(L)) return (int)i;
         return -1;
@@ -827,7 +867,7 @@
         lc.num_leaves = st.NL; lc.max_depth = st.p.max_depth; lc.min_data_in_leaf = st.p.min_data_in_leaf; lc.N = st.N; lc.NS = (st.N + 255) & ~255ll; lc.NG = lc.NS;
         lc.sib_local = (st.dp && comm_rank() == 0) ? 1 : 0;
         lc.has_mult = st.tab.has_mult ? 1u : 0u;
-        passes = plan_level_passes(st.sw, st.h.fmeta, st.h.cmeta, st.N, st.K, st.p.max_depth, st.tab.has_mult, lc.lds_bytes);
+        passes = plan_level_passes(st.sw, st.h.fmeta, st.h.cmeta, st.N, st.K, st.p.max_depth, st.tab.has_mult, lc.lds_bytes, st.NL);
         lc.gx = passes.root_gx; lc.xcd_blocks = 1; lc.max_built = 1;
         node.alloc((size_t)st.K * lc.NS);
         HIPCHK(hipMemsetAsync(node.p, 0xFF, (size_t)st.K * lc.NS, s));
@@ -874,13 +914,13 @@
             const bool li_in_rec = nf_last <= 15 && !st.tab.has_mult;
             mt_lay_keys.push_back(mt_lay_key(L)); h_mt_lay.emplace_back();
             mt_layout_fill(h_mt_lay.back(), st.h.fmeta.data() + cm.first_feat, cm.nfeat, acc2 ? st.h.fmeta.data() + st.h.cmeta[1].first_feat : nullptr, acc2 ? st.h.cmeta[1].nfeat : 0,
-                           cm.wide_bins, L.rot != 0, mt_hist_bytes(lc.lds_bytes, acc2 ? MT_THREADS_ACC2 : LV_THREADS, acc2, acc2, !li_in_rec));
+                           cm.wide_bins, L.rot != 0, mt_hist_bytes(lc.lds_bytes, acc2 ? MT_THREADS_ACC2 : LV_THREADS, acc2, acc2, !li_in_rec, L.ring64 != 0));
         }
         if (!h_mt_lay.empty()) { mt_lay.alloc(h_mt_lay.size()); mt_lay.upload(h_mt_lay.data(), h_mt_lay.size(), s); }
         if (st.sw.timing) {
             fprintf(stderr, "[rgbm] root: gx %d joint %d groups %d\n", lc.gx, joint_root ? 1 : 0, joint_root ? lcj.F : 0);
             for (int level = 1; level < st.p.max_depth; ++level) for (const auto& L : passes.mt[level])
-                fprintf(stderr, "[rgbm] level %d launch: chunk %d slots %d..%d route %d T %d G %d gx %d acc2 %d rot %d\n", level, L.ch, L.slot0, L.slot0 + L.nslots - 1, L.route, L.T, L.G, L.gx, L.acc2, L.rot);
+                fprintf(stderr, "[rgbm] level %d launch: chunk %d slots %d..%d route %d T %d G %d gx %d acc2 %d rot %d ring64 %d\n", level, L.ch, L.slot0, L.slot0 + L.nslots - 1, L.route, L.T, L.G, L.gx, L.acc2, L.rot, L.ring64);
         }
         rgh::once_per_device(st.tab.device, rgh::ONCE_LEVEL_LDS, [] {
             HIPCHK(hipFuncSetAttribute((const void*)rg::k_level_root, hipFuncAttributeMaxDynamicSharedMemorySize, rg::LV_LDS_BYTES));
@@ -943,7 +983,7 @@
                 l1.mt_T = L.T; l1.mt_G = L.G; l1.mt_ch = L.ch; l1.mt_slot0 = L.slot0; l1.mt_nslots = L.nslots; l1.mt_route = L.route; l1.mt_sparse = st.sw.mt_sparse ? 1 : 0;
                 l1.mt_lay = mt_lay.p + mt_lay_index(L);
                 const bool acc2 = L.acc2 != 0;
-                const MtForm form{acc2 ? 2 : (st.h.nchunk <= 2 ? st.h.nchunk : 0), acc2 ? MT_THREADS_ACC2 : LV_THREADS, acc2, acc2, L.rot != 0};
+                const MtForm form{acc2 ? 2 : (st.h.nchunk <= 2 ? st.h.nchunk : 0), acc2 ? MT_THREADS_ACC2 : LV_THREADS, acc2, acc2, L.rot != 0, L.ring64 != 0};
                 st.timers.timed(false, [&]() {
                     launch_level_mt(form, st.use_bagging, L.route != 0, dim3((unsigned)L.G * (unsigned)L.gx), s, st.bins.rec.p, st.gh.p, node.p, st.bag.inbag.p,
                                     plan.p, part.p, count.p, st.bins.fmeta.p, st.bins.cmeta.p, err.p, st.fxs.p, l1);
@@ -2124,7 +2164,7 @@
     });
 }
 
-RGBM_EXPORT int rgbm_level_pass_plan(const int32_t* nbins, int32_t f, int64_t n_rows, int32_t k, int32_t max_depth, int32_t with_mult, double* out, int32_t out_len, int32_t* n_out) {
+RGBM_EXPORT int rgbm_level_pass_plan(const int32_t* nbins, int32_t f, int64_t n_rows, int32_t k, int32_t max_depth, int32_t with_mult, double* out, int32_t out_len, int32_t* n_out, int32_t num_leaves) {
     if (!nbins || !out || !n_out || f < 1 || f > 255 || n_rows < 1 || k < 1 || max_depth < 1 || max_depth > rg::LV_MAX_DEPTH) return fail(RGBM_ERR_ARG, "rgbm_level_pass_plan: bad argument");
     return guarded([&]() {
         using namespace rg;
@@ -2139,7 +2179,7 @@
             ChunkMeta& cm = cmeta[ch]; cm.first_feat = (int)ch * 16; cm.nfeat = std::min(16, f - (int)ch * 16); cm.fast_slots = 0; cm.wide_bins = 0;
             for (int j = 0; j < cm.nfeat; ++j) { fmeta[ch * 16 + j].wide_off = cm.wide_bins; cm.wide_bins += fmeta[ch * 16 + j].nbins; }
         }
-        const LevelPassPlan P = plan_level_passes(sw, fmeta, cmeta, n_rows, k, max_depth, with_mult != 0, level_lds_bytes(sw));
+        const LevelPassPlan P = plan_level_passes(sw, fmeta, cmeta, n_rows, k, max_depth, with_mult != 0, level_lds_bytes(sw), num_leaves < 2 ? 31 : num_leaves);
         std::vector<double> v;
         const long long root_wg = (long long)P.root_gx * k * (long long)cmeta.size();
         v.insert(v.end(), {(double)P.root_gx, (double)P.part_items, 0.0, (double)root_wg, ROOT_PASS_COST.t_fix_us, (double)n_rows / P.root_gx * ROOT_PASS_COST.t_row_ns * 1e-3});
@@ -2147,7 +2187,8 @@
         for (int level = 1; level < max_depth; ++level) for (const MtLaunch& L : P.mt[level]) {
             const PassCost& c = mt_pass_cost(L.acc2 != 0, L.rot != 0);
             v.insert(v.end(), {(double)level, (double)L.ch, (double)L.slot0, (double)L.nslots, (double)L.route, (double)L.T, (double)L.G, (double)L.gx, (double)L.acc2, (double)L.rot,
-                               c.t_fix_us, (double)n_rows / L.gx * (c.t_row_ns + std::min(L.T, (int)k) * c.t_pair_ns) * 1e-3});
+                               c.t_fix_us, (double)n_rows / L.gx * (c.t_row_ns + std::min(L.T, (int)k) * c.t_pair_ns) * 1e-3, (double)L.cap,
+                               (double)level_built_bound(num_leaves < 2 ? 31 : num_leaves, level), (double)L.ring64});
             ++nl;
         }
         v[2] = (double)nl;
@@ -2158,6 +2199,11 @@
     });
 }
 
+RGBM_EXPORT int rgbm_level_built_bound(int32_t num_leaves, int32_t level) {
+    if (num_leaves < 2 || level < 1 || level > rg::LV_MAX_DEPTH) return -1;
+    return level_built_bound(num_leaves, level);
+}
+
 RGBM_EXPORT int rgbm_model_importance(const rgbm_model* m, int32_t type, double* out) {
     if (!m || !out) return fail(RGBM_ERR_ARG, "rgbm_model_importance: bad argument");
     for (int f = 0; f < m->F; ++f) out[f] = 0.0;
diff --git a/spark-data-repair-plugin_amd/csrc/rgbm_level.h b/spark-data-repair-plugin_amd/csrc/rgbm_level.h
--- a/spark-data-repair-plugin_amd/csrc/rgbm_level.h
+++ b/spark-data-repair-plugin_amd/csrc/rgbm_level.h
@@ -22,7 +22,8 @@
 constexpr int MT_WT_ROWS = 256;
 constexpr int MT_RING_PLAIN = 128;
 constexpr int MT_RING_SPEC = 128;
-__host__ __device__ constexpr int mt_ring(bool spec) { return spec ? MT_RING_SPEC : MT_RING_PLAIN; }
+constexpr int MT_RING_SHORT = 64;
+__host__ __device__ constexpr int mt_ring(bool spec, bool ring64 = false) { return spec ? MT_RING_SPEC : (ring64 ? MT_RING_SHORT : MT_RING_PLAIN); }
 constexpr int MT_CNT_REP = 4;
 
 constexpr int MT_THREADS_ACC2 = 768;
@@ -98,13 +99,14 @@
 #define MT_SPARSE_DIV_N 16
 #endif
 constexpr long long MT_SPARSE_DIV = MT_SPARSE_DIV_N;
-__host__ __device__ constexpr long long mt_fixed_bytes(int threads, bool acc2, bool spec = false, bool li = true ) {
+__host__ __device__ constexpr long long mt_fixed_bytes(int threads, bool acc2, bool spec = false, bool li = true ,
+                                                       bool ring64 = false) {
     return ((!acc2 && !spec) ? (long long)MT_MAX_T * 8  : 0) + (long long)MT_MAX_T * 32 + MT_MAX_NODES + 16 + 512 + 256 + (long long)(MT_MAX_T + 2) * 8 + (long long)MT_MAX_RT * 8 + (long long)MT_MAX_NODES * MT_CNT_REP * 4 + (long long)MT_MAX_NODES * 8 +
-           (long long)(threads / 64 - (spec ? MT_CONSUMERS : 0)) * mt_ring(spec) * ((acc2 ? 32 : 16) + 8 + (li ? 2 : 0)) + 256;
-}
-__host__ __device__ constexpr long long mt_hd(int threads, bool acc2, bool spec) { return ((LV_LDS_TOTAL - mt_fixed_bytes(threads, acc2, spec, false)) / 2) & ~15ll; }
-__host__ __device__ constexpr long long mt_hist_bytes(long long lds_bytes, int threads, bool acc2, bool spec, bool li) {
-    const long long fixed = mt_fixed_bytes(threads, acc2, spec, li), hd = mt_hd(threads, acc2, spec);
+           (long long)(threads / 64 - (spec ? MT_CONSUMERS : 0)) * mt_ring(spec, ring64) * ((acc2 ? 32 : 16) + 8 + (li ? 2 : 0)) + 256;
+}
+__host__ __device__ constexpr long long mt_hd(int threads, bool acc2, bool spec, bool ring64 = false) { return ((LV_LDS_TOTAL - mt_fixed_bytes(threads, acc2, spec, false, ring64)) / 2) & ~15ll; }
+__host__ __device__ constexpr long long mt_hist_bytes(long long lds_bytes, int threads, bool acc2, bool spec, bool li, bool ring64 = false) {
+    const long long fixed = mt_fixed_bytes(threads, acc2, spec, li, ring64), hd = mt_hd(threads, acc2, spec, ring64);
     const long long room_h = (long long)LV_LDS_TOTAL - fixed - hd;
     const long long x = hd < room_h ? hd : room_h;
     const long long a = lds_bytes - fixed;
@@ -291,20 +293,21 @@
           bool ROUTE ,
           int THREADS , bool ACC2 ,
           bool SPEC ,
-          bool ROTP = false >
+          bool ROTP = false ,
+          bool RING64 = false >
 __global__ __launch_bounds__(THREADS, 1) void k_level_mt(const uint4* __restrict__ rec, const float2* __restrict__ gh, uint8_t* __restrict__ node ,
                                                          const uint8_t* __restrict__ inbag, const LvPlan* __restrict__ plan, HistBin* __restrict__ part,
                                                          int32_t* __restrict__ count, const FeatMeta* __restrict__ fmeta, const ChunkMeta* __restrict__ cmeta,
                                                          int32_t* __restrict__ err_flag,
                                                          const FxScale* __restrict__ fxs , LevelConst c) {
     static_assert(!ACC2 || NCHR == 2, "a two-chunk pass keeps both records in registers");
-    static_assert(ACC2 == SPEC && THREADS == (ACC2 ? MT_THREADS_ACC2 : LV_THREADS) && (!ROTP || NCHR == 1 || ACC2) && (NCHR == 0 || NCHR == 1 || NCHR == 2),
-                  "k_level_mt: not one of the six launch forms");
+    static_assert(ACC2 == SPEC && THREADS == (ACC2 ? MT_THREADS_ACC2 : LV_THREADS) && (!ROTP || NCHR == 1 || ACC2) && (NCHR == 0 || NCHR == 1 || NCHR == 2) &&
+                  (!RING64 || (ROTP && NCHR == 1 && !ACC2)), "k_level_mt: not one of the seven launch forms");
     constexpr int WAVES = THREADS / 64;
     constexpr int NCONS = SPEC ? MT_CONSUMERS : 0, NPROD = WAVES - NCONS;
     constexpr int NACC = ACC2 ? 2 : 1;
     constexpr int NRINGS = SPEC ? NPROD : WAVES;
-    constexpr int MT_RING = mt_ring(SPEC);
+    constexpr int MT_RING = mt_ring(SPEC, RING64);
     constexpr bool ROT = ROTP;
     constexpr bool SPARSE = (NCHR == 1) && !ACC2 && !SPEC;
     extern __shared__ __attribute__((aligned(16))) unsigned char smem[];
@@ -342,9 +345,9 @@
     unsigned long long* xmask = reinterpret_cast<unsigned long long*>(smem + off);
     if (!ACC2 && !SPEC) off += (size_t)MT_MAX_T * 8;
     unsigned long long* hist_g = reinterpret_cast<unsigned long long*>(smem + off);
-    constexpr int MT_HD = (int)mt_hd(THREADS, ACC2, SPEC);
-    const long long avail = mt_hist_bytes(c.lds_bytes, THREADS, ACC2, SPEC, !li_in_rec);
-    if (tid == 0 && ((long long)off > mt_fixed_bytes(THREADS, ACC2, SPEC, !li_in_rec) || (long long)off + MT_HD + avail / 2 > (long long)LV_LDS_TOTAL)) atomicOr(err_flag, 2);
+    constexpr int MT_HD = (int)mt_hd(THREADS, ACC2, SPEC, RING64);
+    const long long avail = mt_hist_bytes(c.lds_bytes, THREADS, ACC2, SPEC, !li_in_rec, RING64);
+    if (tid == 0 && ((long long)off > mt_fixed_bytes(THREADS, ACC2, SPEC, !li_in_rec, RING64) || (long long)off + MT_HD + avail / 2 > (long long)LV_LDS_TOTAL)) atomicOr(err_flag, 2);
 
     const MtLayout* __restrict__ lay = c.mt_lay;
     if (tid < 64) {
@@ -1064,32 +1067,67 @@
 
 __global__ __launch_bounds__(64) void k_level_plan(LvPlan* __restrict__ plan, SNode* __restrict__ nodes, const FeatMeta* __restrict__ fmeta,
                                                    int level, TrainConst c, LevelConst lc) {
-    __shared__ double pm[256];
+    static_assert(LV_MAX_DEPTH <= 8, "a node's path is the bytes of one 64-bit word");
+    __shared__ double sm[256][LV_MAX_DEPTH];
+    __shared__ unsigned long long anc[256];
+    __shared__ double gn[256];
+    __shared__ short par[256];
+    __shared__ unsigned char dep[256];
     const int k = blockIdx.x, lane = lane_id();
     LvPlan* pp = &plan[k];
     if (pp->done) return;
     SNode* nk = nodes + (long long)k * 256;
     const int first = pp->lvl_first, end = pp->lvl_end, nlev = end - first;
-    for (int n = lane; n < first; n += 64) pm[n] = nk[n].pmin;
-    __syncthreads();
+    double v = -INFINITY;
     if (lane < nlev) {
         const int n = first + lane;
         const double g = nk[n].best.gain;
-        const int par = nk[n].parent;
-        double v = g;
-        if (par >= 0) { const double pv = pm[par]; v = (pv < g) ? pv : g; }
+        const int pa = nk[n].parent;
+        v = g;
+        if (pa >= 0) { const double pv = nk[pa].pmin; v = (pv < g) ? pv : g; }
         if (!(g > -INFINITY)) v = -INFINITY;
-        pm[n] = v; nk[n].pmin = v;
-    }
-    __syncthreads();
-    bool expand = false;
-    if (lane < nlev) {
-        const double v = pm[first + lane];
-        if (v > 0.0) {
-            int rank = 0;
-            for (int y = 0; y < end; ++y) rank += (pm[y] > v) ? 1 : 0;
-            expand = rank < c.num_leaves - 1;
-        }
+        nk[n].pmin = v;
+    }
+    bool expand = lane < nlev && v > 0.0;
+    if (end >= c.num_leaves) {
+        for (int n = lane; n < end; n += 64) {
+            const double g = nk[n].best.gain;
+            gn[n] = (g > -INFINITY) ? g : -INFINITY; par[n] = (short)nk[n].parent; dep[n] = (unsigned char)nk[n].depth;
+        }
+        __syncthreads();
+        for (int n = lane; n < end; n += 64) {
+            const int d = dep[n];
+            double r = gn[n];
+            unsigned long long a = (unsigned long long)n << (8 * d);
+            sm[n][d] = r;
+            int pa = par[n];
+            for (int j = d - 1; j >= 0; --j) {
+                const double gp = gn[pa];
+                r = (gp < r) ? gp : r;
+                sm[n][j] = r; a |= (unsigned long long)pa << (8 * j);
+                pa = par[pa];
+            }
+            anc[n] = a;
+        }
+        __syncthreads();
+        int wl = 0; while ((1 << wl) < nlev) ++wl;
+        const int x = lane & ((1 << wl) - 1), part = lane >> wl, nparts = 64 >> wl;
+        int rank = 0;
+        if (x < nlev) {
+            const int X = first + x;
+            const unsigned long long ax = anc[X];
+#pragma unroll 4
+            for (int y = part; y < end; y += nparts) {
+                const unsigned long long diff = (anc[y] ^ ax) & (~0ull >> (56 - 8 * (int)dep[y]));
+                if (diff) {
+                    const int j = (__ffsll((long long)diff) - 1) >> 3;
+                    rank += (sm[y][j] > sm[X][j]) ? 1 : 0;
+                }
+            }
+        }
+        for (int o = 1 << wl; o < 64; o <<= 1) rank += __shfl_xor(rank, o);
+        rank += level - 1;
+        expand = expand && rank < c.num_leaves - 1;
     }
     const unsigned long long em = __ballot(expand);
     const int n_exp = __popcll(em);
diff --git a/spark-data-repair-plugin_amd/repair/_native.py b/spark-data-repair-plugin_amd/repair/_native.py
--- a/spark-data-repair-plugin_amd/repair/_native.py
+++ b/spark-data-repair-plugin_amd/repair/_native.py
@@ -86,7 +86,7 @@
                      "rgbm_table_read_row_multiplicity", "rgbm_table_detect_dc", "rgbm_table_detect_row_bits",
                      "rgbm_table_kmeans_assign", "rgbm_table_kmeans_read", "rgbm_lof_1d", "rgbm_table_column_stats"):
             getattr(l, name).restype = C.c_int
-        for name in ("rgbm_table_distinct_view_info", "rgbm_distinct_view_eligible", "rgbm_level_pass_plan"):
+        for name in ("rgbm_table_distinct_view_info", "rgbm_distinct_view_eligible", "rgbm_level_pass_plan", "rgbm_level_built_bound"):
             if hasattr(l, name):
                 getattr(l, name).restype = C.c_int
         l.rgbm_local_group_free.restype = None
@@ -113,7 +113,7 @@
     "rgbm_table_fd_map", "rgbm_table_rule_fill", "rgbm_nearest_values", "rgbm_table_detect_cells",
     "rgbm_table_distinct_rows", "rgbm_table_read_row_multiplicity", "rgbm_table_detect_dc", "rgbm_table_detect_row_bits", "rgbm_model_predict_form",
     "rgbm_table_kmeans_assign", "rgbm_table_kmeans_read", "rgbm_table_distinct_view_info", "rgbm_distinct_view_eligible",
-    "rgbm_table_column_stats", "rgbm_level_pass_plan",
+    "rgbm_table_column_stats", "rgbm_level_pass_plan", "rgbm_level_built_bound",
 ]
 EXPORTED_SYMBOLS_WITH_DIGITS = ["rgbm_lof_1d"]
 
@@ -364,17 +364,24 @@
                 ("valid_table", C.c_void_p), ("valid_label_out", C.POINTER(C.c_int32)), ("valid_value_out", C.POINTER(C.c_double))]
 
 
-def level_pass_plan(nbins, rows, K, max_depth=7, with_mult=False):
+def level_built_bound(num_leaves, level):
+    r = lib().rgbm_level_built_bound(C.c_int32(num_leaves), C.c_int32(level))
+    if r < 0:
+        raise RepairGbmError("rgbm_level_built_bound: bad argument")
+    return int(r)
+
+
+def level_pass_plan(nbins, rows, K, max_depth=7, with_mult=False, num_leaves=31):
     nb = _i32(nbins)
-    out = np.zeros(6 + 12 * 4096, np.float64)
+    out = np.zeros(6 + 15 * 4096, np.float64)
     n = C.c_int32(0)
     _check(lib().rgbm_level_pass_plan(_p(nb, C.c_int32), C.c_int32(len(nb)), C.c_int64(rows), C.c_int32(K), C.c_int32(max_depth), C.c_int32(1 if with_mult else 0),
-                                      _p(out, C.c_double), C.c_int32(len(out)), C.byref(n)), "rgbm_level_pass_plan")
+                                      _p(out, C.c_double), C.c_int32(len(out)), C.byref(n), C.c_int32(num_leaves)), "rgbm_level_pass_plan")
     keys = ("level", "ch", "slot0", "nslots", "route", "T", "G", "gx", "acc2", "rot")
     launches = []
     for i in range(int(out[2])):
-        v = out[6 + 12 * i: 18 + 12 * i]
-        launches.append(dict({k: int(x) for k, x in zip(keys, v)}, t_fix_us=float(v[10]), t_rows_us=float(v[11])))
+        v = out[6 + 15 * i: 21 + 15 * i]
+        launches.append(dict({k: int(x) for k, x in zip(keys, v)}, t_fix_us=float(v[10]), t_rows_us=float(v[11]), cap=int(v[12]), bound=int(v[13]), ring64=int(v[14])))
     return dict(root_gx=int(out[0]), part_items=int(out[1]), root_workgroups=int(out[3]), root_t_fix_us=float(out[4]), root_t_rows_us=float(out[5]), launches=launches)
 
 
```
